# JuliaRobotics/IncrementalInference.jl

Measured on AMD Instinct MI355X. Metric: clique-messages/sec, higher is better.
Workload: dtype f64; 1 GPU; config 2: ContinuousEuclid(2) 1000-variable odometry chain + priors every 100, N=200 particles, nested-dissection order, full up+down solveTree; variables_per_gpu=1000, particles=200, cliques=983, parallelism=single GPU

## Files before the change

include/nbp.h:

```cpp
#ifndef NBP_H
#define NBP_H

#include <stdint.h>

#ifdef __cplusplus
extern "C" {
#endif

#define NBP_MAXV 6
#define NBP_MAXF 128
#define NBP_MAXD 3
#define NBP_MAXC 4
#define NBP_MAXK 8
#define NBP_MAXN 512
#define NBP_COMP_STRIDE 13
enum nbp_dist {
  NBP_DIST_GAUSSIAN = 0,
  NBP_DIST_UNIFORM = 1,
  NBP_DIST_RAYLEIGH = 2,
  NBP_DIST_TABLE = 3
};

typedef int32_t nbp_status;
#define NBP_OK 0
#define NBP_ERR_ARG (-1)
#define NBP_ERR_HIP (-2)
#define NBP_ERR_NOGPU (-3)
#define NBP_ERR_RANGE (-4)

enum nbp_manifold {
  NBP_EUCLID1 = 1,
  NBP_EUCLID2 = 2,
  NBP_EUCLID3 = 3,
  NBP_CIRCULAR = 4,
  NBP_SE2 = 5
};

enum nbp_factor {
  NBP_F_PRIOR = 1,
  NBP_F_MSGPRIOR = 2,
  NBP_F_LINREL = 3,
  NBP_F_CIRCULAR = 4,
  NBP_F_SE2 = 5,
  NBP_F_EUCLIDDIST = 6,
  NBP_F_PASSTHROUGH = 7
};

typedef struct nbp_proposal_desc {
  int32_t factor_kind;
  int32_t manifold;
  int32_t nvars;
  int32_t sfidx;
  int32_t var_slot[NBP_MAXV];
  int32_t out_slot;
  int32_t ncomp;
  int32_t has_multihypo;
  int32_t inflate_cycles;
  int32_t mhidx_in;
  int32_t mhidx_out;
  int32_t skip_bandwidth;
  int32_t partial_mask;
  int32_t meas_kde;
  int32_t keep_count;
  double multihypo[NBP_MAXV];
  double nullhypo;
  double inflation;
  double spread_nh;
  double comp[NBP_MAXC][NBP_COMP_STRIDE];
  uint64_t seed;
  uint64_t meas_seed;
} nbp_proposal_desc;

typedef struct nbp_product_desc {
  int32_t manifold;
  int32_t nfactors;
  int32_t niter;
  int32_t out_slot;
  int32_t in_slot[NBP_MAXF];
  int32_t labels_out;
  int32_t old_slot;
  uint8_t in_partial[NBP_MAXF];
  uint64_t seed;
} nbp_product_desc;

typedef struct nbp_copy_desc {
  int32_t src_slot;
  int32_t dst_slot;
} nbp_copy_desc;

typedef struct nbp_diag {
  int64_t solves;
  int64_t nonconverged;
  int64_t nan_results;
  int64_t residual_evals;
  int64_t lcv_evals;
  int64_t lcv_evals_f32;
  int64_t proposal_launches_workgroup;
  int64_t proposal_launches_wave;
  int64_t proposal_launches_split;
  int64_t lane_side_launches;
  int64_t lane_waits;
  int64_t lane_side_updates;
} nbp_diag;

typedef struct nbp_ctx nbp_ctx;

int64_t nbp_arena_bytes(int32_t N, int32_t n_slots);
int64_t nbp_slot_stride_doubles(int32_t N);
nbp_status nbp_ctx_create(int32_t device, int32_t N, int32_t n_slots, void *arena,
                          int64_t arena_bytes, int32_t side_ints, nbp_ctx **out);
nbp_status nbp_ctx_destroy(nbp_ctx *ctx);
nbp_status nbp_ctx_attach(nbp_ctx *ctx, void *obj, void (*destroy)(void *obj));
void *nbp_ctx_attached(const nbp_ctx *ctx);
const char *nbp_last_error(void);
nbp_status nbp_synchronize(nbp_ctx *ctx);
void *nbp_arena_ptr(nbp_ctx *ctx);
void *nbp_stream_ptr(nbp_ctx *ctx);
int32_t nbp_ctx_particles(const nbp_ctx *ctx);
int32_t nbp_ctx_slots(const nbp_ctx *ctx);
int32_t nbp_ctx_device(const nbp_ctx *ctx);
nbp_status nbp_ctx_reserve_resident(nbp_ctx *ctx, int32_t n);
int32_t nbp_ctx_resident(const nbp_ctx *ctx);

nbp_status nbp_slot_write(nbp_ctx *ctx, int32_t slot, int32_t manifold, const double *pts_NxP,
                          const double *bw_D );
nbp_status nbp_slot_read(nbp_ctx *ctx, int32_t slot, int32_t manifold, double *pts_NxP,
                         double *bw_D );
nbp_status nbp_belief_write(nbp_ctx *ctx, int32_t slot, int32_t manifold, const double *pts_NxP, int32_t n_pts,
                            const double *bw_D , const double *ipc_D );
nbp_status nbp_belief_read(nbp_ctx *ctx, int32_t slot, int32_t manifold, double *pts_NxP, int32_t *n_pts ,
                           double *bw_D , double *ipc_D );
nbp_status nbp_belief_write_batch(nbp_ctx *ctx, int32_t n, const int32_t *slots, const int32_t *manifolds, const double *const *pts,
                                  const int32_t *n_pts, const double *const *bw, const double *const *ipc);
nbp_status nbp_belief_read_batch(nbp_ctx *ctx, int32_t n, const int32_t *slots, const int32_t *manifolds, double *const *pts,
                                 int32_t *n_pts, double *const *bw, double *const *ipc);
typedef struct nbp_read_token nbp_read_token;
nbp_status nbp_belief_write_batch_async(nbp_ctx *ctx, int32_t n, const int32_t *slots, const int32_t *manifolds, const double *const *pts,
                                        const int32_t *n_pts, const double *const *bw, const double *const *ipc);
nbp_status nbp_belief_read_batch_begin(nbp_ctx *ctx, int32_t n, const int32_t *slots, nbp_read_token **out);
nbp_status nbp_belief_read_batch_end(nbp_read_token *token, const int32_t *manifolds, double *const *pts, int32_t *n_pts,
                                     double *const *bw, double *const *ipc);
nbp_status nbp_run_resample(nbp_ctx *ctx, const int32_t *slots, const int32_t *manifolds, int32_t n, uint64_t seed);
nbp_status nbp_side_write(nbp_ctx *ctx, int32_t offset, const int32_t *src, int32_t n);
nbp_status nbp_side_read(nbp_ctx *ctx, int32_t offset, int32_t *dst, int32_t n);

nbp_status nbp_run_proposals(nbp_ctx *ctx, const nbp_proposal_desc *descs, int32_t n);
nbp_status nbp_run_bandwidth(nbp_ctx *ctx, const int32_t *slots, const int32_t *manifolds, int32_t n);
nbp_status nbp_run_ppe(nbp_ctx *ctx, const int32_t *slots, const int32_t *manifolds, int32_t n,
                       double *mean_out , double *max_out ,
                       int32_t *max_index_out );
nbp_status nbp_kde_ppe(nbp_ctx *ctx, int32_t manifold, const double *pts_NxP, int32_t n_pts, const double *bw_D,
                       double *mean_out_D, double *max_out_D, int32_t *max_index_out );
nbp_status nbp_run_evaluate(nbp_ctx *ctx, const int32_t *slots, const int32_t *manifolds, int32_t n,
                            const int32_t *q_first ,
                            const double *queries , double *dens_out );
nbp_status nbp_kde_evaluate(nbp_ctx *ctx, int32_t manifold, const double *pts_NxP, int32_t n_pts, const double *bw_D,
                            const double *queries , int32_t nq, double *dens_out);
#define NBP_GRID_MAX 1024
#define NBP_GRID_AUTO_EXTENT 1
typedef struct nbp_grid_desc {
  int32_t slot;
  int32_t manifold;
  int32_t dims[2];
  int32_t n[2];
  int32_t flags;
  double lo[2];
  double step[2];
  double margin;
} nbp_grid_desc;
nbp_status nbp_run_marginal_grid(nbp_ctx *ctx, const nbp_grid_desc *descs, int32_t n_desc, const int32_t *first ,
                                 double *out , double *extent_out );
nbp_status nbp_kde_marginal_grid(nbp_ctx *ctx, int32_t manifold, const double *pts_NxP, int32_t n_pts, const double *bw_D,
                                 const nbp_grid_desc *desc, double *out, double *extent_out_4 );
nbp_status nbp_run_evaluate_marginal(nbp_ctx *ctx, const int32_t *slots, const int32_t *manifolds, const int32_t *masks, int32_t n,
                                     const int32_t *q_first ,
                                     const double *queries , double *dens_out );
nbp_status nbp_run_mmd(nbp_ctx *ctx, const int32_t *slots_a, const int32_t *slots_b, const int32_t *manifolds, int32_t n,
                       double sigma, double *mmd_out );
nbp_status nbp_kde_mmd(nbp_ctx *ctx, int32_t manifold, const double *a_NxP, int32_t na, const double *b_NxP, int32_t nb,
                       double sigma, double *mmd_out);
nbp_status nbp_run_meancov(nbp_ctx *ctx, const int32_t *slots, const int32_t *manifolds, int32_t n,
                           double *mean_out , double *cov_out );
nbp_status nbp_kde_meancov(nbp_ctx *ctx, int32_t manifold, const double *pts_NxP, int32_t n_pts, double *mean_out_D,
                           double *cov_out_DxD);
nbp_status nbp_run_kld(nbp_ctx *ctx, const int32_t *slots_a, const int32_t *slots_b, const int32_t *manifolds, int32_t n,
// ... 124 lines not shown
  double comp[NBP_MAXC][NBP_COMP_STRIDE];
} nbp_likelihood_desc;
nbp_status nbp_run_factor_likelihood(nbp_ctx *ctx, const nbp_likelihood_desc *descs, int32_t n, double *loglik_out ,
                                     double *comp_loglik_out );
nbp_status nbp_factor_likelihood(nbp_ctx *ctx, const nbp_likelihood_desc *desc, const double *a_NxP, int32_t na, const double *b_NxP,
                                 int32_t nb, double *loglik_out, double *comp_loglik_out );
#define NBP_PGRID_AUTO_EXTENT 1
#define NBP_PGRID_MAX_CELLS (1 << 22)
#define NBP_PGRID_CHUNK 256
typedef struct nbp_product_item {
  nbp_likelihood_desc lik;
  int32_t role;
  int32_t other;
  int32_t group;
  int32_t pad;
  double log_prior;
} nbp_product_item;
typedef struct nbp_product_grid_desc {
  int32_t manifold;
  int32_t slot;
  int32_t n[3];
  int32_t flags;
  int32_t first_item;
  int32_t n_items;
  double lo[3];
  double step[3];
  double margin;
} nbp_product_grid_desc;
typedef struct nbp_product_grid_rec {
  double logZ;
  double logmax;
  int32_t argmax;
  int32_t pad;
} nbp_product_grid_rec;
nbp_status nbp_run_product_grid(nbp_ctx *ctx, const nbp_product_grid_desc *descs, int32_t n_desc, const nbp_product_item *items,
                                int32_t n_items, const int32_t *first , double *logp_out ,
                                nbp_product_grid_rec *recs_out , double *extent_out );
nbp_status nbp_product_grid(nbp_ctx *ctx, const nbp_product_grid_desc *desc, const nbp_product_item *items, int32_t n_items,
                            const double *const *others , const int32_t *counts , const double *own_NxP,
                            int32_t n_own, const double *own_bw_D, double *logp_out, nbp_product_grid_rec *rec_out ,
                            double *extent_out_6 );
nbp_status nbp_run_factor_mode_likelihood(nbp_ctx *ctx, const nbp_likelihood_desc *descs, const int32_t *row_a ,
                                          const int32_t *row_b , int32_t n, const int32_t *labels ,
                                          int32_t n_rows, double *table_out ,
                                          int32_t *counts_out );
nbp_status nbp_factor_mode_likelihood(nbp_ctx *ctx, const nbp_likelihood_desc *desc, const double *a_NxP, int32_t na,
                                      const int32_t *labels_a , const double *b_NxP, int32_t nb,
                                      const int32_t *labels_b , double *table_out ,
                                      int32_t *counts_out );
#define NBP_ERR_INVALID (-5)
typedef struct nbp_heatmap nbp_heatmap;
nbp_status nbp_heatmap_create(nbp_ctx *ctx, const double *data , int32_t nx, int32_t ny, const double *x, const double *y,
                              double bw_factor, nbp_heatmap **out);
nbp_status nbp_heatmap_build(nbp_heatmap *hm, int32_t M, uint64_t seed, int32_t *cell_M, double *pre_Mx2, double *d_M, double *W_M);
nbp_status nbp_heatmap_draw(nbp_heatmap *hm, int32_t n, uint64_t seed, int32_t jitter, int32_t slot , int32_t *pick_n,
                            double *pts_nx2, double *bw_2);
nbp_status nbp_heatmap_info(const nbp_heatmap *hm, double *bw_2, double *total, double *wtotal, int32_t *M);
nbp_status nbp_heatmap_destroy(nbp_heatmap *hm);
nbp_status nbp_heatmap_scan_eval(nbp_ctx *ctx, const double *in, int32_t n, double *out);
nbp_status nbp_heatmap_search_eval(nbp_ctx *ctx, const double *cdf, int32_t n, const double *t, int32_t nt, int32_t *idx_out);
nbp_status nbp_run_products(nbp_ctx *ctx, const nbp_product_desc *descs, int32_t n);
nbp_status nbp_kde_bandwidth(nbp_ctx *ctx, int32_t manifold, const double *pts_NxP, double *bw_out_D);
nbp_status nbp_conv(nbp_ctx *ctx, const nbp_proposal_desc *tmpl, const double *const *var_pts, const double *const *var_bw,
                    const int32_t *mhidx_in, double *out_pts_NxP, double *out_bw_D, int32_t *out_mhidx);
nbp_status nbp_manifold_product(nbp_ctx *ctx, int32_t manifold, int32_t nfactors, const double *const *dens_pts,
                                const double *const *dens_bw, const uint8_t *partial_masks, const double *old_pts,
                                int32_t niter, uint64_t seed, double *out_pts_NxP, double *out_bw_D, int32_t *out_labels);

nbp_status nbp_run_deconv(nbp_ctx *ctx, const nbp_proposal_desc *descs, const int32_t *meas_slots, int32_t n);
nbp_status nbp_run_copies(nbp_ctx *ctx, const nbp_copy_desc *descs, int32_t n);
nbp_status nbp_run_copies_async(nbp_ctx *ctx, const nbp_copy_desc *descs, int32_t n, int32_t points_only);

typedef struct nbp_program nbp_program;
enum nbp_stage_kind {
  NBP_STAGE_PROPOSALS = 1,
  NBP_STAGE_PRODUCTS = 2,
  NBP_STAGE_COPIES = 3,
  NBP_STAGE_DECONV = 4,
  NBP_STAGE_COPY_POINTS = 5
};
nbp_status nbp_program_create(nbp_ctx *ctx, nbp_program **out);
nbp_status nbp_program_add_stage(nbp_program *prog, int32_t kind, const void *descs, int32_t n);
enum nbp_program_option { NBP_OPT_LAZY_BANDWIDTH = 1, NBP_OPT_GRAPH_REPLAY = 2, NBP_OPT_FUSED_UPDATES = 3,
                          NBP_OPT_ASYNC_UPLOAD = 4  };
nbp_status nbp_program_set_option(nbp_program *prog, int32_t option, int32_t value);
nbp_status nbp_program_finalize(nbp_program *prog);
nbp_status nbp_program_run(nbp_program *prog, int32_t first_stage, int32_t last_stage );
nbp_status nbp_program_reseed(nbp_program *prog, uint64_t salt);
nbp_status nbp_program_num_seeds(nbp_program *prog, int32_t *out);
nbp_status nbp_program_set_seeds(nbp_program *prog, const uint64_t *seeds, int32_t n);
nbp_status nbp_program_seed_order(nbp_program *prog, int32_t *order, int32_t n);
nbp_status nbp_program_num_stages(nbp_program *prog, int32_t *out);
nbp_status nbp_program_num_fused(nbp_program *prog, int32_t *out);
nbp_status nbp_program_num_two_stream(nbp_program *prog, int32_t *out);
nbp_status nbp_program_set_lanes(nbp_program *prog, int32_t stage, const int32_t *lane_of_descriptor, int32_t n);
typedef struct nbp_lane_part_rec {
  int32_t stage, lane, first_desc, n, wait, signals;
} nbp_lane_part_rec;
nbp_status nbp_program_lane_plan(nbp_program *prog, nbp_lane_part_rec *out, int32_t cap, int32_t *n_out);
nbp_status nbp_program_destroy(nbp_program *prog);
nbp_status nbp_program_retire(nbp_program *prog);

#define NBP_COMM_ID_BYTES 128
typedef struct nbp_comm nbp_comm;
#ifndef NBP_XFER_DEFINED
#define NBP_XFER_DEFINED
typedef struct nbp_xfer { int32_t peer; int32_t slot; } nbp_xfer;
#endif
nbp_status nbp_comm_unique_id(void *id_out );
nbp_status nbp_comm_create(nbp_ctx *ctx, int32_t world, int32_t rank, const void *id, nbp_comm **out);
nbp_status nbp_comm_destroy(nbp_comm *comm);
nbp_status nbp_comm_info(nbp_comm *comm, int32_t *nranks_out, int32_t *rank_out);
nbp_status nbp_exchange(nbp_ctx *ctx, nbp_comm *comm, const nbp_xfer *sends, int32_t n_sends, const nbp_xfer *recvs, int32_t n_recvs);

nbp_status nbp_timing_enable(nbp_ctx *ctx, int32_t on);
nbp_status nbp_timing_read(nbp_ctx *ctx, double *ms, int64_t *launches);
nbp_status nbp_timing_read_n(nbp_ctx *ctx, double *ms, int64_t *launches, int32_t n);
nbp_status nbp_diag_read(nbp_ctx *ctx, nbp_diag *out, int32_t reset);

typedef struct nbp_product_plan_req {
  int32_t N;
  int32_t n;
  int32_t F, D;
  int32_t mani;
  int32_t geom_n;
} nbp_product_plan_req;
#define NBP_PLAN_REFUSED_BIG_IN_ROUND 1
#define NBP_PLAN_REFUSED_LDS 2
#define NBP_PLAN_REFUSED_NO_KERNEL 3
typedef struct nbp_product_plan_rec {
  int32_t status, refusal;
  int32_t HL, wpb, G;
  int32_t big, xs, circ, nch, all_levels, w1;
  int32_t row;
  int32_t row_HL, row_mani, row_xs, row_w1;
  int32_t launch_bound;
  int32_t N, n, F, D, mani, geom_n;
  int32_t pad;
  int64_t lds, gstats;
  char kernel[40];
} nbp_product_plan_rec;
typedef struct nbp_fit_plan_req {
  int32_t N;
  int32_t fits, coords;
  int32_t products, kdF;
  int32_t geom_blocks;
} nbp_fit_plan_req;
typedef struct nbp_fit_plan_rec {
  int32_t status;
  int32_t P, depth, KS, w5, threads;
  int32_t prep;
  int32_t kd_nostats;
  int32_t N, fits, coords, products, kdF, geom_blocks;
  int32_t pad[2];
  int64_t lds;
  char kernel[40];
} nbp_fit_plan_rec;
typedef struct nbp_proposal_plan_req {
  int32_t N, n;
  int32_t manifold;
  int32_t simple;
} nbp_proposal_plan_req;
typedef struct nbp_proposal_plan_rec {
  int32_t status;
  int32_t geometry;
  int32_t blocks, threads;
  int32_t N, n, manifold, simple;
  int64_t lds;
  char kernel[40];
} nbp_proposal_plan_rec;
nbp_status nbp_plan_products(const nbp_product_plan_req *req, nbp_product_plan_rec *out, int64_t n);
nbp_status nbp_plan_fits(const nbp_fit_plan_req *req, nbp_fit_plan_rec *out, int64_t n);
nbp_status nbp_plan_proposals(const nbp_proposal_plan_req *req, nbp_proposal_plan_rec *out, int64_t n);
nbp_status nbp_last_plans(nbp_ctx *ctx, nbp_product_plan_rec *product, nbp_fit_plan_rec *prep, nbp_fit_plan_rec *fits);

nbp_status nbp_math_eval(nbp_ctx *ctx, int32_t fn, const double *a, const double *b, double *out0, double *out1, int64_t n);

#ifdef __cplusplus
}
#endif
#endif
```

incrementalinference.jl_amd/abi.py:

```python
import ctypes as C
import os

MAXV, MAXF, MAXD, MAXC, MAXN, COMP_STRIDE = 6, 128, 3, 4, 512, 13

EUCLID1, EUCLID2, EUCLID3, CIRCULAR, SE2 = 1, 2, 3, 4, 5
F_PRIOR, F_MSGPRIOR, F_LINREL, F_CIRCULAR, F_SE2, F_EUCLIDDIST, F_PASSTHROUGH = 1, 2, 3, 4, 5, 6, 7
DIST_GAUSSIAN, DIST_UNIFORM, DIST_RAYLEIGH, DIST_TABLE = 0, 1, 2, 3
STAGE_PROPOSALS, STAGE_PRODUCTS, STAGE_COPIES, STAGE_DECONV, STAGE_COPY_POINTS = 1, 2, 3, 4, 5
OPT_LAZY_BANDWIDTH = 1
OPT_GRAPH_REPLAY = 2
OPT_FUSED_UPDATES = 3

MANIFOLD_DIM = {EUCLID1: 1, EUCLID2: 2, EUCLID3: 3, CIRCULAR: 1, SE2: 3}
MANIFOLD_P = {EUCLID1: 1, EUCLID2: 2, EUCLID3: 3, CIRCULAR: 1, SE2: 6}


class ProposalDesc(C.Structure):
    _fields_ = [
        ("factor_kind", C.c_int32),
        ("manifold", C.c_int32),
        ("nvars", C.c_int32),
        ("sfidx", C.c_int32),
        ("var_slot", C.c_int32 * MAXV),
        ("out_slot", C.c_int32),
        ("ncomp", C.c_int32),
        ("has_multihypo", C.c_int32),
        ("inflate_cycles", C.c_int32),
        ("mhidx_in", C.c_int32),
        ("mhidx_out", C.c_int32),
        ("skip_bandwidth", C.c_int32),
        ("partial_mask", C.c_int32),
        ("meas_kde", C.c_int32),
        ("keep_count", C.c_int32),
        ("multihypo", C.c_double * MAXV),
        ("nullhypo", C.c_double),
        ("inflation", C.c_double),
        ("spread_nh", C.c_double),
        ("comp", (C.c_double * COMP_STRIDE) * MAXC),
        ("seed", C.c_uint64),
        ("meas_seed", C.c_uint64),
    ]


class ProductDesc(C.Structure):
    _fields_ = [
        ("manifold", C.c_int32),
        ("nfactors", C.c_int32),
        ("niter", C.c_int32),
        ("out_slot", C.c_int32),
        ("in_slot", C.c_int32 * MAXF),
        ("labels_out", C.c_int32),
        ("old_slot", C.c_int32),
        ("in_partial", C.c_uint8 * MAXF),
        ("seed", C.c_uint64),
    ]


class CopyDesc(C.Structure):
    _fields_ = [("src_slot", C.c_int32), ("dst_slot", C.c_int32)]


class GridDesc(C.Structure):
    _fields_ = [
        ("slot", C.c_int32),
        ("manifold", C.c_int32),
        ("dims", C.c_int32 * 2),
        ("n", C.c_int32 * 2),
        ("flags", C.c_int32),
        ("lo", C.c_double * 2),
        ("step", C.c_double * 2),
        ("margin", C.c_double),
    ]


GRID_MAX, GRID_AUTO_EXTENT = 1024, 1


class ModesOpts(C.Structure):
    _fields_ = [("bw_scale", C.c_double), ("tol", C.c_double), ("merge", C.c_double), ("max_iter", C.c_int32), ("pad", C.c_int32)]


class ModeRec(C.Structure):
    _fields_ = [("location", C.c_double * MAXD), ("density", C.c_double), ("count", C.c_int32), ("leader", C.c_int32)]


MODES_MAX = 32
MODES_BW_SCALE, MODES_TOL, MODES_MAX_ITER, MODES_MERGE = 2.0, 1e-6, 500, 1e-2

MIX_MAX = 8
MIX_TOL, MIX_MAX_ITER = 1e-8, 500


class MixtureOpts(C.Structure):
    _fields_ = [("tol", C.c_double), ("max_iter", C.c_int32), ("pad", C.c_int32)]
# ... 10 lines not shown
                ("partial_mask", C.c_int32), ("comp", (C.c_double * COMP_STRIDE) * MAXC)]


class ProductItem(C.Structure):
    _fields_ = [("lik", LikelihoodDesc), ("role", C.c_int32), ("other", C.c_int32), ("group", C.c_int32), ("pad", C.c_int32),
                ("log_prior", C.c_double)]


class ProductGridDesc(C.Structure):
    _fields_ = [("manifold", C.c_int32), ("slot", C.c_int32), ("n", C.c_int32 * 3), ("flags", C.c_int32), ("first_item", C.c_int32),
                ("n_items", C.c_int32), ("lo", C.c_double * 3), ("step", C.c_double * 3), ("margin", C.c_double)]


class ProductGridRec(C.Structure):
    _fields_ = [("logZ", C.c_double), ("logmax", C.c_double), ("argmax", C.c_int32), ("pad", C.c_int32)]


PGRID_AUTO_EXTENT, PGRID_MAX_CELLS, PGRID_CHUNK, PGRID_MARGIN = 1, 1 << 22, 256, 4.0


MAXK = 8


class OverlapRec(C.Structure):
    _fields_ = [("logc", C.c_double), ("lab", C.c_double), ("laa", C.c_double), ("lbb", C.c_double)]


class OverlapOpts(C.Structure):
    _fields_ = [("reach", C.c_double), ("min_coeff", C.c_double), ("topk", C.c_int32), ("pad", C.c_int32)]


OVERLAP_MAXK, OVERLAP_REACH, OVERLAP_MIN_COEFF, OVERLAP_TOPK = 16, 6.0, 1e-3, 8


class SceneDesc(C.Structure):
    _fields_ = [("n", C.c_int32 * 2), ("flags", C.c_int32), ("pad", C.c_int32), ("lo", C.c_double * 2), ("step", C.c_double * 2),
                ("margin", C.c_double), ("reach", C.c_double)]


SCENE_AUTO_EXTENT, SCENE_MAX, SCENE_REACH, SCENE_MARGIN, SCENE_MAX_POINTS = 1, 4096, 6.0, 4.0, 1 << 22

CRED_MAX = 8


class CredibleOpts(C.Structure):
    _fields_ = [("n_mass", C.c_int32), ("n_prob", C.c_int32), ("mass", C.c_double * CRED_MAX), ("prob", C.c_double * CRED_MAX)]


class CredibleRec(C.Structure):
    _fields_ = [("log_level", C.c_double * CRED_MAX), ("quant", (C.c_double * CRED_MAX) * MAXD), ("mean", C.c_double * MAXD),
                ("log_min", C.c_double), ("log_max", C.c_double), ("n_inside", C.c_int32 * CRED_MAX), ("count", C.c_int32),
                ("pad", C.c_int32)]


class CredibilityRec(C.Structure):
    _fields_ = [("logdens", C.c_double), ("mass", C.c_double), ("n_above", C.c_int32), ("pad", C.c_int32)]


ERR_INVALID = -5
HM_MAX_CELLS = 1 << 26


class Xfer(C.Structure):
    _fields_ = [("peer", C.c_int32), ("slot", C.c_int32)]


COMM_ID_BYTES = 128


class Diag(C.Structure):
    _fields_ = [
        ("solves", C.c_int64),
        ("nonconverged", C.c_int64),
        ("nan_results", C.c_int64),
        ("residual_evals", C.c_int64),
        ("lcv_evals", C.c_int64),
        ("lcv_evals_f32", C.c_int64),
        ("proposal_launches_workgroup", C.c_int64),
        ("proposal_launches_wave", C.c_int64),
        ("proposal_launches_split", C.c_int64),
        ("lane_side_launches", C.c_int64),
        ("lane_waits", C.c_int64),
        ("lane_side_updates", C.c_int64),
    ]


class LanePartRec(C.Structure):
    _fields_ = [("stage", C.c_int32), ("lane", C.c_int32), ("first_desc", C.c_int32), ("n", C.c_int32), ("wait", C.c_int32), ("signals", C.c_int32)]


class ProductPlanReq(C.Structure):
    _fields_ = [(k, C.c_int32) for k in ("N", "n", "F", "D", "mani", "geom_n")]


PLAN_REFUSED_BIG_IN_ROUND, PLAN_REFUSED_LDS, PLAN_REFUSED_NO_KERNEL = 1, 2, 3


class _PlanRec(C.Structure):
    def as_dict(self):
        return {k: (getattr(self, k).decode() if k == "kernel" else getattr(self, k)) for k, _ in self._fields_ if not k.startswith("pad")}


class ProductPlanRec(_PlanRec):
    _fields_ = [(k, C.c_int32) for k in ("status", "refusal", "HL", "wpb", "G", "big", "xs", "circ", "nch", "all_levels", "w1", "row", "row_HL",
                                         "row_mani", "row_xs", "row_w1", "launch_bound", "N", "n", "F", "D", "mani", "geom_n", "pad")] + \
               [("lds", C.c_int64), ("gstats", C.c_int64), ("kernel", C.c_char * 40)]


class FitPlanReq(C.Structure):
    _fields_ = [(k, C.c_int32) for k in ("N", "fits", "coords", "products", "kdF", "geom_blocks")]


class FitPlanRec(_PlanRec):
    _fields_ = [(k, C.c_int32) for k in ("status", "P", "depth", "KS", "w5", "threads", "prep", "kd_nostats", "N", "fits", "coords", "products",
                                         "kdF", "geom_blocks")] + [("pad", C.c_int32 * 2), ("lds", C.c_int64), ("kernel", C.c_char * 40)]


class ProposalPlanReq(C.Structure):
    _fields_ = [(k, C.c_int32) for k in ("N", "n", "manifold", "simple")]


class ProposalPlanRec(_PlanRec):
    _fields_ = [(k, C.c_int32) for k in ("status", "geometry", "blocks", "threads", "N", "n", "manifold", "simple")] + \
               [("lds", C.c_int64), ("kernel", C.c_char * 40)]


def _plan(fn_name, Req, Rec, reqs):
    lib = load_library()
    n = len(reqs)
    arr = (Req * n)(*[Req(*r) for r in reqs])
    out = (Rec * n)()
    rc = getattr(lib, fn_name)(arr, out, n)
    if rc != 0:
        raise ValueError(f"{fn_name}: status {rc}: {lib.nbp_last_error().decode()}")
    return out


def plan_products(reqs):
    return _plan("nbp_plan_products", ProductPlanReq, ProductPlanRec, reqs)


def plan_fits(reqs):
    return _plan("nbp_plan_fits", FitPlanReq, FitPlanRec, reqs)


def plan_proposals(reqs):
    return _plan("nbp_plan_proposals", ProposalPlanReq, ProposalPlanRec, reqs)


def slot_stride(N):
    return 3 * N + 8


_PKG_DIR = os.path.dirname(os.path.abspath(__file__))
LIB_PATH = os.path.join(_PKG_DIR, "csrc", "libnbp.so")

EXPORTS = [
    "nbp_arena_bytes", "nbp_slot_stride_doubles", "nbp_ctx_create", "nbp_ctx_destroy",
    "nbp_last_error", "nbp_synchronize", "nbp_arena_ptr", "nbp_stream_ptr", "nbp_ctx_particles", "nbp_ctx_slots", "nbp_ctx_device",
    "nbp_ctx_reserve_resident", "nbp_ctx_resident", "nbp_belief_write_batch_async", "nbp_belief_read_batch_begin", "nbp_belief_read_batch_end",
    "nbp_run_copies_async", "nbp_program_retire",
    "nbp_slot_write", "nbp_slot_read", "nbp_belief_write", "nbp_belief_read", "nbp_belief_write_batch", "nbp_belief_read_batch", "nbp_run_resample", "nbp_side_write", "nbp_side_read",
    "nbp_run_proposals", "nbp_run_bandwidth", "nbp_run_ppe", "nbp_kde_ppe", "nbp_run_evaluate", "nbp_kde_evaluate", "nbp_run_marginal_grid", "nbp_kde_marginal_grid", "nbp_run_evaluate_marginal", "nbp_run_mmd", "nbp_kde_mmd", "nbp_run_meancov", "nbp_kde_meancov", "nbp_run_kld", "nbp_kde_kld", "nbp_run_overlap", "nbp_kde_overlap", "nbp_run_overlap_search", "nbp_run_scene_grid", "nbp_run_credible", "nbp_kde_credible", "nbp_run_modes", "nbp_kde_modes", "nbp_run_mixture", "nbp_kde_mixture", "nbp_run_factor_likelihood", "nbp_factor_likelihood", "nbp_run_factor_mode_likelihood", "nbp_factor_mode_likelihood", "nbp_run_product_grid", "nbp_product_grid", "nbp_heatmap_create", "nbp_heatmap_build", "nbp_heatmap_draw", "nbp_heatmap_info", "nbp_heatmap_destroy", "nbp_heatmap_scan_eval", "nbp_heatmap_search_eval", "nbp_run_products", "nbp_run_copies", "nbp_run_deconv", "nbp_kde_bandwidth", "nbp_conv", "nbp_manifold_product",
    "nbp_program_create", "nbp_program_add_stage", "nbp_program_set_option", "nbp_program_finalize", "nbp_program_run",
    "nbp_program_reseed", "nbp_program_num_seeds", "nbp_program_set_seeds", "nbp_program_seed_order", "nbp_ctx_attach", "nbp_ctx_attached", "nbp_program_num_stages", "nbp_program_num_fused", "nbp_program_num_two_stream", "nbp_program_set_lanes", "nbp_program_lane_plan", "nbp_program_destroy",
    "nbp_timing_enable", "nbp_timing_read", "nbp_timing_read_n", "nbp_diag_read",
    "nbp_plan_products", "nbp_plan_fits", "nbp_plan_proposals", "nbp_last_plans",
    "nbp_comm_unique_id", "nbp_comm_create", "nbp_comm_destroy", "nbp_comm_info", "nbp_exchange", "nbp_math_eval",
]

_lib = None


def load_library(path=None):
    global _lib
    if _lib is not None and path is None:
        return _lib
    path = path or os.environ.get("NBP_LIB_OVERRIDE") or LIB_PATH
    if not os.path.exists(path):
        raise RuntimeError(
            f"libnbp.so not found at {path}: build it with `python __graft_entry__.py` "
            "(hipcc --offload-arch=gfx950). The product path has no CPU fallback."
        )
    try:
        import torch
    except ImportError:
        pass
    lib = C.CDLL(path)
    vp, i32, i64, dp = C.c_void_p, C.c_int32, C.c_int64, C.POINTER(C.c_double)
    ip = C.POINTER(C.c_int32)
    lib.nbp_arena_bytes.restype = i64
    lib.nbp_arena_bytes.argtypes = [i32, i32]
    lib.nbp_slot_stride_doubles.restype = i64
    lib.nbp_slot_stride_doubles.argtypes = [i32]
    lib.nbp_ctx_create.argtypes = [i32, i32, i32, vp, i64, i32, C.POINTER(vp)]
    lib.nbp_ctx_destroy.argtypes = [vp]
    lib.nbp_last_error.restype = C.c_char_p
    lib.nbp_synchronize.argtypes = [vp]
    lib.nbp_arena_ptr.restype = vp
    lib.nbp_arena_ptr.argtypes = [vp]
    lib.nbp_stream_ptr.restype = vp
    lib.nbp_stream_ptr.argtypes = [vp]
    lib.nbp_ctx_particles.argtypes = [vp]
    lib.nbp_ctx_slots.argtypes = [vp]
    lib.nbp_ctx_device.argtypes = [vp]
    lib.nbp_slot_write.argtypes = [vp, i32, i32, dp, dp]
    lib.nbp_slot_read.argtypes = [vp, i32, i32, dp, dp]
    lib.nbp_belief_write.argtypes = [vp, i32, i32, dp, i32, dp, dp]
    lib.nbp_belief_read.argtypes = [vp, i32, i32, dp, ip, dp, dp]
    lib.nbp_belief_write_batch.argtypes = [vp, i32, ip, ip, C.POINTER(dp), ip, C.POINTER(dp), C.POINTER(dp)]
    lib.nbp_belief_read_batch.argtypes = [vp, i32, ip, ip, C.POINTER(dp), ip, C.POINTER(dp), C.POINTER(dp)]
    lib.nbp_run_resample.argtypes = [vp, ip, ip, i32, C.c_uint64]
    lib.nbp_side_write.argtypes = [vp, i32, ip, i32]
    lib.nbp_side_read.argtypes = [vp, i32, ip, i32]
    lib.nbp_run_proposals.argtypes = [vp, C.POINTER(ProposalDesc), i32]
    lib.nbp_run_bandwidth.argtypes = [vp, ip, ip, i32]
    lib.nbp_run_ppe.argtypes = [vp, ip, ip, i32, dp, dp, ip]
    lib.nbp_kde_ppe.argtypes = [vp, i32, dp, i32, dp, dp, dp, ip]
    lib.nbp_run_evaluate.argtypes = [vp, ip, ip, i32, ip, dp, dp]
    lib.nbp_kde_evaluate.argtypes = [vp, i32, dp, i32, dp, dp, i32, dp]
    lib.nbp_run_marginal_grid.argtypes = [vp, C.POINTER(GridDesc), i32, ip, dp, dp]
    lib.nbp_kde_marginal_grid.argtypes = [vp, i32, dp, i32, dp, C.POINTER(GridDesc), dp, dp]
    lib.nbp_run_evaluate_marginal.argtypes = [vp, ip, ip, ip, i32, ip, dp, dp]
    lib.nbp_run_mmd.argtypes = [vp, ip, ip, ip, i32, C.c_double, dp]
    lib.nbp_kde_mmd.argtypes = [vp, i32, dp, i32, dp, i32, C.c_double, dp]
    lib.nbp_run_meancov.argtypes = [vp, ip, ip, i32, dp, dp]
    lib.nbp_kde_meancov.argtypes = [vp, i32, dp, i32, dp, dp]
    lib.nbp_run_kld.argtypes = [vp, ip, ip, ip, i32, dp, dp]
    lib.nbp_kde_kld.argtypes = [vp, i32, dp, i32, dp, dp, i32, dp, dp, dp]
    lib.nbp_run_overlap.argtypes = [vp, ip, ip, ip, ip, ip, ip, i32, C.POINTER(OverlapRec)]
    lib.nbp_kde_overlap.argtypes = [vp, i32, dp, i32, dp, i32, i32, dp, i32, dp, i32, C.POINTER(OverlapRec)]
    lib.nbp_run_overlap_search.argtypes = [vp, ip, ip, ip, i32, C.POINTER(OverlapOpts), ip, dp, ip, ip]
    lib.nbp_run_scene_grid.argtypes = [vp, ip, ip, ip, dp, i32, C.POINTER(SceneDesc), dp, ip, ip, dp, C.POINTER(i64)]
    lib.nbp_run_credible.argtypes = [vp, ip, ip, ip, i32, C.POINTER(CredibleOpts), ip, dp, C.POINTER(CredibleRec), dp, ip,
                                     C.POINTER(CredibilityRec)]
    lib.nbp_kde_credible.argtypes = [vp, i32, dp, i32, dp, i32, C.POINTER(CredibleOpts), dp, i32, C.POINTER(CredibleRec), dp, ip,
                                     C.POINTER(CredibilityRec)]
    lib.nbp_run_modes.argtypes = [vp, ip, ip, i32, C.POINTER(ModesOpts), C.POINTER(ModeRec), ip, ip, ip, ip]
    lib.nbp_kde_modes.argtypes = [vp, i32, dp, i32, dp, C.POINTER(ModesOpts), C.POINTER(ModeRec), ip, ip, ip, ip]
    lib.nbp_run_mixture.argtypes = [vp, ip, ip, i32, ip, ip, dp, C.POINTER(MixtureOpts), C.POINTER(MixtureRec), ip]
    lib.nbp_kde_mixture.argtypes = [vp, i32, dp, i32, dp, ip, dp, C.POINTER(MixtureOpts), C.POINTER(MixtureRec), ip]
    lib.nbp_run_factor_likelihood.argtypes = [vp, C.POINTER(LikelihoodDesc), i32, dp, dp]
    lib.nbp_factor_likelihood.argtypes = [vp, C.POINTER(LikelihoodDesc), dp, i32, dp, i32, dp, dp]
    lib.nbp_run_factor_mode_likelihood.argtypes = [vp, C.POINTER(LikelihoodDesc), ip, ip, i32, ip, i32, dp, ip]
    lib.nbp_factor_mode_likelihood.argtypes = [vp, C.POINTER(LikelihoodDesc), dp, i32, ip, dp, i32, ip, dp, ip]
    lib.nbp_run_product_grid.argtypes = [vp, C.POINTER(ProductGridDesc), i32, C.POINTER(ProductItem), i32, ip, dp, C.POINTER(ProductGridRec), dp]
    lib.nbp_product_grid.argtypes = [vp, C.POINTER(ProductGridDesc), C.POINTER(ProductItem), i32, C.POINTER(dp), ip, dp, i32, dp, dp,
                                     C.POINTER(ProductGridRec), dp]
    lib.nbp_heatmap_create.argtypes = [vp, dp, i32, i32, dp, dp, C.c_double, C.POINTER(vp)]
    lib.nbp_heatmap_build.argtypes = [vp, i32, C.c_uint64, ip, dp, dp, dp]
    lib.nbp_heatmap_draw.argtypes = [vp, i32, C.c_uint64, i32, i32, ip, dp, dp]
    lib.nbp_heatmap_info.argtypes = [vp, dp, dp, dp, ip]
    lib.nbp_heatmap_destroy.argtypes = [vp]
    lib.nbp_heatmap_scan_eval.argtypes = [vp, dp, i32, dp]
    lib.nbp_heatmap_search_eval.argtypes = [vp, dp, i32, dp, i32, ip]
    lib.nbp_run_deconv.argtypes = [vp, C.POINTER(ProposalDesc), ip, i32]
    dpp = C.POINTER(dp)
    lib.nbp_kde_bandwidth.argtypes = [vp, i32, dp, dp]
    lib.nbp_conv.argtypes = [vp, C.POINTER(ProposalDesc), dpp, dpp, ip, dp, dp, ip]
    lib.nbp_manifold_product.argtypes = [vp, i32, i32, dpp, dpp, C.POINTER(C.c_uint8), dp, i32, C.c_uint64, dp, dp, ip]
    lib.nbp_run_products.argtypes = [vp, C.POINTER(ProductDesc), i32]
    lib.nbp_run_copies.argtypes = [vp, C.POINTER(CopyDesc), i32]
    lib.nbp_program_create.argtypes = [vp, C.POINTER(vp)]
    lib.nbp_program_add_stage.argtypes = [vp, i32, vp, i32]
    lib.nbp_program_set_option.argtypes = [vp, i32, i32]
    lib.nbp_program_finalize.argtypes = [vp]
    lib.nbp_program_run.argtypes = [vp, i32, i32]
    lib.nbp_program_reseed.argtypes = [vp, C.c_uint64]
    lib.nbp_program_num_seeds.argtypes = [vp, ip]
    lib.nbp_program_set_seeds.argtypes = [vp, C.POINTER(C.c_uint64), i32]
    lib.nbp_program_seed_order.argtypes = [vp, ip, i32]
    lib.nbp_program_num_stages.argtypes = [vp, ip]
    lib.nbp_program_destroy.argtypes = [vp]
    lib.nbp_comm_unique_id.argtypes = [vp]
    lib.nbp_comm_create.argtypes = [vp, i32, i32, vp, C.POINTER(vp)]
    lib.nbp_comm_destroy.argtypes = [vp]
    lib.nbp_comm_info.argtypes = [vp, ip, ip]
    lib.nbp_math_eval.argtypes = [vp, i32, dp, dp, dp, dp, i64]
    lib.nbp_exchange.argtypes = [vp, vp, C.POINTER(Xfer), i32, C.POINTER(Xfer), i32]
    lib.nbp_timing_enable.argtypes = [vp, i32]
    lib.nbp_timing_read.argtypes = [vp, dp, C.POINTER(i64)]
    lib.nbp_timing_read_n.argtypes = [vp, dp, C.POINTER(i64), i32]
    lib.nbp_program_num_fused.argtypes = [vp, C.POINTER(i32)]
    lib.nbp_program_num_two_stream.argtypes = [vp, C.POINTER(i32)]
    lib.nbp_program_set_lanes.argtypes = [vp, i32, ip, i32]
    lib.nbp_program_lane_plan.argtypes = [vp, C.POINTER(LanePartRec), i32, C.POINTER(i32)]
    lib.nbp_diag_read.argtypes = [vp, C.POINTER(Diag), i32]
    lib.nbp_plan_products.argtypes = [C.POINTER(ProductPlanReq), C.POINTER(ProductPlanRec), i64]
    lib.nbp_plan_fits.argtypes = [C.POINTER(FitPlanReq), C.POINTER(FitPlanRec), i64]
    lib.nbp_plan_proposals.argtypes = [C.POINTER(ProposalPlanReq), C.POINTER(ProposalPlanRec), i64]
    lib.nbp_last_plans.argtypes = [vp, C.POINTER(ProductPlanRec), C.POINTER(FitPlanRec), C.POINTER(FitPlanRec)]
    for name in EXPORTS:
        fn = getattr(lib, name)
        if fn.restype is C.c_int:
            fn.restype = C.c_int32
    if path == LIB_PATH:
        _lib = lib
    return lib
```

incrementalinference.jl_amd/backend.py:

```python
import ctypes as C
import weakref

import numpy as np

from . import abi


class NbpError(RuntimeError):
    """Hard error from libnbp (status < 0).  The Julia shim maps this to `error()`, which fails
    the clique Task and makes `monitorCSMs` tear the solve down with a CompositeException
    (reference: CliqStateMachineUtils.jl:184-246, test/testCSMMonitor.jl:51)."""


_IP, _DP = C.POINTER(C.c_int32), C.POINTER(C.c_double)


def _i32(seq):
    a = np.ascontiguousarray(seq, dtype=np.int32)
    return a, a.ctypes.data_as(_IP)


def _f64(a, shape=None):
    a = np.ascontiguousarray(a, dtype=np.float64)
    a = a if shape is None else a.reshape(shape)
# ... 637 lines not shown

    def math_eval(self, fn, a, b=None):
        dp = C.POINTER(C.c_double)
        a = np.ascontiguousarray(a, dtype=np.float64)
        b = None if b is None else np.ascontiguousarray(b, dtype=np.float64)
        o0, o1 = np.empty_like(a), np.empty_like(a)
        self._check(self.lib.nbp_math_eval(self._ctx, fn, a.ctypes.data_as(dp), b.ctypes.data_as(dp) if b is not None else C.cast(None, dp),
                                           o0.ctypes.data_as(dp), o1.ctypes.data_as(dp), a.size))
        return o0, o1

    def comm_destroy(self):
        if getattr(self, "_comm", None):
            self.lib.nbp_comm_destroy(self._comm)
            self._comm = None

    def exchange(self, sends, recvs):
        sx = (abi.Xfer * max(1, len(sends)))(*[abi.Xfer(p, s) for p, s in sends])
        rx = (abi.Xfer * max(1, len(recvs)))(*[abi.Xfer(p, s) for p, s in recvs])
        self._check(self.lib.nbp_exchange(self._ctx, self._comm, sx, len(sends), rx, len(recvs)))

    def program(self, stages, lazy_bandwidth=False, fused_updates=True):
        return HipProgram(self, stages, lazy_bandwidth, fused_updates)

    def timing_enable(self, on=True):
        self._check(self.lib.nbp_timing_enable(self._ctx, int(on)))

    KERNELS = ("nbp_proposal_kernel", "nbp_prep_kernel", "nbp_product_kernel", "nbp_bandwidth_kernel", "nbp_update_kernel")

    def timing_read(self):
        ms = (C.c_double * 5)()
        nl = (C.c_int64 * 5)()
        self._check(self.lib.nbp_timing_read_n(self._ctx, ms, nl, 5))
        return {k: (ms[i], nl[i]) for i, k in enumerate(self.KERNELS)}

    def diag(self, reset=False):
        d = abi.Diag()
        self._check(self.lib.nbp_diag_read(self._ctx, C.byref(d), int(reset)))
        return {k: getattr(d, k) for k, _ in abi.Diag._fields_}

    def last_plans(self):
        p, q, f = abi.ProductPlanRec(), abi.FitPlanRec(), abi.FitPlanRec()
        self._check(self.lib.nbp_last_plans(self._ctx, C.byref(p), C.byref(q), C.byref(f)))
        return {"product": p.as_dict(), "prep": q.as_dict(), "fits": f.as_dict()}

    def arena_ptr(self):
        return self.lib.nbp_arena_ptr(self._ctx)

    def stream_ptr(self):
        return self.lib.nbp_stream_ptr(self._ctx)


_STAGE_CTYPE = {abi.STAGE_PROPOSALS: abi.ProposalDesc, abi.STAGE_PRODUCTS: abi.ProductDesc,
                abi.STAGE_COPIES: abi.CopyDesc, abi.STAGE_DECONV: abi.ProposalDesc,
                abi.STAGE_COPY_POINTS: abi.CopyDesc}


class HipProgram:

    def __init__(self, backend, stages, lazy_bandwidth=False, fused_updates=True, lanes=None):
        self.backend, lib = backend, backend.lib
        self._p = C.c_void_p()
        backend._check(lib.nbp_program_create(backend._ctx, C.byref(self._p)))
        backend._programs.add(self)
        if lazy_bandwidth:
            backend._check(lib.nbp_program_set_option(self._p, abi.OPT_LAZY_BANDWIDTH, 1))
        if not fused_updates:
            backend._check(lib.nbp_program_set_option(self._p, abi.OPT_FUSED_UPDATES, 0))
        for kind, descs in stages:
            arr, n = _as_array(descs, _STAGE_CTYPE[kind])
            backend._check(lib.nbp_program_add_stage(self._p, kind, C.cast(arr, C.c_void_p), n))
        for s, hint in (lanes or {}).items():
            arr = (C.c_int32 * max(len(hint), 1))(*[int(x) for x in hint])
            backend._check(lib.nbp_program_set_lanes(self._p, s, arr, len(hint)))
        backend._check(lib.nbp_program_finalize(self._p))
        self.n_stages = len(stages)

    def lane_plan(self):
        n = C.c_int32(0)
        self.backend._check(self.backend.lib.nbp_program_lane_plan(self._p, None, 0, C.byref(n)))
        recs = (abi.LanePartRec * max(n.value, 1))()
        self.backend._check(self.backend.lib.nbp_program_lane_plan(self._p, recs, n.value, C.byref(n)))
        return [{k: getattr(r, k) for k, _ in abi.LanePartRec._fields_} for r in recs[:n.value]]

    def num_fused(self):
        n = C.c_int32(0)
        self.backend._check(self.backend.lib.nbp_program_num_fused(self._p, C.byref(n)))
        return n.value

    def num_two_stream(self):
        n = C.c_int32(0)
        self.backend._check(self.backend.lib.nbp_program_num_two_stream(self._p, C.byref(n)))
        return n.value

    def run(self, first=0, last=-1):
        self.backend._check(self.backend.lib.nbp_program_run(self._p, first, last))

    def reseed(self, salt):
        self.backend._check(self.backend.lib.nbp_program_reseed(self._p, C.c_uint64(salt)))

    def num_seeds(self):
        n = C.c_int32(0)
        self.backend._check(self.backend.lib.nbp_program_num_seeds(self._p, C.byref(n)))
        return n.value

    def set_seeds(self, seeds):
        arr = (C.c_uint64 * len(seeds))(*[int(x) for x in seeds])
        self.backend._check(self.backend.lib.nbp_program_set_seeds(self._p, arr, len(seeds)))

    def seed_order(self):
        n = self.num_seeds()
        arr = (C.c_int32 * max(n, 1))()
        self.backend._check(self.backend.lib.nbp_program_seed_order(self._p, arr, n))
        return list(arr[:n])

    @staticmethod
    def seeds_of(stages):
        out = []
        for kind, descs in stages:
            if kind in (abi.STAGE_PROPOSALS, abi.STAGE_DECONV):
                for d in descs:
                    out.append(d.seed)
                    if d.meas_seed:
                        out.append(d.meas_seed)
            elif kind == abi.STAGE_PRODUCTS:
                out.extend(d.seed for d in descs)
        return out

    def close(self):
        if self._p:
            self.backend.lib.nbp_program_destroy(self._p)
            self._p = C.c_void_p()

    def __del__(self):
        try:
            self.close()
        except Exception:
            pass
```

incrementalinference.jl_amd/csrc/nbp_api.hip:

```cpp
#include <hip/hip_runtime.h>

#include <cmath>
#include <cstdio>
#include <cstring>
#include <string>
#include <thread>
#include <vector>

#include <unordered_map>

#include <dlfcn.h>
#include <algorithm>
#include <rccl/rccl.h>

#ifndef NBP_TU
#define NBP_TU 0
#endif
#include "nbp_kernels.h"
#include "nbp_fused.h"
#include "nbp_ppe.h"
#include "nbp_query.h"
#include "nbp_stats.h"
#include "nbp_marginal.h"
#include "nbp_heatmap.h"
#include "nbp_modes.h"
#include "nbp_likelihood.h"
#include "nbp_overlap.h"
#include "nbp_credible.h"
#include "nbp_mixture.h"
#include "nbp_scene.h"
#include "nbp_productgrid.h"
#include "../../include/nbp_lanes.h"

static thread_local std::string g_err;
static nbp_status fail(nbp_status code, const std::string &msg) {
  g_err = msg;
  return code;
}
template <class F>
static void host_parallel_for(int n, int grain, F &&f) {
  const unsigned hw = std::thread::hardware_concurrency();
  int nt = n / grain;
  if (nt > 8) nt = 8;
  if (hw && nt > (int)hw) nt = (int)hw;
  if (nt <= 1) {
    for (int i = 0; i < n; i++) f(i);
    return;
  }
  auto part = [&](int t) {
    const int a = (int)((int64_t)n * t / nt), b = (int)((int64_t)n * (t + 1) / nt);
    for (int i = a; i < b; i++) f(i);
  };
  std::vector<std::thread> th;
  for (int t = 1; t < nt; t++) th.emplace_back(part, t);
  part(0);
  for (std::thread &x : th) x.join();
}

extern "C" nbp_status nbp_internal_fail(nbp_status code, const char *msg) { return fail(code, msg ? msg : ""); }
#define HIPCHK(expr)                                                                               \
  do {                                                                                             \
    hipError_t e_ = (expr);                                                                        \
    if (e_ != hipSuccess)                                                                          \
      return fail(NBP_ERR_HIP, std::string(#expr) + " (nbp_api.hip:" + std::to_string(__LINE__) + "): " + hipGetErrorString(e_)); \
  } while (0)

#ifndef NBP_SPEC_MAXJOBS
#define NBP_SPEC_MAXJOBS 40
#endif
#ifndef NBP_SPEC_MAXBLOCKS
#define NBP_SPEC_MAXBLOCKS 224
#endif
struct nbp_program;
struct nbp_comm;
struct nbp_ctx {
  std::vector<nbp_heatmap *> heatmaps;
  std::vector<nbp_program *> programs;
  std::vector<nbp_comm *> comms;
  void *attached = nullptr;
  void (*attached_destroy)(void *) = nullptr;
  uint64_t ws_gen = 0;
  int device = 0, N = 0, n_slots = 0, side_ints = 0, threads = 0, Npad = 0, P = 1;
  int64_t S = 0;
  double *arena = nullptr;
  bool own_arena = false;
  int32_t *side = nullptr;
  nbp_counters *counters = nullptr;
  hipStream_t stream = nullptr;
  nbp_levels T{};
  int32_t *lv_ints = nullptr;
  double *lv_dbls = nullptr;
  double *ws = nullptr;
  size_t ws_doubles = 0;
  nbp_spec_area *spec = nullptr;
  bool spec_on = true;
  bool spec_depth3 = true;
  double *gstats = nullptr;
  size_t gstats_doubles = 0;
  void *stage = nullptr;
  size_t stage_bytes = 0;
  double *query = nullptr;
  size_t query_cap = 0;
  double *pin = nullptr;
  size_t pin_doubles = 0;
  std::vector<std::pair<char *, size_t>> blob_cache;
  struct pin_buf { char *p = nullptr; size_t bytes = 0; hipEvent_t ev = nullptr; bool pending = false, held = false; };
  std::vector<pin_buf *> pin_pool;
  std::vector<std::pair<nbp_program *, hipEvent_t>> retired;
  int resident = 0;
  bool fused_on = true;
  int fused_min = 1 << 30;
  int prop_wave_min = -1;
  int prop_split_min = -1;
  int64_t prop_launches[3] = {0, 0, 0};
  int fused_p1_min = 2048;
  hipStream_t stream2 = nullptr;
  hipEvent_t pipe_ev[2] = {nullptr, nullptr};
  int pipe_min = 1 << 30;
  bool no_lanes = false;
  std::vector<hipEvent_t> lane_ev;
  hipEvent_t lane_fork = nullptr, lane_join = nullptr;
  double *gstats1 = nullptr;
  size_t gstats1_doubles = 0;
  int64_t lane_side_launches = 0, lane_waits = 0, lane_side_updates = 0;
  int lcv_p2_min = 256, lcv_p1_min = 4 * 256;
  bool fit_w5 = true, debug_occupancy = false;
  int prod_hl2_min = 192, prod_nch = 0, prod_all_levels_hl = 8;
  bool prod_xs = true, prod_lat_uni = true;
  nbp_product_plan_rec last_product{};
  nbp_fit_plan_rec last_prep{}, last_fit{};
  bool timing = false;
  std::vector<std::pair<hipEvent_t, hipEvent_t>> ev[5];
  double ms[5] = {0, 0, 0, 0, 0};
  int64_t nl[5] = {0, 0, 0, 0, 0};
};

typedef void (*nbp_product_fn)(const nbp_product_desc *, double *, const double *, int, double *, int, int64_t, int32_t *, nbp_levels);
struct nbp_product_kernel_row { nbp_product_fn fn; int HL, mani; bool xs, w1; const char *name; int lb; };
#define NBP_ROW(NAME, HL_, MANI_, XS_, W1_, LB_) {NAME, HL_, MANI_, XS_, W1_, #NAME, LB_}
static const nbp_product_kernel_row NBP_PRODUCT_KERNELS[] = {
    NBP_ROW(nbp_product_kernel_y32, 32, 0, false, false, 512),           NBP_ROW(nbp_product_kernel_y32_w1, 32, 0, false, true, 256),
    NBP_ROW(nbp_product_kernel_l8, 8, 0, false, false, 512),             NBP_ROW(nbp_product_kernel_l8_w1, 8, 0, false, true, 256),
    NBP_ROW(nbp_product_kernel_t2, 2, 0, false, false, 512),
    NBP_ROW(nbp_product_kernel_y32_e1, 32, NBP_EUCLID1, false, false, 512), NBP_ROW(nbp_product_kernel_y32_e2, 32, NBP_EUCLID2, false, false, 512),
    NBP_ROW(nbp_product_kernel_y32_e3, 32, NBP_EUCLID3, false, false, 512), NBP_ROW(nbp_product_kernel_y32_ci, 32, NBP_CIRCULAR, false, false, 512),
    NBP_ROW(nbp_product_kernel_y32_se, 32, NBP_SE2, false, false, 512),
    NBP_ROW(nbp_product_kernel_l8_e1, 8, NBP_EUCLID1, false, false, 512),   NBP_ROW(nbp_product_kernel_l8_e2, 8, NBP_EUCLID2, false, false, 512),
    NBP_ROW(nbp_product_kernel_l8_e3, 8, NBP_EUCLID3, false, false, 512),   NBP_ROW(nbp_product_kernel_l8_ci, 8, NBP_CIRCULAR, false, false, 512),
    NBP_ROW(nbp_product_kernel_l8_se, 8, NBP_SE2, false, false, 512),
    NBP_ROW(nbp_product_kernel_t2_e1, 2, NBP_EUCLID1, false, false, NBP_PROD_LB(NBP_EUCLID1)),   NBP_ROW(nbp_product_kernel_t2_e2, 2, NBP_EUCLID2, false, false, NBP_PROD_LB(NBP_EUCLID2)),
    NBP_ROW(nbp_product_kernel_t2_e3, 2, NBP_EUCLID3, false, false, NBP_PROD_LB(NBP_EUCLID3)),   NBP_ROW(nbp_product_kernel_t2_ci, 2, NBP_CIRCULAR, false, false, NBP_PROD_LB(NBP_CIRCULAR)),
    NBP_ROW(nbp_product_kernel_t2_se, 2, NBP_SE2, false, false, NBP_PROD_LB(NBP_SE2)),
    NBP_ROW(nbp_product_kernel_t2_e1_xs, 2, NBP_EUCLID1, true, false, NBP_PROD_LB(NBP_EUCLID1)), NBP_ROW(nbp_product_kernel_t2_e2_xs, 2, NBP_EUCLID2, true, false, NBP_PROD_LB(NBP_EUCLID2)),
    NBP_ROW(nbp_product_kernel_t2_e3_xs, 2, NBP_EUCLID3, true, false, NBP_PROD_LB(NBP_EUCLID3)), NBP_ROW(nbp_product_kernel_t2_ci_xs, 2, NBP_CIRCULAR, true, false, NBP_PROD_LB(NBP_CIRCULAR)),
    NBP_ROW(nbp_product_kernel_t2_se_xs, 2, NBP_SE2, true, false, NBP_PROD_LB(NBP_SE2)),
};
#undef NBP_ROW

static int manifold_dim_h(int m) { return m == NBP_SE2 ? 3 : (m == NBP_CIRCULAR ? 1 : m); }
static int manifold_P_h(int m) { return m == NBP_SE2 ? 6 : manifold_dim_h(m); }
static bool manifold_ok(int m) { return m >= NBP_EUCLID1 && m <= NBP_SE2; }
static bool manifold_circ_h(int m, int d) { return (m == NBP_CIRCULAR && d == 0) || (m == NBP_SE2 && d == 2); }
static double wrap_h(double a) { return nbpm_wrap_pi(a); }

#define NBPCHK(...)                    \
  do {                                 \
    nbp_status rc_ = (__VA_ARGS__);    \
    if (rc_) return rc_;               \
  } while (0)
struct refusal {
  nbp_status code;
  const char *what;
};
static refusal no_refusal(int) { return {NBP_OK, nullptr}; }
static refusal mask_refusal(int manifold, int32_t mask) {
  if (mask == 0) return {NBP_ERR_RANGE, "empty mask"};
  if (mask < 0 || (mask >> manifold_dim_h(manifold)) != 0) return {NBP_ERR_RANGE, "coordinate outside the manifold"};
  return {NBP_OK, nullptr};
}

template <class K, class... A>
static nbp_status launch_checked(nbp_ctx *c, K kernel, size_t blocks, int lanes, size_t lds, A... args) {
  (void)hipGetLastError();
  hipLaunchKernelGGL(kernel, dim3((unsigned)blocks), dim3(lanes), lds, c->stream, args...);
  HIPCHK(hipGetLastError());
  return NBP_OK;
}

template <class Extra>
static nbp_status batch_check(nbp_ctx *c, const char *who, std::initializer_list<const int32_t *> slot_cols, const int32_t *manifolds,
                              int n, Extra extra) {
  HIPCHK(hipSetDevice(c->device));
  for (int i = 0; i < n; i++) {
    refusal r{NBP_OK, nullptr};
    for (const int32_t *s : slot_cols)
      if (s[i] < 0 || s[i] >= c->n_slots) r = {NBP_ERR_RANGE, "slot out of range"};
    if (!r.what && !manifold_ok(manifolds[i])) r = {NBP_ERR_ARG, "unknown manifold"};
    if (!r.what) r = extra(i);
    if (r.what) return fail(r.code, std::string(who) + ": belief " + std::to_string(i) + ": " + r.what);
  }
  return NBP_OK;
}

extern "C" {

int64_t nbp_slot_stride_doubles(int32_t N) { return 3 * (int64_t)N + 8; }
int64_t nbp_arena_bytes(int32_t N, int32_t n_slots) { return nbp_slot_stride_doubles(N) * 8 * (int64_t)n_slots; }
// ... 4 lines not shown
  lo[0] = {0};
  hi[0] = {N};
  int l = 0;
  for (;;) {
    bool all_leaf = true;
    for (size_t k = 0; k < lo[l].size(); k++)
      if (hi[l][k] - lo[l][k] > 1) all_leaf = false;
    if (all_leaf) break;
    lo.emplace_back();
    hi.emplace_back();
    child.emplace_back();
    for (size_t k = 0; k < lo[l].size(); k++) {
      int a = lo[l][k], b = hi[l][k];
      if (b - a == 1) {
        lo[l + 1].push_back(a);
        hi[l + 1].push_back(b);
      } else {
        int mid = a + (b - a + 1) / 2;
        lo[l + 1].push_back(a); hi[l + 1].push_back(mid);
        lo[l + 1].push_back(mid); hi[l + 1].push_back(b);
      }
      child[l].push_back((int)lo[l + 1].size() - 1);
    }
    l++;
    if (l >= NBP_MAXLEVELS - 1) return fail(NBP_ERR_RANGE, "tree too deep");
  }
  const int L = l;
  int total = 0;
  for (int i = 0; i <= L; i++) { T.cnt[i] = (int)lo[i].size(); T.off[i] = total; total += T.cnt[i]; }
  if ((size_t)total > nbp_kd_nodes_cap(N)) return fail(NBP_ERR_RANGE, "level tables exceed the node-sum workspace");
  std::vector<int32_t> nlo(total), nhi(total), nch(total, 0), pos((size_t)(L + 1) * N);
  dbls.resize(2 * (size_t)total);
  for (int i = 0; i <= L; i++)
    for (int k = 0; k < T.cnt[i]; k++) {
      nlo[T.off[i] + k] = lo[i][k];
      nhi[T.off[i] + k] = hi[i][k];
      if (i < L) nch[T.off[i] + k] = child[i][k];
      dbls[T.off[i] + k] = std::log((double)(hi[i][k] - lo[i][k]) / (double)N);
      dbls[total + T.off[i] + k] = (double)(hi[i][k] - lo[i][k]) / (double)N;
      for (int p = lo[i][k]; p < hi[i][k]; p++) pos[(size_t)i * N + p] = k;
    }
  ints.insert(ints.end(), nlo.begin(), nlo.end());
  ints.insert(ints.end(), nhi.begin(), nhi.end());
  ints.insert(ints.end(), nch.begin(), nch.end());
  ints.insert(ints.end(), pos.begin(), pos.end());
  T.N = N;
  T.L = L;
  return NBP_OK;
}
static nbp_status build_levels(nbp_ctx *c) {
  std::vector<int32_t> ints;
  std::vector<double> dbls;
  NBPCHK(levels_host(c->N, c->T, ints, dbls));
  const int total = c->T.off[c->T.L] + c->T.cnt[c->T.L];
  HIPCHK(hipMalloc(&c->lv_ints, ints.size() * 4));
  HIPCHK(hipMalloc(&c->lv_dbls, dbls.size() * 8));
  HIPCHK(hipMemcpy(c->lv_ints, ints.data(), ints.size() * 4, hipMemcpyHostToDevice));
  HIPCHK(hipMemcpy(c->lv_dbls, dbls.data(), dbls.size() * 8, hipMemcpyHostToDevice));
  c->T.node_lo = c->lv_ints;
  c->T.node_hi = c->lv_ints + total;
  c->T.node_child = c->lv_ints + 2 * total;
  c->T.pos_node = c->lv_ints + 3 * total;
  c->T.node_logw = c->lv_dbls;
  c->T.node_w = c->lv_dbls + total;
  return NBP_OK;
}

static void ctx_plan_fields(nbp_ctx *c, int N) {
  c->N = N;
  c->S = nbp_slot_stride_doubles(N);
  c->Npad = ((N + 63) / 64) * 64;
  c->P = 1024 / c->Npad;
  if (c->P > 4) c->P = 4;
  if (c->P < 1) c->P = 1;
  c->threads = c->P * c->Npad;
  c->spec_on = getenv("NBP_NO_SPECULATIVE_FITS") == nullptr;
  c->spec_depth3 = !(getenv("NBP_SPEC_DEPTH3") && atoi(getenv("NBP_SPEC_DEPTH3")) == 0);
  c->fused_on = getenv("NBP_NO_FUSED_UPDATE") == nullptr;
  if (getenv("NBP_FUSED_MIN")) c->fused_min = atoi(getenv("NBP_FUSED_MIN"));
  if (getenv("NBP_PROPOSAL_WAVE_MIN")) c->prop_wave_min = atoi(getenv("NBP_PROPOSAL_WAVE_MIN"));
  if (getenv("NBP_PROPOSAL_SPLIT_MIN")) c->prop_split_min = atoi(getenv("NBP_PROPOSAL_SPLIT_MIN"));
  if (getenv("NBP_PIPELINE_MIN")) c->pipe_min = atoi(getenv("NBP_PIPELINE_MIN"));
  c->no_lanes = getenv("NBP_NO_LANES") && atoi(getenv("NBP_NO_LANES")) != 0;
  if (getenv("NBP_FUSED_P1_MIN")) c->fused_p1_min = atoi(getenv("NBP_FUSED_P1_MIN"));
  if (getenv("NBP_PRODUCT_HL2_MIN")) c->prod_hl2_min = atoi(getenv("NBP_PRODUCT_HL2_MIN"));
  if (getenv("NBP_PRODUCT_NCH")) c->prod_nch = atoi(getenv("NBP_PRODUCT_NCH"));
  if (getenv("NBP_PRODUCT_ALL_LEVELS_HL")) c->prod_all_levels_hl = atoi(getenv("NBP_PRODUCT_ALL_LEVELS_HL"));
  c->prod_xs = getenv("NBP_NO_XS_PRODUCTS") == nullptr;
  c->prod_lat_uni = getenv("NBP_NO_UNIFORM_LATENCY_PRODUCTS") == nullptr;
  if (getenv("NBP_LCV_P2_MIN")) c->lcv_p2_min = atoi(getenv("NBP_LCV_P2_MIN"));
  if (getenv("NBP_LCV_P1_MIN")) c->lcv_p1_min = atoi(getenv("NBP_LCV_P1_MIN"));
  c->fit_w5 = getenv("NBP_NO_W5_FITS") == nullptr;
  c->debug_occupancy = getenv("NBP_DEBUG_OCCUPANCY") != nullptr;
}

nbp_status nbp_ctx_create(int32_t device, int32_t N, int32_t n_slots, void *arena, int64_t arena_bytes,
                          int32_t side_ints, nbp_ctx **out) {
  if (!out) return fail(NBP_ERR_ARG, "out is null");
  if (N < 8 || N > NBP_MAXN) return fail(NBP_ERR_RANGE, "N must be in [8, 512]");
  if (n_slots < 1) return fail(NBP_ERR_ARG, "n_slots < 1");
  int ndev = 0;
  if (hipGetDeviceCount(&ndev) != hipSuccess || ndev == 0)
    return fail(NBP_ERR_NOGPU, "no HIP device visible: libnbp has no CPU fallback");
  if (device < 0 || device >= ndev) return fail(NBP_ERR_ARG, "bad device index");
  HIPCHK(hipSetDevice(device));
  nbp_ctx *c = new nbp_ctx();
  struct guard_t {
    nbp_ctx *c;
    ~guard_t() { if (c) nbp_ctx_destroy(c); }
  } guard{c};
  c->device = device;
  c->n_slots = n_slots;
  ctx_plan_fields(c, N);
  c->side_ints = side_ints > 0 ? side_ints : 1;
  if (arena) {
    if (arena_bytes < nbp_arena_bytes(N, n_slots)) return fail(NBP_ERR_ARG, "arena too small");
    c->arena = (double *)arena;
  } else {
    HIPCHK(hipMalloc(&c->arena, nbp_arena_bytes(N, n_slots)));
    HIPCHK(hipMemset(c->arena, 0, nbp_arena_bytes(N, n_slots)));
    c->own_arena = true;
  }
  HIPCHK(hipMalloc(&c->side, (size_t)c->side_ints * 4));
  HIPCHK(hipMemset(c->side, 0, (size_t)c->side_ints * 4));
  HIPCHK(hipMalloc(&c->counters, sizeof(nbp_counters)));
  HIPCHK(hipMemset(c->counters, 0, sizeof(nbp_counters)));
  {
    const char *e = getenv("NBP_FIT_F64");
    const unsigned long long fl = (e && *e && *e != '0') ? 1ull : 0ull;
    HIPCHK(hipMemcpy(&c->counters->flags, &fl, sizeof(fl), hipMemcpyHostToDevice));
  }
  HIPCHK(hipStreamCreateWithFlags(&c->stream, hipStreamNonBlocking));
  HIPCHK(hipMalloc(&c->spec, sizeof(nbp_spec_area) * 3 * NBP_SPEC_MAXJOBS * 2));
  HIPCHK(hipStreamCreateWithFlags(&c->stream2, hipStreamNonBlocking));
  for (int i = 0; i < 2; i++) HIPCHK(hipEventCreateWithFlags(&c->pipe_ev[i], hipEventDisableTiming));
  HIPCHK(hipEventCreateWithFlags(&c->lane_fork, hipEventDisableTiming));
  HIPCHK(hipEventCreateWithFlags(&c->lane_join, hipEventDisableTiming));
  nbp_status rc = build_levels(c);
  if (rc != NBP_OK) return rc;
  for (const nbp_product_kernel_row &k : NBP_PRODUCT_KERNELS)
    HIPCHK(hipFuncSetAttribute((const void *)k.fn, hipFuncAttributeMaxDynamicSharedMemorySize, 160 * 1024));
  for (const void *k : {(const void *)nbp_bandwidth_kernel, (const void *)nbp_prep_kernel, (const void *)nbp_bandwidth_kernel_spec<2>,
                        (const void *)nbp_bandwidth_kernel_spec<3>, (const void *)nbp_prep_kernel_spec<2>, (const void *)nbp_prep_kernel_spec<3>})
    HIPCHK(hipFuncSetAttribute(k, hipFuncAttributeMaxDynamicSharedMemorySize, 160 * 1024));
  HIPCHK(hipFuncSetAttribute((const void *)nbp_update_kernel_lin2_p1, hipFuncAttributeMaxDynamicSharedMemorySize, 158 * 1024));
  HIPCHK(hipFuncSetAttribute((const void *)nbp_update_kernel_lin2_p2, hipFuncAttributeMaxDynamicSharedMemorySize, 158 * 1024));

  guard.c = nullptr;
  *out = c;
  return NBP_OK;
}

static void program_detach(nbp_program *p);
static void program_delete(nbp_program *p);
static void ctx_detach_comms(nbp_ctx *c);
static void heatmap_release(nbp_heatmap *hm);
static void reap_retired(nbp_ctx *c);

nbp_status nbp_ctx_attach(nbp_ctx *c, void *obj, void (*destroy)(void *)) {
  if (!c) return fail(NBP_ERR_ARG, "ctx is null");
  if (c->attached && c->attached_destroy && c->attached != obj) c->attached_destroy(c->attached);
  c->attached = obj;
  c->attached_destroy = destroy;
  return NBP_OK;
}
void *nbp_ctx_attached(const nbp_ctx *c) { return c ? c->attached : nullptr; }
// ... 2276 lines not shown
  delete hm;
  return NBP_OK;
}

nbp_status nbp_heatmap_scan_eval(nbp_ctx *c, const double *in, int32_t n, double *out) {
  if (!c) return fail(NBP_ERR_ARG, "null argument");
  if (n < 1 || n > NBP_HM_MAX_CELLS) return fail(NBP_ERR_INVALID, "heatmap scan_eval: n outside 1 .. 2^26");
  if (!in || !out) return fail(NBP_ERR_ARG, "null argument");
  HIPCHK(hipSetDevice(c->device));
  const size_t tiles = ((size_t)n + NBP_HM_TILE - 1) / NBP_HM_TILE;
  double *d_in = nullptr, *d_out = nullptr, *t2 = nullptr, *p2 = nullptr;
  auto body = [&]() -> nbp_status {
    HIPCHK(hipMalloc(&d_in, sizeof(double) * (size_t)n));
    HIPCHK(hipMalloc(&d_out, sizeof(double) * (size_t)n));
    HIPCHK(hipMalloc(&t2, sizeof(double) * tiles));
    HIPCHK(hipMalloc(&p2, sizeof(double) * tiles));
    HIPCHK(hipMemcpyAsync(d_in, in, sizeof(double) * (size_t)n, hipMemcpyHostToDevice, c->stream));
    NBPCHK(heatmap_scan(c, d_in, n, t2, p2, d_out));
    HIPCHK(hipMemcpyAsync(out, d_out, sizeof(double) * (size_t)n, hipMemcpyDeviceToHost, c->stream));
    HIPCHK(hipStreamSynchronize(c->stream));
    return NBP_OK;
  };
  const nbp_status rc = body();
  if (rc) hipStreamSynchronize(c->stream);
  for (void *p : {(void *)d_in, (void *)d_out, (void *)t2, (void *)p2})
    if (p) hipFree(p);
  return rc;
}

nbp_status nbp_heatmap_search_eval(nbp_ctx *c, const double *cdf, int32_t n, const double *t, int32_t nt, int32_t *idx_out) {
  if (!c) return fail(NBP_ERR_ARG, "null argument");
  if (n < 1 || n > NBP_HM_MAX_CELLS) return fail(NBP_ERR_INVALID, "heatmap search_eval: n outside 1 .. 2^26");
  if (nt < 1 || nt > NBP_HM_MAX_CELLS) return fail(NBP_ERR_INVALID, "heatmap search_eval: nt outside 1 .. 2^26");
  if (!cdf || !t || !idx_out) return fail(NBP_ERR_ARG, "null argument");
  HIPCHK(hipSetDevice(c->device));
  double *d_cdf = nullptr, *d_t = nullptr;
  int32_t *d_idx = nullptr;
  auto body = [&]() -> nbp_status {
    HIPCHK(hipMalloc(&d_cdf, sizeof(double) * (size_t)n));
    HIPCHK(hipMalloc(&d_t, sizeof(double) * (size_t)nt));
    HIPCHK(hipMalloc(&d_idx, sizeof(int32_t) * (size_t)nt));
    HIPCHK(hipMemcpyAsync(d_cdf, cdf, sizeof(double) * (size_t)n, hipMemcpyHostToDevice, c->stream));
    HIPCHK(hipMemcpyAsync(d_t, t, sizeof(double) * (size_t)nt, hipMemcpyHostToDevice, c->stream));
    NBPCHK(launch_checked(c, nbp_hm_search_eval_kernel, ((size_t)nt + NBP_HM_LANES - 1) / NBP_HM_LANES, NBP_HM_LANES, 0,
                          (const double *)d_cdf, (int)n, (const double *)d_t, (int)nt, d_idx));
    HIPCHK(hipMemcpyAsync(idx_out, d_idx, sizeof(int32_t) * (size_t)nt, hipMemcpyDeviceToHost, c->stream));
    HIPCHK(hipStreamSynchronize(c->stream));
    return NBP_OK;
  };
  const nbp_status rc = body();
  if (rc) hipStreamSynchronize(c->stream);
  for (void *p : {(void *)d_cdf, (void *)d_t, (void *)d_idx})
    if (p) hipFree(p);
  return rc;
}

nbp_status nbp_run_resample(nbp_ctx *c, const int32_t *slots, const int32_t *manifolds, int32_t n, uint64_t seed) {
  if (!c || ((!slots || !manifolds) && n > 0)) return fail(NBP_ERR_ARG, "null argument");
  if (n <= 0) return NBP_OK;
  NBPCHK(batch_check(c, "resample", {slots}, manifolds, n, no_refusal));
  const int32_t *d[2];
  NBPCHK(stage_columns(c, {{slots, 4 * (size_t)n}, {manifolds, 4 * (size_t)n}}, d, 0));
  NBPCHK(launch_checked(c, nbp_resample_kernel, n, 256, 0, d[0], d[1], c->arena, c->N, c->S, seed));
  HIPCHK(hipStreamSynchronize(c->stream));
  return NBP_OK;
}

struct nbp_stage {
  int kind = 0, n = 0, maxfd = 0, mani = 0;
  size_t offset = 0;
  nbp_fits ent;
  bool flush_before = false;
  bool need_prep = true;
  bool fused = false, fused_second = false;
  int upd_F = 0;
  std::vector<nbp_update_desc> upd;
  size_t upd_off = 0;
  nbp_fits split_out;
  bool pipe = false;
  int pipe_split = -1, pipe_ent = 0;
  std::vector<int> moved_to;
  std::vector<int32_t> lane_hint;
  int lane_split = -1;
  int lane = 0, user = -1;
  nbp_fits bound;
  std::vector<int> waits;
  bool signals = false;
};
struct nbp_program {
  nbp_ctx *ctx = nullptr;
  std::vector<nbp_stage> stages;
  std::vector<char> blob;
  char *dev = nullptr;
  size_t dev_bytes = 0;
  bool finalized = false;
  bool lazy_bw = false;
  bool use_graph = true;
  bool use_fused = true;
  bool async_upload = false;
  int n_user_stages = 0;
  struct captured { hipGraphExec_t exec; uint64_t ws_gen; };
  std::unordered_map<uint64_t, captured> graphs;
  std::unordered_map<uint64_t, int> runs;
  size_t seed_off = 0;
  size_t seed_val_off = 0;
  int n_seeds = 0;
  std::vector<int32_t> seed_rank;
  std::vector<nbp_stage> parts;
  std::vector<int> first_part;
  size_t lane_ws = 0, lane_gstats = 0;
};

nbp_status nbp_program_create(nbp_ctx *c, nbp_program **out) {
  if (!c || !out) return fail(NBP_ERR_ARG, "null argument");
  nbp_program *p = new nbp_program();
  p->ctx = c;
  c->programs.push_back(p);
  *out = p;
  return NBP_OK;
}
static void program_detach(nbp_program *p) {
  for (auto &kv : p->graphs) hipGraphExecDestroy(kv.second.exec);
  p->graphs.clear();
  if (p->dev) hipFree(p->dev);
  p->dev = nullptr;
  p->ctx = nullptr;
}
static void program_delete(nbp_program *p) {
  program_detach(p);
  delete p;
}
#define PROG_ALIVE(p) do { if (!(p)->ctx) return fail(NBP_ERR_ARG, "the program's context was destroyed"); } while (0)

nbp_status nbp_program_add_stage(nbp_program *p, int32_t kind, const void *descs, int32_t n) {
  if (!p || (!descs && n > 0)) return fail(NBP_ERR_ARG, "null argument");
  PROG_ALIVE(p);
  if (p->finalized) return fail(NBP_ERR_ARG, "program already finalized");
  if (n < 0) return fail(NBP_ERR_ARG, "n < 0");
  size_t esz;
  nbp_status rc = NBP_OK;
  nbp_stage st;
  switch (kind) {
  case NBP_STAGE_PROPOSALS:
    esz = sizeof(nbp_proposal_desc);
    rc = check_proposals(p->ctx, (const nbp_proposal_desc *)descs, n);
    st.mani = proposals_uniform_class((const nbp_proposal_desc *)descs, n);
    break;
  case NBP_STAGE_PRODUCTS:
    esz = sizeof(nbp_product_desc);
    rc = check_products(p->ctx, (const nbp_product_desc *)descs, n);
    st.maxfd = products_maxfd((const nbp_product_desc *)descs, n);
    st.mani = products_uniform_manifold((const nbp_product_desc *)descs, n);
    break;
  case NBP_STAGE_COPIES:
  case NBP_STAGE_COPY_POINTS: esz = sizeof(nbp_copy_desc); rc = check_copies(p->ctx, (const nbp_copy_desc *)descs, n); break;
  case NBP_STAGE_DECONV: esz = sizeof(nbp_proposal_desc); rc = check_deconv(p->ctx, (const nbp_proposal_desc *)descs, n); break;
  default: return fail(NBP_ERR_ARG, "unknown stage kind");
  }
  if (rc) return rc;
  size_t off = (p->blob.size() + 63) & ~(size_t)63;
  p->blob.resize(off + esz * (size_t)n);
  if (n) memcpy(p->blob.data() + off, descs, esz * (size_t)n);
  st.kind = kind; st.n = n; st.offset = off;
  p->stages.push_back(st);
  return NBP_OK;
}

nbp_status nbp_program_set_lanes(nbp_program *p, int32_t stage, const int32_t *lane_of_descriptor, int32_t n) {
  if (!p || (!lane_of_descriptor && n > 0)) return fail(NBP_ERR_ARG, "null argument");
  PROG_ALIVE(p);
  if (p->finalized) return fail(NBP_ERR_ARG, "program already finalized");
  if (stage < 0 || stage >= (int)p->stages.size()) return fail(NBP_ERR_RANGE, "set_lanes: no such stage");
  nbp_stage &st = p->stages[(size_t)stage];
  if (n != st.n) return fail(NBP_ERR_ARG, "set_lanes: one lane per descriptor of the stage");
  for (int i = 0; i < n; i++)
    if (lane_of_descriptor[i] != 0 && lane_of_descriptor[i] != 1) return fail(NBP_ERR_RANGE, "set_lanes: a lane is 0 or 1");
  st.lane_hint.assign(lane_of_descriptor, lane_of_descriptor + n);
  return NBP_OK;
}

nbp_status nbp_program_set_option(nbp_program *p, int32_t option, int32_t value) {
  if (!p) return fail(NBP_ERR_ARG, "null argument");
  if (option == NBP_OPT_GRAPH_REPLAY && p->finalized) { p->use_graph = value != 0; return NBP_OK; }
  if (p->finalized) return fail(NBP_ERR_ARG, "program already finalized");
  if (option == NBP_OPT_LAZY_BANDWIDTH) { p->lazy_bw = value != 0 && getenv("NBP_NO_LAZY_BANDWIDTH") == nullptr; return NBP_OK; }
  if (option == NBP_OPT_GRAPH_REPLAY) { p->use_graph = value != 0; return NBP_OK; }
  if (option == NBP_OPT_FUSED_UPDATES) { p->use_fused = value != 0; return NBP_OK; }
  if (option == NBP_OPT_ASYNC_UPLOAD) { p->async_upload = value != 0; return NBP_OK; }
  return fail(NBP_ERR_ARG, "unknown program option");
}

enum nbp_access {
  NBP_RD_POINTS,
  NBP_RD_KDE,
  NBP_RD_CARRY
};
extern "C++" {
template <class F>
static void proposal_reads(const nbp_proposal_desc &d, F &&f) {
  for (int k = 0; k < d.nvars; k++) f(d.var_slot[k], NBP_RD_POINTS);
  if (d.factor_kind == NBP_F_MSGPRIOR || d.factor_kind == NBP_F_PASSTHROUGH) f(d.var_slot[1], NBP_RD_KDE);
  if (d.meas_kde > 0) f(d.meas_kde - 1, NBP_RD_KDE);
}
template <class F>
static void stage_reads(const nbp_program *p, const nbp_stage &st, F &&f, bool idle_old = false) {
  const char *d = p->blob.data() + st.offset;
  for (int i = 0; i < st.n; i++)
    if (st.kind == NBP_STAGE_PROPOSALS || st.kind == NBP_STAGE_DECONV) {
      proposal_reads(((const nbp_proposal_desc *)d)[i], [&](int32_t slot, nbp_access a) { f(i, slot, a); });
    } else if (st.kind == NBP_STAGE_PRODUCTS) {
      const nbp_product_desc &q = ((const nbp_product_desc *)d)[i];
      for (int j = 0; j < q.nfactors; j++) f(i, q.in_slot[j], q.nfactors > 1 ? NBP_RD_KDE : NBP_RD_CARRY);
      if (q.old_slot >= 0 && (q.nfactors > 1 || idle_old)) f(i, q.old_slot, NBP_RD_POINTS);
    } else if (st.kind == NBP_STAGE_COPIES || st.kind == NBP_STAGE_COPY_POINTS) {
      f(i, ((const nbp_copy_desc *)d)[i].src_slot, st.kind == NBP_STAGE_COPIES ? NBP_RD_KDE : NBP_RD_POINTS);
    }
}
template <class F>
static void stage_writes(const nbp_program *p, const nbp_stage &st, F &&f) {
  const char *d = p->blob.data() + st.offset;
  for (int i = 0; i < st.n; i++)
    if (st.kind == NBP_STAGE_PROPOSALS || st.kind == NBP_STAGE_DECONV) f(i, ((const nbp_proposal_desc *)d)[i].out_slot);
    else if (st.kind == NBP_STAGE_PRODUCTS) f(i, ((const nbp_product_desc *)d)[i].out_slot);
    else if (st.kind == NBP_STAGE_COPIES || st.kind == NBP_STAGE_COPY_POINTS) f(i, ((const nbp_copy_desc *)d)[i].dst_slot);
}
}

struct nbp_liveness {
  std::vector<std::vector<char>> dead_product, dead_proposal;
};
static nbp_liveness product_liveness(const nbp_program *p) {
  nbp_liveness L;
  L.dead_product.resize(p->n_user_stages);
  L.dead_proposal.resize(p->n_user_stages);
  struct Open { int stage, idx, pstage, pidx; };
  std::unordered_map<int32_t, Open> open;
  std::unordered_map<int32_t, std::pair<int, int>> last_prop;
  std::vector<std::pair<int, int>> needed;
  auto read_kde = [&](int32_t slot) {
    open.erase(slot);
    auto lp = last_prop.find(slot);
    if (lp != last_prop.end()) needed.push_back(lp->second);
  };
  auto kill = [&](int32_t slot) {
    auto it = open.find(slot);
    if (it == open.end()) return;
    const Open &o = it->second;
    if (o.pstage >= 0) L.dead_proposal[o.pstage][o.pidx] = 1;
    else L.dead_product[o.stage][o.idx] = 1;
    open.erase(it);
  };
  for (int s = 0; s < p->n_user_stages; s++) {
    const nbp_stage &st = p->stages[s];
    if (st.kind == NBP_STAGE_PROPOSALS) L.dead_proposal[s].assign(st.n, 0);
    if (st.kind == NBP_STAGE_PRODUCTS) L.dead_product[s].assign(st.n, 0);
    if (!p->lazy_bw) continue;
    if (st.kind == NBP_STAGE_COPIES && st.n == 0) {
      open.clear();
      for (auto &lp : last_prop) needed.push_back(lp.second);
    }
    if (st.kind != NBP_STAGE_DECONV)
      stage_reads(p, st, [&](int, int32_t slot, nbp_access a) {
        if (a == NBP_RD_KDE) read_kde(slot);
        else if (a == NBP_RD_CARRY) open.erase(slot);
      });
    stage_writes(p, st, [&](int i, int32_t slot) {
      kill(slot);
      if (st.kind == NBP_STAGE_PROPOSALS) { last_prop[slot] = {s, i}; return; }
      if (st.kind == NBP_STAGE_PRODUCTS) {
        const nbp_product_desc &q = ((const nbp_product_desc *)(p->blob.data() + st.offset))[i];
        if (q.nfactors > 1) {
          open[slot] = {s, i, -1, -1};
        } else {
          auto lp = last_prop.find(q.in_slot[0]);
          if (lp != last_prop.end() && !((const nbp_proposal_desc *)(p->blob.data() + p->stages[lp->second.first].offset))[lp->second.second].skip_bandwidth)
            open[slot] = {s, i, lp->second.first, lp->second.second};
        }
      }
      last_prop.erase(slot);
    });
  }
  for (auto &nd : needed) L.dead_proposal[nd.first][nd.second] = 0;
  return L;
}

static bool fused_plan(const nbp_program *p, int s, std::vector<nbp_update_desc> &upd, int &Fmax) {
  const nbp_ctx *c = p->ctx;
  if (!c->fused_on || !p->use_fused || s + 1 >= p->n_user_stages || c->Npad > 256) return false;
  const nbp_stage &A = p->stages[s], &B = p->stages[s + 1];
  if (A.kind != NBP_STAGE_PROPOSALS || B.kind != NBP_STAGE_PRODUCTS || B.n < c->fused_min || A.n < B.n) return false;
  if ((A.mani & (NBP_CLS_SIMPLE - 1)) != NBP_CLS_LIN2) return false;
  const int M = NBP_EUCLID2;
  const nbp_proposal_desc *pd = (const nbp_proposal_desc *)(p->blob.data() + A.offset);
  const nbp_product_desc *qd = (const nbp_product_desc *)(p->blob.data() + B.offset);
  std::unordered_map<int32_t, int> prop_of, prod_of;
  for (int i = 0; i < A.n; i++) {
    if (pd[i].manifold != M) return false;
    if (!prop_of.emplace(pd[i].out_slot, i).second) return false;
  }
  for (int i = 0; i < B.n; i++) {
    if (qd[i].manifold != M || qd[i].nfactors > NBP_FUSED_MAXF || qd[i].labels_out >= 0 || qd[i].old_slot >= 0) return false;
    if (!prod_of.emplace(qd[i].out_slot, i).second) return false;
  }
  upd.assign(B.n, nbp_update_desc{});
  std::vector<char> used(A.n, 0);
  int nused = 0;
  Fmax = 2;
  for (int i = 0; i < B.n; i++) {
    nbp_update_desc &u = upd[i];
    u.prod = i;
    if (qd[i].nfactors > Fmax) Fmax = qd[i].nfactors;
    for (int j = 0; j < qd[i].nfactors; j++) {
      if (qd[i].in_partial[j]) return false;
      auto it = prop_of.find(qd[i].in_slot[j]);
      if (it == prop_of.end() || used[it->second]) return false;
      const nbp_proposal_desc &q = pd[it->second];
      if (qd[i].nfactors > 1 && q.skip_bandwidth && q.factor_kind != NBP_F_PASSTHROUGH) return false;
      if (q.factor_kind == NBP_F_PASSTHROUGH && qd[i].nfactors == 1 && q.keep_count) return false;
      used[it->second] = 1;
      nused++;
      u.prop[j] = it->second;
      bool clash = false;
      proposal_reads(q, [&](int32_t r, nbp_access) {
        auto w = prod_of.find(r);
        clash |= (w != prod_of.end() && w->second != i) || prop_of.count(r);
      });
      if (clash) return false;
    }
  }
  if (nused != A.n) return false;
  std::unordered_map<int32_t, std::pair<int, int>> watch;
  for (int i = 0; i < B.n; i++)
    for (int j = 0; j < qd[i].nfactors; j++) watch[qd[i].in_slot[j]] = {i, j};
  for (int i = 0; i < B.n; i++) watch.erase(qd[i].out_slot);
  for (int t = s + 2; t < p->n_user_stages && !watch.empty(); t++) {
    const nbp_stage &st = p->stages[t];
    if ((st.kind == NBP_STAGE_COPIES || st.kind == NBP_STAGE_COPY_POINTS) && st.n == 0) break;
    stage_reads(p, st, [&](int, int32_t slot, nbp_access) {
      auto it = watch.find(slot);
      if (it == watch.end()) return;
      upd[it->second.first].flags |= 2 << it->second.second;
      watch.erase(it);
    }, true);
    stage_writes(p, st, [&](int, int32_t slot) { watch.erase(slot); });
  }
  for (auto &w : watch) upd[w.second.first].flags |= 2 << w.second.second;
  return true;
}

static nbp_status launch_update(nbp_ctx *c, const nbp_stage &st, const nbp_update_desc *uds, const nbp_proposal_desc *props,
                                const nbp_product_desc *prods, int n) {
  nbp_status rc = tic(c, c->ev[4]);
  if (rc) return rc;
  (void)hipGetLastError();
  const int P = n >= c->fused_p1_min ? 1 : 2;
  const size_t lds = nbp_update_lds_bytes(st.upd_F, 2, c->N, c->Npad, P, false);
  hipLaunchKernelGGL(P == 1 ? nbp_update_kernel_lin2_p1 : nbp_update_kernel_lin2_p2, dim3(n), dim3(P * c->Npad), lds, c->stream, uds, props, prods,
                     c->arena, c->N, c->Npad, c->S, c->side, c->T, c->counters, st.upd_F);
  HIPCHK(hipGetLastError());
  return toc(c, c->ev[4]);
}

static void plan_lanes(nbp_program *p) {
  if (p->ctx->no_lanes) return;
  for (int s = 0; s < p->n_user_stages; s++) {
    nbp_stage &st = p->stages[(size_t)s];
    if (st.lane_hint.empty()) continue;
    const size_t esz = st.kind == NBP_STAGE_PROPOSALS ? sizeof(nbp_proposal_desc) : (st.kind == NBP_STAGE_PRODUCTS ? sizeof(nbp_product_desc) :
                       (st.kind == NBP_STAGE_COPY_POINTS ? sizeof(nbp_copy_desc) : 0));
    if (!esz) continue;
    int n1 = 0;
    for (int32_t l : st.lane_hint) n1 += l;
    if (!n1) continue;
    std::vector<char> moved((size_t)st.n * esz);
    st.moved_to.assign((size_t)st.n, 0);
    int at = 0;
    for (int l = 0; l < 2; l++)
      for (int i = 0; i < st.n; i++)
        if (st.lane_hint[(size_t)i] == l) {
          st.moved_to[(size_t)i] = at;
          memcpy(moved.data() + (size_t)at++ * esz, p->blob.data() + st.offset + (size_t)i * esz, esz);
        }
    memcpy(p->blob.data() + st.offset, moved.data(), moved.size());
    st.lane_split = st.n - n1;
  }
}

static void plan_pipeline(nbp_program *p, int s) {
  nbp_stage &ps = p->stages[s], &qs = p->stages[s + 1];
  if (ps.kind != NBP_STAGE_PROPOSALS || qs.kind != NBP_STAGE_PRODUCTS || qs.n < p->ctx->pipe_min || qs.n < 128) return;
  if (ps.lane_split >= 0 || qs.lane_split >= 0) return;
  nbp_proposal_desc *pd = (nbp_proposal_desc *)(p->blob.data() + ps.offset);
  nbp_product_desc *qd = (nbp_product_desc *)(p->blob.data() + qs.offset);
  std::unordered_map<int32_t, int> prop_of, prod_of, reader_of;
  for (int i = 0; i < ps.n; i++) prop_of[pd[i].out_slot] = i;
  for (int i = 0; i < qs.n; i++) prod_of[qd[i].out_slot] = i;
  std::vector<int> uf(qs.n), owner(ps.n, -1);
  for (int i = 0; i < qs.n; i++) uf[i] = i;
  auto find = [&](int a) { while (uf[a] != a) a = uf[a] = uf[uf[a]]; return a; };
  auto unite = [&](int a, int b) { a = find(a); b = find(b); if (a != b) uf[a] = b; };
  for (int i = 0; i < qs.n; i++) {
    if (qd[i].old_slot >= 0) return;
    for (int j = 0; j < qd[i].nfactors; j++) {
      auto rd = reader_of.find(qd[i].in_slot[j]);
      if (rd == reader_of.end()) reader_of[qd[i].in_slot[j]] = i; else unite(rd->second, i);
      auto it = prop_of.find(qd[i].in_slot[j]);
      if (it != prop_of.end() && owner[it->second] < 0) owner[it->second] = i;
    }
  }
  stage_reads(p, ps, [&](int k, int32_t slot, nbp_access) {
    if (owner[k] < 0) return;
    auto it = prod_of.find(slot);
    if (it != prod_of.end()) unite(owner[k], it->second);
  });
  std::unordered_map<int, std::pair<int, std::vector<int>>> comp;
  for (int i = 0; i < qs.n; i++) { auto &c = comp[find(i)]; c.first += qd[i].nfactors; c.second.push_back(i); }
  std::vector<std::pair<int, std::vector<int>>> cs;
  for (auto &kv : comp) cs.push_back(std::move(kv.second));
  std::sort(cs.begin(), cs.end(), [](const auto &a, const auto &b) { return a.first != b.first ? a.first > b.first : a.second[0] < b.second[0]; });
  std::vector<char> half(qs.n, 0);
  int w[2] = {0, 0}, cnt[2] = {0, 0};
  for (auto &c : cs) {
    const int h = w[1] < w[0] ? 1 : 0;
    w[h] += c.first;
    for (int i : c.second) { half[i] = (char)h; cnt[h]++; }
  }
  if (cnt[0] < qs.n / 3 || cnt[1] < qs.n / 3) return;
  std::vector<nbp_product_desc> q2;
  qs.moved_to.assign((size_t)qs.n, 0);
  for (int h = 0; h < 2; h++)
    for (int i = 0; i < qs.n; i++) if (half[i] == h) { qs.moved_to[(size_t)i] = (int)q2.size(); q2.push_back(qd[i]); }
  std::vector<nbp_proposal_desc> p2;
  ps.moved_to.assign((size_t)ps.n, 0);
  int np0 = 0;
  for (int h = 0; h < 2; h++)
    for (int k = 0; k < ps.n; k++) {
      const int hk = owner[k] < 0 ? 0 : half[owner[k]];
      if (hk == h) { ps.moved_to[(size_t)k] = (int)p2.size(); p2.push_back(pd[k]); np0 += h == 0; }
    }
  memcpy(qd, q2.data(), q2.size() * sizeof(nbp_product_desc));
  memcpy(pd, p2.data(), p2.size() * sizeof(nbp_proposal_desc));
  ps.pipe_split = np0;
  qs.pipe_split = cnt[0];
}

static void schedule_fused_pair(nbp_program *p, int s, std::vector<nbp_update_desc> &upd, int Fmax, const nbp_liveness &live, nbp_fits &pend) {
  nbp_stage &st = p->stages[s], &nx = p->stages[s + 1];
  const nbp_proposal_desc *pd = (const nbp_proposal_desc *)(p->blob.data() + st.offset);
  const nbp_product_desc *qd = (const nbp_product_desc *)(p->blob.data() + nx.offset);
  nx.split_out.clear();
  for (int i = 0; i < nx.n; i++) {
    const int k = upd[i].prop[0];
    if (wants_fit(qd[i]) ? live.dead_product[s + 1][i] : (!wants_fit(pd[k]) || live.dead_proposal[s][k])) continue;
    upd[i].flags |= NBP_UPD_FIT_OUT;
    nx.split_out.push(qd[i].out_slot, qd[i].manifold);
  }
  nx.ent.clear();
  queue_fits(nx.ent, pd, st.n);
  nx.fused_second = true;
  nx.need_prep = false;
  st.fused = true;
  st.upd = std::move(upd);
  st.upd_F = Fmax;
  st.flush_before = !pend.empty();
  pend.clear();
}

static void schedule_fits(nbp_program *p, const nbp_liveness &live) {
  nbp_fits pend;
  for (int s = 0; s < (int)p->stages.size(); s++) {
    nbp_stage &st = p->stages[s];
    if (st.fused_second) continue;
    const char *d = p->blob.data() + st.offset;
    st.ent = pend;
    auto flush_if_read = [&](nbp_access what) {
      stage_reads(p, st, [&](int, int32_t slot, nbp_access a) { st.flush_before |= a == what && pend.has(slot); });
      if (st.flush_before) pend.clear();
    };
    if (st.kind == NBP_STAGE_PROPOSALS) {
      std::vector<nbp_update_desc> upd;
      int Fm = 0;
      if (s + 1 < p->n_user_stages && fused_plan(p, s, upd, Fm) && nbp_update_lds_bytes(Fm, 2, p->ctx->N, p->ctx->Npad, 2, false) <= 158 * 1024) {
        schedule_fused_pair(p, s, upd, Fm, live, pend);
        continue;
      }
      flush_if_read(NBP_RD_KDE);
      queue_fits(pend, (const nbp_proposal_desc *)d, st.n, live.dead_proposal[s].data());
    } else if (st.kind == NBP_STAGE_PRODUCTS) {
      const nbp_product_desc *qd = (const nbp_product_desc *)d;
      st.need_prep = false;
      for (int i = 0; i < st.n; i++) st.need_prep |= qd[i].nfactors > 1;
      flush_if_read(NBP_RD_POINTS);
      if (st.need_prep) {
        pend.clear();
      } else {
        for (int i = 0; i < st.n; i++) pend.rename(qd[i].in_slot[0], qd[i].out_slot);
        pend.dedup();
      }
      queue_fits(pend, qd, st.n, live.dead_product[s].data());
    } else if (st.kind == NBP_STAGE_DECONV || st.kind == NBP_STAGE_COPY_POINTS) {
      stage_writes(p, st, [&](int, int32_t slot) { pend.drop(slot); });
      st.ent = pend;
      if (st.kind == NBP_STAGE_DECONV)
        for (int i = 0; i < st.n; i++) pend.push(((const nbp_proposal_desc *)d)[i].out_slot, ((const nbp_proposal_desc *)d)[i].manifold);
    } else {
      st.flush_before = true;
      pend.clear();
    }
  }
}

static void split_piped_entry_fits(nbp_program *p) {
  for (int s = 0; s + 1 < p->n_user_stages; s++) {
    nbp_stage &ps = p->stages[s], &qs = p->stages[s + 1];
    if (ps.kind != NBP_STAGE_PROPOSALS || qs.kind != NBP_STAGE_PRODUCTS || ps.pipe_split < 0 || qs.pipe_split < 0) continue;
    if (ps.fused || !qs.need_prep || qs.flush_before) continue;
    nbp_launch_env round = ctx_env(p->ctx);
    round.geom_n = qs.n;
    if (product_plan(p->ctx, round, qs.n, qs.maxfd, qs.mani).big) continue;
    const nbp_product_desc *qd = (const nbp_product_desc *)(p->blob.data() + qs.offset);
    std::unordered_map<int32_t, int> second;
    for (int i = qs.pipe_split; i < qs.n; i++)
      for (int j = 0; j < qd[i].nfactors; j++) second[qd[i].in_slot[j]] = 1;
    nbp_fits ent;
    for (int h = 0; h < 2; h++)
      for (const nbp_fits::fit &f : qs.ent.v)
        if ((int)second.count(f.slot) == h) { ent.push(f.slot, f.mani); if (!h) qs.pipe_ent++; }
    qs.ent = ent;
    ps.pipe = true;
  }
}

#define NBP_LANE_SLOT_SIDE (-2)
static void plan_parts(nbp_program *p, const nbp_liveness &live) {
  bool any = false;
  for (int s = 0; s < p->n_user_stages; s++) {
    const nbp_stage &st = p->stages[(size_t)s];
    if (st.lane_split < 0) continue;
    if (st.fused || st.fused_second) return;
    any = true;
  }
  if (!any) return;
  std::vector<nbp_stage> &parts = p->parts;
  std::vector<const char *> dead;
  p->first_part.assign((size_t)p->n_user_stages + 1, 0);
  for (int s = 0; s < p->n_user_stages; s++) {
    const nbp_stage &st = p->stages[(size_t)s];
    p->first_part[(size_t)s] = (int)parts.size();
    const size_t esz = st.kind == NBP_STAGE_PRODUCTS ? sizeof(nbp_product_desc) : (st.kind == NBP_STAGE_COPIES || st.kind == NBP_STAGE_COPY_POINTS ?
                       sizeof(nbp_copy_desc) : sizeof(nbp_proposal_desc));
    const int cut = st.lane_split < 0 ? st.n : st.lane_split;
    for (int l = 0; l < 2; l++) {
      const int from = l ? cut : 0, n = l ? st.n - cut : cut;
      if (n == 0 && (l || st.lane_split >= 0)) continue;
      nbp_stage pt;
      pt.kind = st.kind; pt.n = n; pt.offset = st.offset + (size_t)from * esz; pt.lane = l; pt.user = s;
      pt.maxfd = st.maxfd; pt.mani = st.mani;
      if (st.kind == NBP_STAGE_PRODUCTS && st.lane_split >= 0) {
        pt.maxfd = products_maxfd((const nbp_product_desc *)(p->blob.data() + pt.offset), n);
        pt.mani = products_uniform_manifold((const nbp_product_desc *)(p->blob.data() + pt.offset), n);
      }
      if (st.kind == NBP_STAGE_PROPOSALS && st.lane_split >= 0) pt.mani = proposals_uniform_class((const nbp_proposal_desc *)(p->blob.data() + pt.offset), n);
      const std::vector<char> &row = st.kind == NBP_STAGE_PRODUCTS ? live.dead_product[(size_t)s] : live.dead_proposal[(size_t)s];
      dead.push_back(row.empty() ? nullptr : row.data() + from);
      parts.push_back(std::move(pt));
    }
  }
  p->first_part[(size_t)p->n_user_stages] = (int)parts.size();
  {
    nbp_stage pt;
    pt.user = p->n_user_stages;
    dead.push_back(nullptr);
    parts.push_back(std::move(pt));
  }
  nbp_fits pend[2];
  std::vector<nbp_fits> ran(parts.size());
  for (int k = 0; k < (int)parts.size(); k++) {
    nbp_stage &st = parts[(size_t)k];
    const int l = st.lane, o = 1 - l;
    const char *d = p->blob.data() + st.offset;
    if (k == p->first_part[(size_t)st.user]) {
      st.bound = pend[0];
      for (const nbp_fits::fit &f : pend[1].v) st.bound.push(f.slot, f.mani);
    }
    if (st.kind == NBP_STAGE_DECONV || st.kind == NBP_STAGE_COPY_POINTS)
      stage_writes(p, st, [&](int, int32_t slot) { pend[0].drop(slot); pend[1].drop(slot); });
    if (!pend[o].empty()) {
      auto claim = [&](int32_t slot) {
        for (size_t i = 0; i < pend[o].v.size();)
          if (pend[o].v[i].slot == slot) { pend[l].v.push_back(pend[o].v[i]); pend[o].v.erase(pend[o].v.begin() + (long)i); } else i++;
      };
      stage_reads(p, st, [&](int, int32_t slot, nbp_access a) { if (a != NBP_RD_POINTS || st.kind == NBP_STAGE_PRODUCTS) claim(slot); });
      if (st.kind == NBP_STAGE_PROPOSALS || st.kind == NBP_STAGE_PRODUCTS) stage_writes(p, st, [&](int, int32_t slot) { claim(slot); });
      if (st.kind == NBP_STAGE_COPIES || st.kind == 0) {
        for (const nbp_fits::fit &f : pend[o].v) pend[l].v.push_back(f);
        pend[o].clear();
      }
    }
    st.ent = pend[l];
    auto flush_if_read = [&](nbp_access what) {
      stage_reads(p, st, [&](int, int32_t slot, nbp_access a) { st.flush_before |= a == what && pend[l].has(slot); });
      if (st.flush_before) { for (const nbp_fits::fit &f : pend[l].v) ran[(size_t)k].push(f.slot, f.mani); pend[l].clear(); }
    };
    if (st.kind == NBP_STAGE_PROPOSALS) {
      flush_if_read(NBP_RD_KDE);
      queue_fits(pend[l], (const nbp_proposal_desc *)d, st.n, dead[(size_t)k]);
    } else if (st.kind == NBP_STAGE_PRODUCTS) {
      const nbp_product_desc *qd = (const nbp_product_desc *)d;
      st.need_prep = false;
      for (int i = 0; i < st.n; i++) st.need_prep |= qd[i].nfactors > 1;
      flush_if_read(NBP_RD_POINTS);
      if (st.need_prep) {
        for (const nbp_fits::fit &f : pend[l].v) ran[(size_t)k].push(f.slot, f.mani);
        pend[l].clear();
      } else {
        for (int i = 0; i < st.n; i++) pend[l].rename(qd[i].in_slot[0], qd[i].out_slot);
        pend[l].dedup();
      }
      queue_fits(pend[l], qd, st.n, dead[(size_t)k]);
    } else if (st.kind == NBP_STAGE_DECONV || st.kind == NBP_STAGE_COPY_POINTS) {
      if (st.kind == NBP_STAGE_DECONV)
        for (int i = 0; i < st.n; i++) pend[l].push(((const nbp_proposal_desc *)d)[i].out_slot, ((const nbp_proposal_desc *)d)[i].manifold);
    } else {
      st.flush_before = true;
      for (const nbp_fits::fit &f : pend[l].v) ran[(size_t)k].push(f.slot, f.mani);
      pend[l].clear();
    }
  }
  std::vector<nbp_lane_part> sw(parts.size());
  for (int k = 0; k < (int)parts.size(); k++) {
    const nbp_stage &st = parts[(size_t)k];
    nbp_lane_part &a = sw[(size_t)k];
    a.stage = st.user;
    a.lane = st.lane;
    a.barrier = st.kind == 0 || ((st.kind == NBP_STAGE_COPIES || st.kind == NBP_STAGE_COPY_POINTS) && st.n == 0);
    stage_reads(p, st, [&](int, int32_t slot, nbp_access acc) {
      a.reads.push_back(2 * slot);
      if (acc != NBP_RD_POINTS || st.kind == NBP_STAGE_PRODUCTS) a.reads.push_back(2 * slot + 1);
      if (acc == NBP_RD_POINTS && st.kind == NBP_STAGE_PRODUCTS) a.writes.push_back(2 * slot);
    }, true);
    stage_writes(p, st, [&](int, int32_t slot) {
      a.writes.push_back(2 * slot);
      if (st.kind != NBP_STAGE_COPY_POINTS) a.writes.push_back(2 * slot + 1);
    });
    for (const nbp_fits::fit &f : ran[(size_t)k].v) { a.reads.push_back(2 * f.slot); a.writes.push_back(2 * f.slot + 1); }
    const char *d = p->blob.data() + st.offset;
    for (int i = 0; i < st.n; i++)
      if (st.kind == NBP_STAGE_PROPOSALS || st.kind == NBP_STAGE_DECONV) {
        const nbp_proposal_desc &q = ((const nbp_proposal_desc *)d)[i];
        if (q.mhidx_in >= 0) a.reads.push_back(NBP_LANE_SLOT_SIDE);
        if (q.mhidx_out >= 0) a.writes.push_back(NBP_LANE_SLOT_SIDE);
      } else if (st.kind == NBP_STAGE_PRODUCTS && ((const nbp_product_desc *)d)[i].labels_out >= 0) {
        a.writes.push_back(NBP_LANE_SLOT_SIDE);
      }
  }
  nbp_lane_sweep(sw);
  for (int k = 0; k < (int)parts.size(); k++) {
    parts[(size_t)k].waits = sw[(size_t)k].waits;
    parts[(size_t)k].signals = sw[(size_t)k].signals;
  }
  for (const nbp_stage &st : parts)
    if (st.lane == 1 && st.kind == NBP_STAGE_PRODUCTS && st.n > 0) {
      p->lane_ws = std::max(p->lane_ws, (size_t)st.n * (size_t)(st.maxfd / 4) * nbp_kd_ws_doubles(p->ctx->N));
      nbp_launch_env env = ctx_env(p->ctx);
      p->lane_gstats = std::max(p->lane_gstats, std::max(product_plan(p->ctx, env, st.n, st.maxfd, st.mani).gstats, product_plan(p->ctx, env, st.n, st.maxfd, -1).gstats));
    }
}

static void layout_blob(nbp_program *p) {
  for (nbp_stage &st : p->stages) append_fits(p->blob, st.ent);
  for (nbp_stage &st : p->stages)
    if (st.fused_second) append_fits(p->blob, st.split_out, 4);
  for (nbp_stage &st : p->parts) {
    append_fits(p->blob, st.ent);
    append_fits(p->blob, st.bound);
  }
  for (nbp_stage &st : p->stages)
    if (st.fused) {
      st.upd_off = (p->blob.size() + 63) & ~(size_t)63;
      p->blob.resize(st.upd_off + st.upd.size() * sizeof(nbp_update_desc));
      memcpy(p->blob.data() + st.upd_off, st.upd.data(), st.upd.size() * sizeof(nbp_update_desc));
    }
  std::vector<int64_t> so;
  for (int s = 0; s < p->n_user_stages; s++) {
    const nbp_stage &st = p->stages[s];
    if (st.kind == NBP_STAGE_PROPOSALS || st.kind == NBP_STAGE_DECONV)
      for (int i = 0; i < st.n; i++) {
        const size_t o = st.offset + (size_t)(st.moved_to.empty() ? i : st.moved_to[(size_t)i]) * sizeof(nbp_proposal_desc);
        so.push_back((int64_t)(o + offsetof(nbp_proposal_desc, seed)));
        if (((const nbp_proposal_desc *)(p->blob.data() + o))->meas_seed) so.push_back((int64_t)(o + offsetof(nbp_proposal_desc, meas_seed)));
      }
    else if (st.kind == NBP_STAGE_PRODUCTS)
      for (int i = 0; i < st.n; i++)
        so.push_back((int64_t)(st.offset + (size_t)(st.moved_to.empty() ? i : st.moved_to[(size_t)i]) * sizeof(nbp_product_desc) + offsetof(nbp_product_desc, seed)));
  }
  std::vector<int64_t> sorted(so);
  std::sort(sorted.begin(), sorted.end());
  p->seed_rank.resize(so.size());
  for (size_t i = 0; i < so.size(); i++) p->seed_rank[i] = (int32_t)(std::lower_bound(sorted.begin(), sorted.end(), so[i]) - sorted.begin());
  p->seed_off = (p->blob.size() + 63) & ~(size_t)63;
  p->n_seeds = (int)so.size();
  p->seed_val_off = p->seed_off + so.size() * 8;
  p->blob.resize(p->seed_val_off + so.size() * 8);
  if (!so.empty()) memcpy(p->blob.data() + p->seed_off, so.data(), so.size() * 8);
}

static nbp_status presize(nbp_program *p) {
  for (const nbp_stage &st : p->stages)
    if (st.kind == NBP_STAGE_PRODUCTS && st.n > 0 && !st.fused_second) {
      nbp_status rc = presize_products(p->ctx, st.n, st.maxfd, st.mani);
      if (rc) return rc;
    }
  if (p->parts.empty()) return NBP_OK;
  nbp_ctx *c = p->ctx;
  size_t nsig = 0;
  for (const nbp_stage &st : p->parts) nsig += st.signals ? 1 : 0;
  while (c->lane_ev.size() < nsig) {
    hipEvent_t e = nullptr;
    HIPCHK(hipEventCreateWithFlags(&e, hipEventDisableTiming));
    c->lane_ev.push_back(e);
  }
  size_t main = 0;
  for (const nbp_stage &st : p->parts)
    if (st.lane == 0 && st.kind == NBP_STAGE_PRODUCTS) main = std::max(main, (size_t)st.n * (size_t)(st.maxfd / 4) * nbp_kd_ws_doubles(c->N));
  if (main + p->lane_ws > c->ws_doubles) {
    HIPCHK(hipStreamSynchronize(c->stream));
    HIPCHK(hipStreamSynchronize(c->stream2));
    if (c->ws) HIPCHK(hipFree(c->ws));
    c->ws = nullptr;
    c->ws_doubles = 0;
    c->ws_gen++;
    const size_t grown = main + p->lane_ws + (main + p->lane_ws) / 4;
    HIPCHK(hipMalloc(&c->ws, grown * 8));
    c->ws_doubles = grown;
  }
  if (p->lane_gstats > c->gstats1_doubles) {
    HIPCHK(hipStreamSynchronize(c->stream2));
    if (c->gstats1) HIPCHK(hipFree(c->gstats1));
    c->gstats1 = nullptr;
    c->ws_gen++;
    c->gstats1_doubles = p->lane_gstats + p->lane_gstats / 4;
    HIPCHK(hipMalloc(&c->gstats1, c->gstats1_doubles * 8));
  }
  return NBP_OK;
}

static nbp_status acquire_device_blob(nbp_program *p) {
  const size_t bytes = p->blob.size() ? p->blob.size() : 64;
  auto &bc = p->ctx->blob_cache;
  int best = -1;
  for (size_t i = 0; i < bc.size(); i++)
    if (bc[i].second >= bytes && (best < 0 || bc[i].second < bc[(size_t)best].second)) best = (int)i;
  if (best >= 0) {
    p->dev = bc[(size_t)best].first;
    p->dev_bytes = bc[(size_t)best].second;
    bc.erase(bc.begin() + best);
    return NBP_OK;
  }
  p->dev_bytes = bytes < 65536 ? 65536 : bytes;
  HIPCHK(hipMalloc(&p->dev, p->dev_bytes));
  return NBP_OK;
}

static nbp_status upload_blob(nbp_program *p) {
  if (p->blob.empty()) return NBP_OK;
  if (p->async_upload) {
    nbp_ctx::pin_buf *b = pin_acquire(p->ctx, p->blob.size());
    if (!b) return fail(NBP_ERR_HIP, "pinned staging buffer");
    memcpy(b->p, p->blob.data(), p->blob.size());
    const hipError_t e = hipMemcpyAsync(p->dev, b->p, p->blob.size(), hipMemcpyHostToDevice, p->ctx->stream);
    pin_release_behind_stream(p->ctx, b);
    if (e != hipSuccess) return fail(NBP_ERR_HIP, std::string("hipMemcpyAsync (descriptors): ") + hipGetErrorString(e));
    return NBP_OK;
  }
  if (!p->ctx->retired.empty()) HIPCHK(hipStreamSynchronize(p->ctx->stream));
  HIPCHK(hipMemcpy(p->dev, p->blob.data(), p->blob.size(), hipMemcpyHostToDevice));
  return NBP_OK;
}

nbp_status nbp_program_finalize(nbp_program *p) {
  if (!p) return fail(NBP_ERR_ARG, "null argument");
  PROG_ALIVE(p);
  if (p->finalized) return NBP_OK;
  HIPCHK(hipSetDevice(p->ctx->device));
  p->n_user_stages = (int)p->stages.size();
  p->stages.emplace_back();
  plan_lanes(p);
  for (int s = 0; s + 1 < p->n_user_stages; s++) plan_pipeline(p, s);
  const nbp_liveness live = product_liveness(p);
  schedule_fits(p, live);
  split_piped_entry_fits(p);
  plan_parts(p, live);
  layout_blob(p);
  nbp_status rc = presize(p);
  if (!rc) rc = acquire_device_blob(p);
  if (!rc) rc = upload_blob(p);
  if (rc) return rc;
  p->finalized = true;
  return NBP_OK;
}

static bool lanes_apply(const nbp_program *p, int first, int last) {
  if (p->parts.empty() || p->ctx->timing || first >= last) return false;
  auto has1 = [&](int s) { return s >= 0 && s < p->n_user_stages && p->stages[(size_t)s].lane_split >= 0; };
  if ((has1(first - 1) && has1(first)) || (has1(last - 1) && has1(last))) return false;
  for (int s = first; s < last; s++)
    if (has1(s)) return true;
  return false;
}
static nbp_status run_lanes(nbp_program *p, int first, int last) {
  nbp_ctx *c = p->ctx;
  if (p->lane_ws > c->ws_doubles) return fail(NBP_ERR_RANGE, "KD workspace smaller than lane 1's share (sized at nbp_program_finalize)");
  nbp_launch_env env[2] = {ctx_env(c), ctx_env(c)};
  env[0].lane = 1;
  env[0].ws_doubles = c->ws_doubles - p->lane_ws;
  env[1].lane = 2;
  env[1].stream = c->stream2;
  env[1].ws = c->ws + env[0].ws_doubles;
  env[1].ws_doubles = p->lane_ws;
  const int k0 = p->first_part[(size_t)first], k1 = p->first_part[(size_t)last];
  std::vector<hipEvent_t> ev((size_t)(k1 - k0), nullptr);
  size_t nev = 0;
  std::vector<char> issued((size_t)(k1 - k0), 0);
#define LANECHK(expr) do { hipError_t e_ = (expr); if (e_ != hipSuccess) return fail(NBP_ERR_HIP, std::string("lanes: " #expr ": ") + hipGetErrorString(e_)); } while (0)
  LANECHK(hipEventRecord(c->lane_fork, c->stream));
  LANECHK(hipStreamWaitEvent(c->stream2, c->lane_fork, 0));
  int nx[2] = {k0, k0};
  auto seek = [&](int l) { while (nx[l] < k1 && p->parts[(size_t)nx[l]].lane != l) nx[l]++; };
  auto ready = [&](int k) {
    for (int w : p->parts[(size_t)k].waits)
      if (w >= k0 && !issued[(size_t)(w - k0)]) return false;
    return true;
  };
  for (;;) {
    seek(0);
    seek(1);
    if (nx[0] >= k1 && nx[1] >= k1) break;
    const int l = nx[1] < k1 && (ready(nx[1]) || nx[0] >= k1) ? 1 : 0;
    const int k = nx[l]++;
    issued[(size_t)(k - k0)] = 1;
    const nbp_stage &st = p->parts[(size_t)k];
    nbp_launch_env &e = env[st.lane];
    for (int w : st.waits)
      if (w >= k0) {
        LANECHK(hipStreamWaitEvent(e.stream, ev[(size_t)(w - k0)], 0));
        c->lane_waits++;
      }
    int launches = 0;
    nbp_status rc = NBP_OK;
    if (st.flush_before && st.ent.size()) { rc = launch_bandwidth(c, e, fits_dev(st.ent, p->dev)); launches++; }
    if (rc) return rc;
    if (st.kind == NBP_STAGE_PROPOSALS) {
      rc = launch_proposals(c, e, (const nbp_proposal_desc *)(p->dev + st.offset), st.n, st.mani);
      launches += st.n > 0;
    } else if (st.kind == NBP_STAGE_PRODUCTS) {
      const nbp_product_desc *dd = (const nbp_product_desc *)(p->dev + st.offset);
      if (st.need_prep) { rc = launch_prep(c, e, fits_dev(st.ent, p->dev), dd, st.n, st.maxfd, st.mani); launches++; }
      if (!rc) rc = launch_products(c, e, dd, st.n, st.maxfd, st.mani);
      launches += st.n > 0;
      if (st.lane) c->lane_side_updates += st.n;
    } else if (st.kind == NBP_STAGE_DECONV) {
      rc = launch_deconv(c, (const nbp_proposal_desc *)(p->dev + st.offset), nullptr, st.n);
    } else {
      rc = launch_copies(c, (const nbp_copy_desc *)(p->dev + st.offset), st.n, st.kind == NBP_STAGE_COPY_POINTS, e.stream);
      launches += st.n > 0;
    }
    if (rc) return rc;
    if (st.lane) c->lane_side_launches += launches;
    if (st.signals) {
      if (nev >= c->lane_ev.size()) return fail(NBP_ERR_RANGE, "lanes: fewer events than signalling parts (sized at nbp_program_finalize)");
      ev[(size_t)(k - k0)] = c->lane_ev[nev++];
      LANECHK(hipEventRecord(ev[(size_t)(k - k0)], e.stream));
    }
  }
  LANECHK(hipEventRecord(c->lane_join, c->stream2));
  LANECHK(hipStreamWaitEvent(c->stream, c->lane_join, 0));
#undef LANECHK
  return launch_bandwidth(c, ctx_env(c), fits_dev(p->parts[(size_t)k1].bound, p->dev));
}

static nbp_status run_range(nbp_program *p, int first, int last) {
  if (lanes_apply(p, first, last)) return run_lanes(p, first, last);
  nbp_ctx *c = p->ctx;
  nbp_launch_env env = ctx_env(c);
  for (int s = first; s < last; s++) {
    const nbp_stage &st = p->stages[s];
    nbp_status rc = NBP_OK;
    if (st.flush_before) rc = launch_bandwidth(c, env, fits_dev(st.ent, p->dev));
    if (rc) return rc;
    if (st.kind == NBP_STAGE_PROPOSALS && st.fused && s + 1 >= last) {
      rc = launch_proposals(c, env, (const nbp_proposal_desc *)(p->dev + st.offset), st.n, st.mani);
    } else if (st.kind == NBP_STAGE_PROPOSALS && st.fused) {
      const nbp_stage &nx = p->stages[s + 1];
      rc = launch_update(c, st, (const nbp_update_desc *)(p->dev + st.upd_off), (const nbp_proposal_desc *)(p->dev + st.offset),
                         (const nbp_product_desc *)(p->dev + nx.offset), nx.n);
      s++;
    } else if (st.kind == NBP_STAGE_PROPOSALS && st.pipe && !c->timing && s + 1 < last) {
      const nbp_stage &nx = p->stages[s + 1];
      const nbp_proposal_desc *pd = (const nbp_proposal_desc *)(p->dev + st.offset);
      const nbp_product_desc *dd = (const nbp_product_desc *)(p->dev + nx.offset);
      const int ne = nx.ent.size(), ea = nx.pipe_ent, qa = nx.pipe_split, pa = st.pipe_split;
      const size_t wsa = (size_t)qa * (size_t)(nx.maxfd / 4) * nbp_kd_ws_doubles(c->N);
      nbp_launch_env h[2] = {env, env};
      h[0].geom_n = h[1].geom_n = nx.n;
      h[0].geom_blocks = h[1].geom_blocks = 2 * ne + 2 * nx.n;
      h[1].stream = c->stream2;
      h[1].ws = env.ws + wsa;
      h[1].ws_doubles = env.ws_doubles - wsa;
      auto half = [&](int k) -> nbp_status {
        const nbp_product_desc *dh = dd + (k ? qa : 0);
        const int nq = k ? nx.n - qa : qa;
        nbp_status r = launch_prep(c, h[k], fits_dev(nx.ent, p->dev, k ? ea : 0, k ? ne - ea : ea), dh, nq, nx.maxfd, nx.mani);
        if (!r) r = launch_products(c, h[k], dh, nq, nx.maxfd, nx.mani);
        return r;
      };
      rc = launch_proposals(c, h[0], pd, pa, st.mani);
      hipError_t he = hipSuccess;
      if (!rc) he = hipEventRecord(c->pipe_ev[0], env.stream);
      if (!rc && he == hipSuccess) he = hipStreamWaitEvent(c->stream2, c->pipe_ev[0], 0);
      if (!rc && he == hipSuccess) {
        rc = launch_proposals(c, h[1], pd + pa, st.n - pa, st.mani);
        if (!rc) rc = half(1);
        if (!rc) he = hipEventRecord(c->pipe_ev[1], c->stream2);
      }
      if (!rc && he == hipSuccess) rc = half(0);
      if (!rc && he == hipSuccess) he = hipStreamWaitEvent(env.stream, c->pipe_ev[1], 0);
      if (he != hipSuccess) return fail(NBP_ERR_HIP, std::string("two-stream round: ") + hipGetErrorString(he));
      s++;
    } else if (st.kind == NBP_STAGE_PROPOSALS) {
      rc = launch_proposals(c, env, (const nbp_proposal_desc *)(p->dev + st.offset), st.n, st.mani);
    } else if (st.kind == NBP_STAGE_PRODUCTS) {
      const nbp_product_desc *dd = (const nbp_product_desc *)(p->dev + st.offset);
      if (st.need_prep || st.fused_second) rc = launch_prep(c, env, fits_dev(st.ent, p->dev), dd, st.n, st.maxfd, st.mani);
      if (!rc) rc = launch_products(c, env, dd, st.n, st.maxfd, st.mani);
      if (!rc && st.fused_second) rc = launch_bandwidth(c, env, fits_dev(st.split_out, p->dev));
    } else if (st.kind == NBP_STAGE_DECONV) {
      rc = launch_deconv(c, (const nbp_proposal_desc *)(p->dev + st.offset), nullptr, st.n);
    } else {
      rc = launch_copies(c, (const nbp_copy_desc *)(p->dev + st.offset), st.n, st.kind == NBP_STAGE_COPY_POINTS);
    }
    if (rc) return rc;
  }
  return launch_bandwidth(c, env, fits_dev(p->stages[last].ent, p->dev));
}

nbp_status nbp_program_run(nbp_program *p, int32_t first, int32_t last) {
  if (!p) return fail(NBP_ERR_ARG, "null argument");
  PROG_ALIVE(p);
  if (!p->finalized) return fail(NBP_ERR_ARG, "program not finalized");
  nbp_ctx *c = p->ctx;
  HIPCHK(hipSetDevice(c->device));
  const int nuser = p->n_user_stages;
  if (last < 0 || last > nuser) last = nuser;
  if (first < 0) first = 0;
  if (c->timing || !p->use_graph || last - first < 4) return run_range(p, first, last);
  const uint64_t key = ((uint64_t)(uint32_t)first << 32) | (uint32_t)last;
  auto it = p->graphs.find(key);
  if (it != p->graphs.end() && it->second.ws_gen != c->ws_gen) {
    HIPCHK(hipStreamSynchronize(c->stream));
    hipGraphExecDestroy(it->second.exec);
    p->graphs.erase(it);
    it = p->graphs.end();
  }
  if (it == p->graphs.end() && p->runs[key]++ == 0) return run_range(p, first, last);
  if (it == p->graphs.end()) {
    hipGraph_t g = nullptr;
    hipGraphExec_t ge = nullptr;
    HIPCHK(hipStreamBeginCapture(c->stream, hipStreamCaptureModeRelaxed));
    nbp_status rc = run_range(p, first, last);
    hipError_t e = hipStreamEndCapture(c->stream, &g);
    if (rc) { if (g) hipGraphDestroy(g); return rc; }
    if (e != hipSuccess || !g) {
      (void)hipGetLastError();
      p->use_graph = false;
      return run_range(p, first, last);
    }
    e = hipGraphInstantiate(&ge, g, nullptr, nullptr, 0);
    hipGraphDestroy(g);
    if (e != hipSuccess) {
      (void)hipGetLastError();
      p->use_graph = false;
      return run_range(p, first, last);
    }
    it = p->graphs.emplace(key, nbp_program::captured{ge, c->ws_gen}).first;
  }
  HIPCHK(hipGraphLaunch(it->second.exec, c->stream));
  return NBP_OK;
}

nbp_status nbp_program_reseed(nbp_program *p, uint64_t salt) {
  if (!p || !p->finalized) return fail(NBP_ERR_ARG, "program not finalized");
  PROG_ALIVE(p);
  nbp_ctx *c = p->ctx;
  HIPCHK(hipSetDevice(c->device));
  (void)hipGetLastError();
  if (p->n_seeds > 0)
    hipLaunchKernelGGL(nbp_reseed_kernel, dim3((p->n_seeds + 255) / 256), dim3(256), 0, c->stream, p->dev,
                       (const int64_t *)(p->dev + p->seed_off), p->n_seeds, salt);
  HIPCHK(hipGetLastError());
  return NBP_OK;
}

__global__ void nbp_setseed_kernel(char *blob, const int64_t *seed_off, const uint64_t *vals, int n) {
  const int i = blockIdx.x * blockDim.x + threadIdx.x;
  if (i < n) *(uint64_t *)(blob + seed_off[i]) = vals[i];
}
nbp_status nbp_program_num_seeds(nbp_program *p, int32_t *out) {
  if (!p || !out) return fail(NBP_ERR_ARG, "null argument");
  if (!p->finalized) return fail(NBP_ERR_ARG, "program not finalized");
  *out = p->n_seeds;
  return NBP_OK;
}
nbp_status nbp_program_set_seeds(nbp_program *p, const uint64_t *seeds, int32_t n) {
  if (!p || !p->finalized) return fail(NBP_ERR_ARG, "program not finalized");
  PROG_ALIVE(p);
  if (n != p->n_seeds || (n > 0 && !seeds)) return fail(NBP_ERR_ARG, "set_seeds: the count is not the program's (nbp_program_num_seeds)");
  if (n == 0) return NBP_OK;
  nbp_ctx *c = p->ctx;
  HIPCHK(hipSetDevice(c->device));
  nbp_ctx::pin_buf *b = pin_acquire(c, (size_t)n * 8);
  if (!b) return fail(NBP_ERR_HIP, "pinned staging buffer");
  memcpy(b->p, seeds, (size_t)n * 8);
  const hipError_t e = hipMemcpyAsync(p->dev + p->seed_val_off, b->p, (size_t)n * 8, hipMemcpyHostToDevice, c->stream);
  pin_release_behind_stream(c, b);
  if (e != hipSuccess) return fail(NBP_ERR_HIP, std::string("hipMemcpyAsync (seeds): ") + hipGetErrorString(e));
  (void)hipGetLastError();
  hipLaunchKernelGGL(nbp_setseed_kernel, dim3((n + 255) / 256), dim3(256), 0, c->stream, p->dev, (const int64_t *)(p->dev + p->seed_off),
                     (const uint64_t *)(p->dev + p->seed_val_off), n);
  HIPCHK(hipGetLastError());
  return NBP_OK;
}

nbp_status nbp_program_seed_order(nbp_program *p, int32_t *order, int32_t n) {
  if (!p || !p->finalized) return fail(NBP_ERR_ARG, "program not finalized");
  if (n != p->n_seeds || (n > 0 && !order)) return fail(NBP_ERR_ARG, "seed_order: the count is not the program's (nbp_program_num_seeds)");
  if (n > 0) memcpy(order, p->seed_rank.data(), (size_t)n * sizeof(int32_t));
  return NBP_OK;
}

nbp_status nbp_program_num_stages(nbp_program *p, int32_t *out) {
  if (!p || !out) return fail(NBP_ERR_ARG, "null argument");
  *out = p->finalized ? p->n_user_stages : (int32_t)p->stages.size();
  return NBP_OK;
}

nbp_status nbp_program_num_fused(nbp_program *p, int32_t *out) {
  if (!p || !out) return fail(NBP_ERR_ARG, "null argument");
  int n = 0;
  for (const nbp_stage &st : p->stages) n += st.fused ? 1 : 0;
  *out = n;
  return NBP_OK;
}

nbp_status nbp_program_num_two_stream(nbp_program *p, int32_t *out) {
  if (!p || !out) return fail(NBP_ERR_ARG, "null argument");
  int n = 0;
  for (const nbp_stage &st : p->stages) n += st.pipe ? 1 : 0;
  *out = n;
  return NBP_OK;
}

nbp_status nbp_program_lane_plan(nbp_program *p, nbp_lane_part_rec *out, int32_t cap, int32_t *n_out) {
  if (!p || !n_out || (!out && cap > 0)) return fail(NBP_ERR_ARG, "null argument");
  if (!p->finalized) return fail(NBP_ERR_ARG, "program not finalized");
  const int np = p->parts.empty() ? 0 : (int)p->parts.size() - 1;
  *n_out = np;
  for (int k = 0; k < np && k < cap; k++) {
    const nbp_stage &st = p->parts[(size_t)k];
    const nbp_stage &us = p->stages[(size_t)st.user];
    const size_t esz = st.kind == NBP_STAGE_PRODUCTS ? sizeof(nbp_product_desc) : (st.kind == NBP_STAGE_COPIES || st.kind == NBP_STAGE_COPY_POINTS ?
                       sizeof(nbp_copy_desc) : sizeof(nbp_proposal_desc));
    out[k] = {st.user, st.lane, (int32_t)((st.offset - us.offset) / esz), st.n, st.waits.empty() ? -1 : st.waits[0], st.signals ? 1 : 0};
  }
  return NBP_OK;
}

static void program_free(nbp_program *p, bool sync);
static void reap_retired(nbp_ctx *c) {
  for (size_t i = 0; i < c->retired.size();) {
    if (hipEventQuery(c->retired[i].second) == hipSuccess) {
      hipEventDestroy(c->retired[i].second);
      nbp_program *p = c->retired[i].first;
      c->retired.erase(c->retired.begin() + (long)i);
      program_free(p, false);
    } else
      i++;
  }
}
nbp_status nbp_program_retire(nbp_program *p) {
  if (!p) return NBP_OK;
  if (!p->ctx) { delete p; return NBP_OK; }
  nbp_ctx *c = p->ctx;
  hipSetDevice(c->device);
  reap_retired(c);
  hipEvent_t ev = nullptr;
  if (hipEventCreateWithFlags(&ev, hipEventDisableTiming) != hipSuccess || hipEventRecord(ev, c->stream) != hipSuccess) {
    if (ev) hipEventDestroy(ev);
    return nbp_program_destroy(p);
  }
  c->retired.emplace_back(p, ev);
  return NBP_OK;
}
nbp_status nbp_program_destroy(nbp_program *p) {
  if (!p) return NBP_OK;
  program_free(p, true);
  return NBP_OK;
}
static void program_free(nbp_program *p, bool sync) {
  if (p->ctx) {
    hipSetDevice(p->ctx->device);
    if (sync) hipStreamSynchronize(p->ctx->stream);
    if (p->dev) {
      auto &bc = p->ctx->blob_cache;
      if (p->dev_bytes <= (16u << 20) && bc.size() < 64) bc.emplace_back(p->dev, p->dev_bytes);
      else hipFree(p->dev);
    }
    for (auto &kv : p->graphs) hipGraphExecDestroy(kv.second.exec);
    auto &v = p->ctx->programs;
    for (size_t i = 0; i < v.size(); i++)
      if (v[i] == p) { v.erase(v.begin() + i); break; }
  }
  delete p;
}

struct rccl_api {
  void *h = nullptr;
  decltype(&ncclGetUniqueId) GetUniqueId = nullptr;
  decltype(&ncclCommInitRank) CommInitRank = nullptr;
  decltype(&ncclCommDestroy) CommDestroy = nullptr;
  decltype(&ncclCommCount) CommCount = nullptr;
  decltype(&ncclCommUserRank) CommUserRank = nullptr;
  decltype(&ncclGroupStart) GroupStart = nullptr;
  decltype(&ncclGroupEnd) GroupEnd = nullptr;
  decltype(&ncclSend) Send = nullptr;
  decltype(&ncclRecv) Recv = nullptr;
  decltype(&ncclGetErrorString) GetErrorString = nullptr;
};
static rccl_api g_rccl;
static nbp_status rccl_load() {
  if (g_rccl.Send) return NBP_OK;
  const char *env = getenv("NBP_RCCL_LIB");
  const char *names[] = {env, "librccl.so", "librccl.so.1"};
  void *h = nullptr;
  for (const char *n : names)
    if (n && !h) h = dlopen(n, RTLD_NOW | RTLD_NOLOAD);
  for (const char *n : names)
    if (n && !h) h = dlopen(n, RTLD_NOW | RTLD_GLOBAL);
  if (!h) return fail(NBP_ERR_HIP, std::string("RCCL not found (librccl.so): ") + (dlerror() ? dlerror() : ""));
  g_rccl.h = h;
#define NBP_RCCL_SYM(F) g_rccl.F = (decltype(g_rccl.F))dlsym(h, "nccl" #F); if (!g_rccl.F) return fail(NBP_ERR_HIP, "RCCL: missing symbol nccl" #F)
  NBP_RCCL_SYM(GetUniqueId);
  NBP_RCCL_SYM(CommInitRank);
  NBP_RCCL_SYM(CommDestroy);
  NBP_RCCL_SYM(CommCount);
  NBP_RCCL_SYM(CommUserRank);
  NBP_RCCL_SYM(GroupStart);
// ... 196 lines not shown
      return fail(NBP_ERR_ARG, "plan query: request " + std::to_string(i) + ": out of range");
    nbp_launch_env env;
    env.geom_n = q.geom_n;
    if (q.mani > 0 && manifold_dim_h(q.mani) != q.D) {
      out[i] = nbp_product_plan_rec{};
      out[i].status = NBP_ERR_ARG;
      out[i].row = -1;
      out[i].N = q.N; out[i].n = q.n; out[i].F = q.F; out[i].D = q.D; out[i].mani = q.mani; out[i].geom_n = q.geom_n;
      continue;
    }
    out[i] = product_plan_rec(&c, env, q.n, q.F * 4 + q.D, q.mani, product_plan(&c, env, q.n, q.F * 4 + q.D, q.mani));
  }
  return NBP_OK;
}
nbp_status nbp_plan_fits(const nbp_fit_plan_req *req, nbp_fit_plan_rec *out, int64_t n) {
  if ((!req || !out) && n > 0) return fail(NBP_ERR_ARG, "null argument");
  nbp_ctx c;
  for (int64_t i = 0; i < n; i++) {
    const nbp_fit_plan_req &q = req[i];
    if (c.N != q.N) {
      c = nbp_ctx();
      NBPCHK(plan_ctx(c, q.N));
    }
    if (q.fits < 0 || q.coords < 0 || q.products < 0 || q.kdF < 0 || q.geom_blocks < 0 || (q.fits == 0 && q.products == 0))
      return fail(NBP_ERR_ARG, "plan query: request " + std::to_string(i) + ": out of range");
    nbp_launch_env env;
    env.geom_blocks = q.geom_blocks;
    env.geom_n = q.geom_blocks ? std::max(q.products, 1) : 0;
    const bool prep = q.products > 0;
    out[i] = fit_plan_rec(&c, env, q.fits, q.coords, q.products, q.kdF, prep, fit_plan(&c, env, q.fits, q.coords, q.products, q.kdF));
  }
  return NBP_OK;
}
nbp_status nbp_plan_proposals(const nbp_proposal_plan_req *req, nbp_proposal_plan_rec *out, int64_t n) {
  if ((!req || !out) && n > 0) return fail(NBP_ERR_ARG, "null argument");
  nbp_ctx c;
  for (int64_t i = 0; i < n; i++) {
    const nbp_proposal_plan_req &q = req[i];
    if (c.N != q.N) {
      c = nbp_ctx();
      NBPCHK(plan_ctx(c, q.N));
    }
    if (q.n < 1 || q.manifold < 0 || q.manifold > NBP_SE2) return fail(NBP_ERR_ARG, "plan query: request " + std::to_string(i) + ": out of range");
    const int M = q.manifold;
    const int cls = M == NBP_EUCLID2 ? NBP_CLS_LIN2 : (M == NBP_EUCLID3 ? NBP_CLS_LIN3 : (M == NBP_CIRCULAR ? NBP_CLS_CIRC : (M == NBP_SE2 ? NBP_CLS_SE2 : 0)));
    const nbp_proposal_plan p = proposal_plan(&c, q.n, cls | ((cls && q.simple) ? NBP_CLS_SIMPLE : 0));
    nbp_proposal_plan_rec r{};
    r.status = NBP_OK;
    r.geometry = p.geometry; r.blocks = p.blocks; r.threads = p.threads;
    r.N = q.N; r.n = q.n; r.manifold = q.manifold; r.simple = q.simple;
    r.lds = (int64_t)p.lds;
    snprintf(r.kernel, sizeof(r.kernel), "%s", p.name);
    out[i] = r;
  }
  return NBP_OK;
}
nbp_status nbp_last_plans(nbp_ctx *c, nbp_product_plan_rec *product, nbp_fit_plan_rec *prep, nbp_fit_plan_rec *fits) {
  if (!c) return fail(NBP_ERR_ARG, "ctx is null");
  if (product) *product = c->last_product;
  if (prep) *prep = c->last_prep;
  if (fits) *fits = c->last_fit;
  return NBP_OK;
}

nbp_status nbp_diag_read(nbp_ctx *c, nbp_diag *out, int32_t reset) {
  if (!c || !out) return fail(NBP_ERR_ARG, "null argument");
  nbp_counters h;
  HIPCHK(hipStreamSynchronize(c->stream));
  HIPCHK(hipMemcpy(&h, c->counters, sizeof(h), hipMemcpyDeviceToHost));
  out->solves = (int64_t)h.solves;
  out->nonconverged = (int64_t)h.nonconverged;
  out->nan_results = (int64_t)h.nan_results;
  out->residual_evals = (int64_t)h.residual_evals;
  out->lcv_evals = (int64_t)h.lcv_evals;
  out->lcv_evals_f32 = (int64_t)h.lcv_evals_f32;
  out->proposal_launches_workgroup = c->prop_launches[0];
  out->proposal_launches_wave = c->prop_launches[1];
  out->proposal_launches_split = c->prop_launches[2];
  if (reset) c->prop_launches[0] = c->prop_launches[1] = c->prop_launches[2] = 0;
  out->lane_side_launches = c->lane_side_launches;
  out->lane_waits = c->lane_waits;
  out->lane_side_updates = c->lane_side_updates;
  if (reset) c->lane_side_launches = c->lane_waits = c->lane_side_updates = 0;
  if (reset) HIPCHK(hipMemset(c->counters, 0, offsetof(nbp_counters, flags)));
  return NBP_OK;
}

#ifdef NBP_PHASE_TIMING
nbp_status nbp_debug_phase_read(long long *out, int n, int reset) {
  long long h[64];
  HIPCHK(hipDeviceSynchronize());
  HIPCHK(hipMemcpyFromSymbol(h, HIP_SYMBOL(nbp_phase_clk), sizeof(h)));
  for (int i = 0; i < n && i < 64; i++) out[i] = h[i];
  if (reset) {
    memset(h, 0, sizeof(h));
    HIPCHK(hipMemcpyToSymbol(HIP_SYMBOL(nbp_phase_clk), h, sizeof(h)));
  }
  return NBP_OK;
}
nbp_status nbp_debug_block_read(long long *out, int nblocks) {
  HIPCHK(hipDeviceSynchronize());
  HIPCHK(hipMemcpyFromSymbol(out, HIP_SYMBOL(nbp_block_clk), sizeof(long long) * 3 * (size_t)(nblocks < 8192 ? nblocks : 8192)));
  return NBP_OK;
}
nbp_status nbp_debug_block_hist(unsigned int *out, int reset) {
  HIPCHK(hipDeviceSynchronize());
  HIPCHK(hipMemcpyFromSymbol(out, HIP_SYMBOL(nbp_block_hist), sizeof(unsigned int) * 4 * 64));
  if (reset) {
    unsigned int z[4 * 64] = {0};
    HIPCHK(hipMemcpyToSymbol(HIP_SYMBOL(nbp_block_hist), z, sizeof(z)));
  }
  return NBP_OK;
}
#endif

}
```

incrementalinference.jl_amd/csrc/nbp_host.cpp:

```cpp
#include <algorithm>
#include <atomic>
#include <chrono>
#include <array>
#include <deque>
#include <cstdio>
#include <cstdlib>
#include <cstring>
#include <map>
#include <set>
#include <string>
#include <condition_variable>
#include <functional>
#include <mutex>
#include <thread>
#include <vector>

#include "../../include/nbp_host.h"

extern "C" nbp_status nbp_internal_fail(nbp_status code, const char *msg);
static nbp_status hfail(nbp_status c, const char *m) { return nbp_internal_fail(c, m); }

namespace {

struct HVar { int manifold; bool initialized, ismargin; };
// ... 1320 lines not shown
        if (nbp_status rc = batch(true, tt, start, finish, side)) return rc;
      }
    }
    add_stage(t->stages, NBP_STAGE_COPIES, final_cps.data(), sizeof(nbp_copy_desc), (int)final_cps.size());
  }
  t->segments.push_back({0, t->seg_start, (int)t->stages.size(), {}, {}});
  t->st.stages = (int64_t)t->stages.size();
  for (const Stage &s : t->stages) {
    if (s.kind == NBP_STAGE_PROPOSALS) t->st.proposals += s.n;
    if (s.kind == NBP_STAGE_PRODUCTS) t->st.products += s.n;
  }
  int64_t edges = 0;
  for (const Clique &c : t->cl) edges += c.parent != 0;
  t->st.messages = ((g->sp.upsolve ? 1 : 0) + (g->sp.downsolve ? 1 : 0)) * edges;
  t->st.slots = t->n_slots;
  for (Clique &c : t->cl)
    if (c.status != NBP_CLIQ_MARGINALIZED) c.status = g->sp.downsolve ? NBP_CLIQ_DOWNSOLVED : NBP_CLIQ_UPSOLVED;
  return NBP_OK;
}

static void clique_set_status(nbp_tree *t, Clique &c, int status, bool allmarginalized, bool reused) {
  c.status = status;
  c.allmarginalized = allmarginalized;
  c.reused = reused;
  t->replan = true;
}
nbp_status nbp_tree_set_clique_status(nbp_tree *t, int32_t k, int32_t status) {
  if (!t || k < 1 || k > (int)t->cl.size()) return hfail(NBP_ERR_RANGE, "clique id");
  if (status < NBP_CLIQ_NULL || status > NBP_CLIQ_ERROR_STATUS) return hfail(NBP_ERR_ARG, "unknown clique status");
  if (!t->main_slot.empty()) return hfail(NBP_ERR_ARG, "clique statuses are set before the slots are planned");
  clique_set_status(t, t->cl[k - 1], status, status == NBP_CLIQ_MARGINALIZED, status == NBP_CLIQ_UPRECYCLED);
  return NBP_OK;
}
nbp_status nbp_tree_clique_status(const nbp_tree *t, int32_t k, int32_t *status, int32_t *allmarginalized, int32_t *reused) {
  if (!t || k < 1 || k > (int)t->cl.size()) return hfail(NBP_ERR_RANGE, "clique id");
  const Clique &c = t->cl[k - 1];
  if (status) *status = c.status;
  if (allmarginalized) *allmarginalized = c.allmarginalized;
  if (reused) *reused = c.reused;
  return NBP_OK;
}
nbp_status nbp_tree_recycle(nbp_tree *t, const nbp_tree *old, int32_t incremental) {
  if (!t) return hfail(NBP_ERR_ARG, "null argument");
  if (!t->main_slot.empty()) return hfail(NBP_ERR_ARG, "clique statuses are set before the slots are planned");
  const nbp_graph *g = t->g;
  auto same_set = [](std::vector<int> a, std::vector<int> b) {
    std::sort(a.begin(), a.end());
    std::sort(b.begin(), b.end());
    return a == b;
  };
  std::vector<int> oldstatus(t->cl.size(), NBP_CLIQ_NULL);
  for (const Clique &c : t->cl) {
    const int f0 = c.frontals[0];
    if (!old || f0 >= (int)old->frontal_of.size() || old->frontal_of[f0] < 1) continue;
    const Clique &cand = old->cl[old->frontal_of[f0] - 1];
    if (same_set(cand.frontals, c.frontals) && same_set(cand.seps, c.seps) && same_set(cand.potentials, c.potentials))
      oldstatus[c.id - 1] = cand.status;
  }
  for (Clique &c : t->cl) {
    bool allmarg = true;
    for (int v : c.all()) allmarg = allmarg && g->vars[v].ismargin && g->vars[v].initialized;
    if (allmarg) clique_set_status(t, c, NBP_CLIQ_MARGINALIZED, true, false);
    else if (incremental && oldstatus[c.id - 1] == NBP_CLIQ_DOWNSOLVED) clique_set_status(t, c, NBP_CLIQ_UPRECYCLED, false, true);
    else clique_set_status(t, c, NBP_CLIQ_NULL, false, false);
  }
  return NBP_OK;
}
nbp_status nbp_tree_cliques_recycled(const nbp_tree *t, int32_t out[4]) {
  if (!t || !out) return hfail(NBP_ERR_ARG, "null argument");
  out[0] = (int32_t)t->cl.size();
  out[1] = out[2] = out[3] = 0;
  for (const Clique &c : t->cl) {
    out[1] += c.allmarginalized;
    out[2] += c.reused;
    out[3] += c.allmarginalized && c.reused;
  }
  return NBP_OK;
}

nbp_status nbp_tree_compile(nbp_tree *t, nbp_ctx *ctx, uint64_t seed, nbp_program **out) {
  if (!t || !ctx || !out) return hfail(NBP_ERR_ARG, "null argument");
  nbp_status rc = nbp_tree_schedule(t, seed);
  if (rc) return rc;
  return assemble_program(ctx, t->stages, {{NBP_OPT_LAZY_BANDWIDTH, 1}}, out);
}

nbp_status nbp_tree_set_owner(nbp_tree *t, const int32_t *owner, int32_t rank) {
  if (!t) return hfail(NBP_ERR_ARG, "null argument");
  if (!owner) { t->owner.clear(); t->rank = 0; return NBP_OK; }
  if (rank < 0) return hfail(NBP_ERR_ARG, "rank < 0");
  t->owner.assign(owner, owner + t->cl.size());
  for (int o : t->owner)
    if (o < 0) return hfail(NBP_ERR_RANGE, "owner: negative rank");
  t->rank = rank;
  t->main_slot.clear();
  return NBP_OK;
}

nbp_status nbp_tree_partition(const nbp_tree *t, int32_t world, int32_t *owner_out) {
  if (!t || !owner_out || world < 1) return hfail(NBP_ERR_ARG, "bad argument");
  const size_t nc = t->cl.size();
  std::vector<double> w(nc + 1, 0.0), sub(nc + 1, 0.0);
  for (const Clique &c : t->cl) w[c.id] = 1.0 + (double)c.upsched.size();
  for (int cid : postorder(t)) {
    sub[cid] = w[cid];
    for (int chd : t->cl[cid - 1].children) sub[cid] += sub[chd];
  }
  double total = 0;
  for (size_t k = 1; k <= nc; k++) total += w[k];
  std::vector<int> roots(t->roots.begin(), t->roots.end()), top;
  while ((int)roots.size() < 6 * world) {
    int best = -1;
    for (int r : roots)
      if (!t->cl[r - 1].children.empty() && (best < 0 || sub[r] > sub[best])) best = r;
    if (best < 0) break;
    if ((int)roots.size() >= world && sub[best] <= 0.6 * total / world) break;
    roots.erase(std::find(roots.begin(), roots.end(), best));
    top.push_back(best);
    for (int chd : t->cl[best - 1].children) roots.push_back(chd);
  }
  std::vector<int> owner(nc + 1, 0);
  std::vector<double> load(world, 0.0);
  std::stable_sort(roots.begin(), roots.end(), [&](int a, int b) { return sub[a] > sub[b]; });
  for (int r : roots) {
    int k = 0;
    for (int q = 1; q < world; q++)
      if (load[q] < load[k]) k = q;
    load[k] += sub[r];
    std::vector<int> st{r};
    while (!st.empty()) {
      const int c = st.back();
      st.pop_back();
      owner[c] = k;
      for (int chd : t->cl[c - 1].children) st.push_back(chd);
    }
  }
  {
    std::map<int, int> level;
    int maxlevel = 0;
    for (auto it = top.rbegin(); it != top.rend(); ++it) {
      int lv = 0;
      for (int chd : t->cl[*it - 1].children)
        if (level.count(chd)) lv = std::max(lv, level[chd] + 1);
      level[*it] = lv;
      maxlevel = std::max(maxlevel, lv);
    }
    for (int lv = 0; lv <= maxlevel; lv++) {
      std::vector<char> used(world, 0);
      for (auto it = top.rbegin(); it != top.rend(); ++it) {
        if (level[*it] != lv) continue;
        std::vector<int> kids(t->cl[*it - 1].children.begin(), t->cl[*it - 1].children.end());
        std::stable_sort(kids.begin(), kids.end(), [&](int a, int b) { return sub[a] > sub[b]; });
        int pick = owner[kids[0]];
        for (int chd : kids)
          if (!used[owner[chd]]) { pick = owner[chd]; break; }
        owner[*it] = pick;
        used[pick] = 1;
        load[pick] += w[*it];
      }
    }
  }
  for (size_t k = 1; k <= nc; k++) owner_out[k - 1] = owner[k];
  return NBP_OK;
}

nbp_status nbp_tree_run_sharded_cb(const nbp_tree *t, nbp_program *prog, nbp_exchange_fn xchg, void *user) {
  if (!t || !prog) return hfail(NBP_ERR_ARG, "null argument");
// ... 995 lines not shown
```

Baseline: 144,200 messages/s.

## Sink deferrable up-pass product updates into later batched stages

Adds a planner that finds lane-0 proposal/product pairs in the up pass whose outputs are not read until later, and defers them into a shared later stage (the last step, or an earlier pre-wait step). Those descriptors are gathered into a combined launch, with seed duplication so reseeding stays consistent. The aim is to remove many small serial kernel launches along the elimination chain by batching independent clique updates. It adds planning complexity and descriptor gathering, and it is enabled by default for single-owner trees.

```diff
diff --git a/include/nbp.h b/include/nbp.h
--- a/include/nbp.h
+++ b/include/nbp.h
@@ -101,6 +101,8 @@
   int64_t lane_side_launches;
   int64_t lane_waits;
   int64_t lane_side_updates;
+  int64_t sunk_updates;
+  int64_t sink_launches;
 } nbp_diag;
 
 typedef struct nbp_ctx nbp_ctx;
@@ -391,7 +393,8 @@
 nbp_status nbp_program_create(nbp_ctx *ctx, nbp_program **out);
 nbp_status nbp_program_add_stage(nbp_program *prog, int32_t kind, const void *descs, int32_t n);
 enum nbp_program_option { NBP_OPT_LAZY_BANDWIDTH = 1, NBP_OPT_GRAPH_REPLAY = 2, NBP_OPT_FUSED_UPDATES = 3,
-                          NBP_OPT_ASYNC_UPLOAD = 4  };
+                          NBP_OPT_ASYNC_UPLOAD = 4 ,
+                          NBP_OPT_UP_PASS_SINKS = 5  };
 nbp_status nbp_program_set_option(nbp_program *prog, int32_t option, int32_t value);
 nbp_status nbp_program_finalize(nbp_program *prog);
 nbp_status nbp_program_run(nbp_program *prog, int32_t first_stage, int32_t last_stage );
@@ -407,6 +410,7 @@
   int32_t stage, lane, first_desc, n, wait, signals;
 } nbp_lane_part_rec;
 nbp_status nbp_program_lane_plan(nbp_program *prog, nbp_lane_part_rec *out, int32_t cap, int32_t *n_out);
+nbp_status nbp_program_sink_plan(nbp_program *prog, int32_t *gained, int32_t cap, int32_t *n_out);
 nbp_status nbp_program_destroy(nbp_program *prog);
 nbp_status nbp_program_retire(nbp_program *prog);
 
diff --git a/include/nbp_sinks.h b/include/nbp_sinks.h
--- /dev/null
+++ b/include/nbp_sinks.h
@@ -0,0 +1,159 @@
+#ifndef NBP_SINKS_H
+#define NBP_SINKS_H
+#include <cstddef>
+#include <cstdint>
+#include <unordered_map>
+#include <unordered_set>
+#include <vector>
+
+enum { NBP_SINK_OTHER = 0, NBP_SINK_PROPOSALS = 1, NBP_SINK_PRODUCTS = 2 };
+enum { NBP_SINK_TWO = 0, NBP_SINK_LAST = 1 };
+
+struct nbp_sink_desc {
+  int lane = 0;
+  int nfactors = 0;
+  std::vector<int32_t> reads, writes;
+  int to = -1;
+  bool deferrable = false;
+  bool waits_lane1 = false;
+  std::vector<int> props;
+};
+struct nbp_sink_stage {
+  int kind = NBP_SINK_OTHER, pass = -1;
+  std::vector<nbp_sink_desc> d;
+  int gained = 0;
+};
+
+static inline void nbp_sink_plan(std::vector<nbp_sink_stage> &st, int placement = NBP_SINK_TWO) {
+  const int ns = (int)st.size();
+  for (int s = 0; s < ns; s++) {
+    st[(size_t)s].gained = 0;
+    for (nbp_sink_desc &d : st[(size_t)s].d) { d.to = s; d.deferrable = d.waits_lane1 = false; d.props.clear(); }
+  }
+  for (int a = 0; a < ns;) {
+    int b = a;
+    while (b + 1 < ns && st[(size_t)b + 1].pass == st[(size_t)a].pass) b++;
+    const int first = a, last = b;
+    a = b + 1;
+    if (st[(size_t)first].pass < 0) continue;
+    auto is_step = [&](int s) { return s > first && s <= last && st[(size_t)s].kind == NBP_SINK_PRODUCTS && st[(size_t)s - 1].kind == NBP_SINK_PROPOSALS; };
+    std::unordered_map<int32_t, int> nr, nw;
+    auto count = [&](const nbp_sink_stage &g) {
+      for (const nbp_sink_desc &d : g.d) {
+        for (int32_t x : d.reads) nr[x]++;
+        for (int32_t x : d.writes) nw[x]++;
+      }
+    };
+    auto at = [](const std::unordered_map<int32_t, int> &m, int32_t x) { auto it = m.find(x); return it == m.end() ? 0 : it->second; };
+    std::vector<char> lets_go((size_t)ns, 0);
+    for (int s = last; s >= first;) {
+      if (!is_step(s)) { count(st[(size_t)s--]); continue; }
+      nbp_sink_stage &P = st[(size_t)s - 1], &Q = st[(size_t)s];
+      std::vector<char> read_later(Q.d.size(), 0);
+      for (size_t i = 0; i < Q.d.size(); i++)
+        for (int32_t x : Q.d[i].writes) read_later[i] |= at(nr, x) > 0;
+      count(Q);
+      count(P);
+      std::unordered_map<int32_t, int> writer, feeds;
+      for (int k = 0; k < (int)P.d.size(); k++)
+        for (int32_t x : P.d[(size_t)k].writes) { auto r = writer.emplace(x, k); if (!r.second && r.first->second != k) r.first->second = -2; }
+      for (int i = 0; i < (int)Q.d.size(); i++)
+        for (int32_t x : Q.d[(size_t)i].reads) {
+          auto w = writer.find(x);
+          if (w == writer.end() || w->second < 0) continue;
+          auto r = feeds.emplace(w->second, i);
+          if (!r.second && r.first->second != i) r.first->second = -2;
+        }
+      for (int i = 0; i < (int)Q.d.size(); i++) {
+        nbp_sink_desc &q = Q.d[(size_t)i];
+        if (q.lane != 0 || q.nfactors < 2) continue;
+        bool ok = true;
+        std::vector<int> props;
+        for (int32_t x : q.reads) {
+          auto w = writer.find(x);
+          if (w == writer.end()) continue;
+          if (w->second < 0 || feeds[w->second] != i || P.d[(size_t)w->second].lane != 0) { ok = false; break; }
+          bool seen = false;
+          for (int k : props) seen |= k == w->second;
+          if (!seen) props.push_back(w->second);
+        }
+        if (!ok) continue;
+        std::unordered_map<int32_t, int> own_r, own_w;
+        auto own = [&](const nbp_sink_desc &d) {
+          for (int32_t x : d.reads) own_r[x]++;
+          for (int32_t x : d.writes) own_w[x]++;
+        };
+        own(q);
+        for (int k : props) own(P.d[(size_t)k]);
+        for (auto &kv : own_w) ok = ok && at(nw, kv.first) == kv.second && at(nr, kv.first) == at(own_r, kv.first);
+        for (auto &kv : own_r) ok = ok && (own_w.count(kv.first) || at(nw, kv.first) == 0);
+        if (!ok) continue;
+        q.deferrable = true;
+        q.props = props;
+      }
+      bool others = false, plain = true, chain = false;
+      for (size_t i = 0; i < Q.d.size(); i++) {
+        const nbp_sink_desc &q = Q.d[i];
+        if (q.lane != 0 || q.deferrable) continue;
+        others = true;
+        plain = plain && q.nfactors == 1;
+        chain = chain || read_later[i];
+      }
+      lets_go[(size_t)s] = others && plain && chain;
+      s -= 2;
+    }
+    std::unordered_set<int32_t> hot;
+    int first_wait = -1;
+    for (int s = first; s <= last; s++) {
+      nbp_sink_stage &g = st[(size_t)s];
+      for (nbp_sink_desc &d : g.d) {
+        d.waits_lane1 = d.lane != 0;
+        for (int32_t x : d.reads) d.waits_lane1 = d.waits_lane1 || hot.count(x) > 0;
+      }
+      for (const nbp_sink_desc &d : g.d)
+        for (int32_t x : d.writes) { if (d.waits_lane1) hot.insert(x); else hot.erase(x); }
+    }
+    for (int s = first; s <= last && first_wait < 0; s++) {
+      const nbp_sink_stage &g = st[(size_t)s];
+      for (size_t i = 0; i < g.d.size(); i++) {
+        const nbp_sink_desc &d = g.d[i];
+        if (d.lane != 0 || !d.waits_lane1) continue;
+        bool leaves = false;
+        if (g.kind == NBP_SINK_PRODUCTS) leaves = is_step(s) && lets_go[(size_t)s] && d.deferrable;
+        if (g.kind == NBP_SINK_PROPOSALS && is_step(s + 1) && lets_go[(size_t)s + 1])
+          for (const nbp_sink_desc &q : st[(size_t)s + 1].d)
+            if (q.deferrable)
+              for (int k : q.props) leaves = leaves || k == (int)i;
+        if (!leaves) { first_wait = s; break; }
+      }
+    }
+    int sink_last = -1, sink_early = -1;
+    for (int s = last; s >= first && sink_last < 0; s--)
+      if (is_step(s)) sink_last = s;
+    if (sink_last < 0) continue;
+    if (placement == NBP_SINK_TWO && first_wait >= 0) {
+      const int step_start = is_step(first_wait) ? first_wait - 1 : first_wait;
+      for (int s = step_start - 1; s >= first && sink_early < 0; s--)
+        if (is_step(s)) sink_early = s;
+    }
+    for (int s = first; s <= last; s++) {
+      if (!is_step(s) || !lets_go[(size_t)s]) continue;
+      auto target = [&](const nbp_sink_desc &q) {
+        bool waits = q.waits_lane1;
+        for (int k : q.props) waits = waits || st[(size_t)s - 1].d[(size_t)k].waits_lane1;
+        return (sink_early >= s && !waits) ? sink_early : sink_last;
+      };
+      bool keeps = false;
+      for (const nbp_sink_desc &q : st[(size_t)s].d) keeps = keeps || (q.deferrable && target(q) == s);
+      if (keeps) continue;
+      for (nbp_sink_desc &q : st[(size_t)s].d) {
+        if (!q.deferrable) continue;
+        const int to = target(q);
+        q.to = to;
+        st[(size_t)to].gained++;
+        for (int k : q.props) { st[(size_t)s - 1].d[(size_t)k].to = to - 1; st[(size_t)to - 1].gained++; }
+      }
+    }
+  }
+}
+#endif
diff --git a/incrementalinference.jl_amd/abi.py b/incrementalinference.jl_amd/abi.py
--- a/incrementalinference.jl_amd/abi.py
+++ b/incrementalinference.jl_amd/abi.py
@@ -10,6 +10,8 @@
 OPT_LAZY_BANDWIDTH = 1
 OPT_GRAPH_REPLAY = 2
 OPT_FUSED_UPDATES = 3
+OPT_ASYNC_UPLOAD = 4
+OPT_UP_PASS_SINKS = 5
 
 MANIFOLD_DIM = {EUCLID1: 1, EUCLID2: 2, EUCLID3: 3, CIRCULAR: 1, SE2: 3}
 MANIFOLD_P = {EUCLID1: 1, EUCLID2: 2, EUCLID3: 3, CIRCULAR: 1, SE2: 6}
@@ -186,6 +188,8 @@
         ("lane_side_launches", C.c_int64),
         ("lane_waits", C.c_int64),
         ("lane_side_updates", C.c_int64),
+        ("sunk_updates", C.c_int64),
+        ("sink_launches", C.c_int64),
     ]
 
 
@@ -267,7 +271,7 @@
     "nbp_slot_write", "nbp_slot_read", "nbp_belief_write", "nbp_belief_read", "nbp_belief_write_batch", "nbp_belief_read_batch", "nbp_run_resample", "nbp_side_write", "nbp_side_read",
     "nbp_run_proposals", "nbp_run_bandwidth", "nbp_run_ppe", "nbp_kde_ppe", "nbp_run_evaluate", "nbp_kde_evaluate", "nbp_run_marginal_grid", "nbp_kde_marginal_grid", "nbp_run_evaluate_marginal", "nbp_run_mmd", "nbp_kde_mmd", "nbp_run_meancov", "nbp_kde_meancov", "nbp_run_kld", "nbp_kde_kld", "nbp_run_overlap", "nbp_kde_overlap", "nbp_run_overlap_search", "nbp_run_scene_grid", "nbp_run_credible", "nbp_kde_credible", "nbp_run_modes", "nbp_kde_modes", "nbp_run_mixture", "nbp_kde_mixture", "nbp_run_factor_likelihood", "nbp_factor_likelihood", "nbp_run_factor_mode_likelihood", "nbp_factor_mode_likelihood", "nbp_run_product_grid", "nbp_product_grid", "nbp_heatmap_create", "nbp_heatmap_build", "nbp_heatmap_draw", "nbp_heatmap_info", "nbp_heatmap_destroy", "nbp_heatmap_scan_eval", "nbp_heatmap_search_eval", "nbp_run_products", "nbp_run_copies", "nbp_run_deconv", "nbp_kde_bandwidth", "nbp_conv", "nbp_manifold_product",
     "nbp_program_create", "nbp_program_add_stage", "nbp_program_set_option", "nbp_program_finalize", "nbp_program_run",
-    "nbp_program_reseed", "nbp_program_num_seeds", "nbp_program_set_seeds", "nbp_program_seed_order", "nbp_ctx_attach", "nbp_ctx_attached", "nbp_program_num_stages", "nbp_program_num_fused", "nbp_program_num_two_stream", "nbp_program_set_lanes", "nbp_program_lane_plan", "nbp_program_destroy",
+    "nbp_program_reseed", "nbp_program_num_seeds", "nbp_program_set_seeds", "nbp_program_seed_order", "nbp_ctx_attach", "nbp_ctx_attached", "nbp_program_num_stages", "nbp_program_num_fused", "nbp_program_num_two_stream", "nbp_program_set_lanes", "nbp_program_lane_plan", "nbp_program_sink_plan", "nbp_program_destroy",
     "nbp_timing_enable", "nbp_timing_read", "nbp_timing_read_n", "nbp_diag_read",
     "nbp_plan_products", "nbp_plan_fits", "nbp_plan_proposals", "nbp_last_plans",
     "nbp_comm_unique_id", "nbp_comm_create", "nbp_comm_destroy", "nbp_comm_info", "nbp_exchange", "nbp_math_eval",
@@ -389,6 +393,7 @@
     lib.nbp_program_num_two_stream.argtypes = [vp, C.POINTER(i32)]
     lib.nbp_program_set_lanes.argtypes = [vp, i32, ip, i32]
     lib.nbp_program_lane_plan.argtypes = [vp, C.POINTER(LanePartRec), i32, C.POINTER(i32)]
+    lib.nbp_program_sink_plan.argtypes = [vp, C.POINTER(i32), i32, C.POINTER(i32)]
     lib.nbp_diag_read.argtypes = [vp, C.POINTER(Diag), i32]
     lib.nbp_plan_products.argtypes = [C.POINTER(ProductPlanReq), C.POINTER(ProductPlanRec), i64]
     lib.nbp_plan_fits.argtypes = [C.POINTER(FitPlanReq), C.POINTER(FitPlanRec), i64]
diff --git a/incrementalinference.jl_amd/backend.py b/incrementalinference.jl_amd/backend.py
--- a/incrementalinference.jl_amd/backend.py
+++ b/incrementalinference.jl_amd/backend.py
@@ -743,6 +743,13 @@
         self.backend._check(self.backend.lib.nbp_program_lane_plan(self._p, recs, n.value, C.byref(n)))
         return [{k: getattr(r, k) for k, _ in abi.LanePartRec._fields_} for r in recs[:n.value]]
 
+    def sink_plan(self):
+        n = C.c_int32(0)
+        self.backend._check(self.backend.lib.nbp_program_sink_plan(self._p, None, 0, C.byref(n)))
+        arr = (C.c_int32 * max(n.value, 1))()
+        self.backend._check(self.backend.lib.nbp_program_sink_plan(self._p, arr, n.value, C.byref(n)))
+        return list(arr[:n.value])
+
     def num_fused(self):
         n = C.c_int32(0)
         self.backend._check(self.backend.lib.nbp_program_num_fused(self._p, C.byref(n)))
diff --git a/incrementalinference.jl_amd/csrc/nbp_api.hip b/incrementalinference.jl_amd/csrc/nbp_api.hip
--- a/incrementalinference.jl_amd/csrc/nbp_api.hip
+++ b/incrementalinference.jl_amd/csrc/nbp_api.hip
@@ -31,6 +31,7 @@
 #include "nbp_scene.h"
 #include "nbp_productgrid.h"
 #include "../../include/nbp_lanes.h"
+#include "../../include/nbp_sinks.h"
 
 static thread_local std::string g_err;
 static nbp_status fail(nbp_status code, const std::string &msg) {
@@ -123,6 +124,9 @@
   double *gstats1 = nullptr;
   size_t gstats1_doubles = 0;
   int64_t lane_side_launches = 0, lane_waits = 0, lane_side_updates = 0;
+  bool no_sinks = false;
+  int sink_placement = 0;
+  int64_t sunk_updates = 0, sink_launches = 0;
   int lcv_p2_min = 256, lcv_p1_min = 4 * 256;
   bool fit_w5 = true, debug_occupancy = false;
   int prod_hl2_min = 192, prod_nch = 0, prod_all_levels_hl = 8;
@@ -293,6 +297,8 @@
   if (getenv("NBP_PROPOSAL_SPLIT_MIN")) c->prop_split_min = atoi(getenv("NBP_PROPOSAL_SPLIT_MIN"));
   if (getenv("NBP_PIPELINE_MIN")) c->pipe_min = atoi(getenv("NBP_PIPELINE_MIN"));
   c->no_lanes = getenv("NBP_NO_LANES") && atoi(getenv("NBP_NO_LANES")) != 0;
+  c->no_sinks = getenv("NBP_NO_SINKS") && atoi(getenv("NBP_NO_SINKS")) != 0;
+  if (getenv("NBP_SINK_PLACEMENT")) c->sink_placement = atoi(getenv("NBP_SINK_PLACEMENT"));
   if (getenv("NBP_FUSED_P1_MIN")) c->fused_p1_min = atoi(getenv("NBP_FUSED_P1_MIN"));
   if (getenv("NBP_PRODUCT_HL2_MIN")) c->prod_hl2_min = atoi(getenv("NBP_PRODUCT_HL2_MIN"));
   if (getenv("NBP_PRODUCT_NCH")) c->prod_nch = atoi(getenv("NBP_PRODUCT_NCH"));
@@ -2735,6 +2741,12 @@
   std::vector<int> moved_to;
   std::vector<int32_t> lane_hint;
   int lane_split = -1;
+  std::vector<int> sink_to;
+  int sink_stay = -1;
+  size_t gather_off = 0;
+  int gather_n = 0, gained = 0;
+  std::vector<std::pair<int, int>> gather_src;
+  bool sink_touched = false, gathered = false;
   int lane = 0, user = -1;
   nbp_fits bound;
   std::vector<int> waits;
@@ -2762,6 +2774,11 @@
   std::vector<nbp_stage> parts;
   std::vector<int> first_part;
   size_t lane_ws = 0, lane_gstats = 0;
+  bool sinks = false;
+  bool sunk = false;
+  std::vector<std::pair<int, int>> sink_regions;
+  size_t dup_src_off = 0;
+  int n_dup = 0;
 };
 
 nbp_status nbp_program_create(nbp_ctx *c, nbp_program **out) {
@@ -2840,6 +2857,7 @@
   if (option == NBP_OPT_GRAPH_REPLAY) { p->use_graph = value != 0; return NBP_OK; }
   if (option == NBP_OPT_FUSED_UPDATES) { p->use_fused = value != 0; return NBP_OK; }
   if (option == NBP_OPT_ASYNC_UPLOAD) { p->async_upload = value != 0; return NBP_OK; }
+  if (option == NBP_OPT_UP_PASS_SINKS) { p->sinks = value != 0; return NBP_OK; }
   return fail(NBP_ERR_ARG, "unknown program option");
 }
 
@@ -2876,6 +2894,28 @@
     if (st.kind == NBP_STAGE_PROPOSALS || st.kind == NBP_STAGE_DECONV) f(i, ((const nbp_proposal_desc *)d)[i].out_slot);
     else if (st.kind == NBP_STAGE_PRODUCTS) f(i, ((const nbp_product_desc *)d)[i].out_slot);
     else if (st.kind == NBP_STAGE_COPIES || st.kind == NBP_STAGE_COPY_POINTS) f(i, ((const nbp_copy_desc *)d)[i].dst_slot);
+}
+#define NBP_LANE_SLOT_SIDE (-2)
+template <class R, class W>
+static void stage_touches(const nbp_program *p, const nbp_stage &st, R &&rd, W &&wr) {
+  stage_reads(p, st, [&](int i, int32_t slot, nbp_access acc) {
+    rd(i, 2 * slot);
+    if (acc != NBP_RD_POINTS || st.kind == NBP_STAGE_PRODUCTS) rd(i, 2 * slot + 1);
+    if (acc == NBP_RD_POINTS && st.kind == NBP_STAGE_PRODUCTS) wr(i, 2 * slot);
+  }, true);
+  stage_writes(p, st, [&](int i, int32_t slot) {
+    wr(i, 2 * slot);
+    if (st.kind != NBP_STAGE_COPY_POINTS) wr(i, 2 * slot + 1);
+  });
+  const char *d = p->blob.data() + st.offset;
+  for (int i = 0; i < st.n; i++)
+    if (st.kind == NBP_STAGE_PROPOSALS || st.kind == NBP_STAGE_DECONV) {
+      const nbp_proposal_desc &q = ((const nbp_proposal_desc *)d)[i];
+      if (q.mhidx_in >= 0) rd(i, NBP_LANE_SLOT_SIDE);
+      if (q.mhidx_out >= 0) wr(i, NBP_LANE_SLOT_SIDE);
+    } else if (st.kind == NBP_STAGE_PRODUCTS && ((const nbp_product_desc *)d)[i].labels_out >= 0) {
+      wr(i, NBP_LANE_SLOT_SIDE);
+    }
 }
 }
 
@@ -3014,28 +3054,104 @@
   return toc(c, c->ev[4]);
 }
 
+static size_t lane_desc_bytes(int kind) {
+  return kind == NBP_STAGE_PROPOSALS ? sizeof(nbp_proposal_desc) : (kind == NBP_STAGE_PRODUCTS ? sizeof(nbp_product_desc) :
+         (kind == NBP_STAGE_COPY_POINTS ? sizeof(nbp_copy_desc) : 0));
+}
+static void plan_sinks(nbp_program *p) {
+  if (!p->sinks || p->ctx->no_lanes || p->ctx->no_sinks) return;
+  const int ns = p->n_user_stages;
+  std::vector<nbp_sink_stage> sk((size_t)ns);
+  int first = -1, last = -1;
+  for (int s = 0, from = 0; s <= ns && first < 0; s++) {
+    const bool edge = s == ns || p->stages[(size_t)s].kind == NBP_STAGE_COPIES || (p->stages[(size_t)s].kind == NBP_STAGE_COPY_POINTS && p->stages[(size_t)s].n == 0);
+    if (!edge) continue;
+    for (int t = from; t < s; t++)
+      if (p->stages[(size_t)t].kind == NBP_STAGE_PRODUCTS) { first = from; last = s - 1; break; }
+    from = s + 1;
+  }
+  if (first < 0) return;
+  for (int s = 0; s < ns; s++) {
+    const nbp_stage &st = p->stages[(size_t)s];
+    nbp_sink_stage &g = sk[(size_t)s];
+    g.kind = st.kind == NBP_STAGE_PROPOSALS ? NBP_SINK_PROPOSALS : (st.kind == NBP_STAGE_PRODUCTS ? NBP_SINK_PRODUCTS : NBP_SINK_OTHER);
+    g.pass = s >= first && s <= last ? 0 : -1;
+    g.d.resize((size_t)st.n);
+    for (int i = 0; i < st.n; i++) {
+      g.d[(size_t)i].lane = !st.lane_hint.empty() && lane_desc_bytes(st.kind) ? st.lane_hint[(size_t)i] : 0;
+      if (st.kind == NBP_STAGE_PRODUCTS) g.d[(size_t)i].nfactors = ((const nbp_product_desc *)(p->blob.data() + st.offset))[i].nfactors;
+    }
+    stage_touches(p, st, [&](int i, int32_t x) { g.d[(size_t)i].reads.push_back(x); }, [&](int i, int32_t x) { g.d[(size_t)i].writes.push_back(x); });
+  }
+  nbp_sink_plan(sk, p->ctx->sink_placement == 1 ? NBP_SINK_LAST : NBP_SINK_TWO);
+  for (int s = 0; s < ns; s++) {
+    nbp_stage &st = p->stages[(size_t)s];
+    bool leaves = false;
+    for (const nbp_sink_desc &d : sk[(size_t)s].d) leaves = leaves || d.to != s;
+    if (!leaves) continue;
+    st.sink_to.resize((size_t)st.n);
+    for (int i = 0; i < st.n; i++) st.sink_to[(size_t)i] = sk[(size_t)s].d[(size_t)i].to;
+    st.sink_touched = true;
+    p->sunk = true;
+  }
+}
+
 static void plan_lanes(nbp_program *p) {
   if (p->ctx->no_lanes) return;
   for (int s = 0; s < p->n_user_stages; s++) {
     nbp_stage &st = p->stages[(size_t)s];
-    if (st.lane_hint.empty()) continue;
-    const size_t esz = st.kind == NBP_STAGE_PROPOSALS ? sizeof(nbp_proposal_desc) : (st.kind == NBP_STAGE_PRODUCTS ? sizeof(nbp_product_desc) :
-                       (st.kind == NBP_STAGE_COPY_POINTS ? sizeof(nbp_copy_desc) : 0));
+    if (st.lane_hint.empty() && st.sink_to.empty()) continue;
+    const size_t esz = lane_desc_bytes(st.kind);
     if (!esz) continue;
-    int n1 = 0;
-    for (int32_t l : st.lane_hint) n1 += l;
-    if (!n1) continue;
+    auto place = [&](int i) { return !st.lane_hint.empty() && st.lane_hint[(size_t)i] ? 2 : (!st.sink_to.empty() && st.sink_to[(size_t)i] != s ? 1 : 0); };
+    int cnt[3] = {0, 0, 0};
+    for (int i = 0; i < st.n; i++) cnt[place(i)]++;
+    if (!cnt[1] && !cnt[2]) continue;
     std::vector<char> moved((size_t)st.n * esz);
     st.moved_to.assign((size_t)st.n, 0);
     int at = 0;
-    for (int l = 0; l < 2; l++)
+    for (int l = 0; l < 3; l++)
       for (int i = 0; i < st.n; i++)
-        if (st.lane_hint[(size_t)i] == l) {
+        if (place(i) == l) {
           st.moved_to[(size_t)i] = at;
           memcpy(moved.data() + (size_t)at++ * esz, p->blob.data() + st.offset + (size_t)i * esz, esz);
         }
     memcpy(p->blob.data() + st.offset, moved.data(), moved.size());
-    st.lane_split = st.n - n1;
+    if (cnt[2]) st.lane_split = st.n - cnt[2];
+    if (cnt[1]) st.sink_stay = cnt[0];
+  }
+}
+
+static void gather_sinks(nbp_program *p) {
+  if (!p->sunk) return;
+  const int ns = p->n_user_stages;
+  std::vector<std::vector<std::pair<int, int>>> came((size_t)ns);
+  std::vector<int> from((size_t)ns, -1);
+  for (int s = 0; s < ns; s++) {
+    const nbp_stage &st = p->stages[(size_t)s];
+    for (int i = 0; i < (int)st.sink_to.size(); i++) {
+      const int to = st.sink_to[(size_t)i];
+      if (to == s) continue;
+      came[(size_t)to].push_back({s, st.moved_to[(size_t)i]});
+      if (from[(size_t)to] < 0) from[(size_t)to] = s;
+    }
+  }
+  for (int s = 0; s < ns; s++) {
+    if (came[(size_t)s].empty()) continue;
+    nbp_stage &st = p->stages[(size_t)s];
+    const size_t esz = lane_desc_bytes(st.kind);
+    const int own = st.sink_stay >= 0 ? st.sink_stay : (st.lane_split >= 0 ? st.lane_split : st.n);
+    for (int i = 0; i < own; i++) st.gather_src.push_back({s, i});
+    for (auto &c : came[(size_t)s]) st.gather_src.push_back(c);
+    st.gained = (int)came[(size_t)s].size();
+    st.gather_n = (int)st.gather_src.size();
+    st.gather_off = (p->blob.size() + 63) & ~(size_t)63;
+    st.sink_touched = true;
+    p->blob.resize(st.gather_off + (size_t)st.gather_n * esz);
+    for (int j = 0; j < st.gather_n; j++)
+      memcpy(p->blob.data() + st.gather_off + (size_t)j * esz,
+             p->blob.data() + p->stages[(size_t)st.gather_src[(size_t)j].first].offset + (size_t)st.gather_src[(size_t)j].second * esz, esz);
+    if (st.kind == NBP_STAGE_PRODUCTS) p->sink_regions.push_back({from[(size_t)s] - 1, s});
   }
 }
 
@@ -3043,6 +3159,7 @@
   nbp_stage &ps = p->stages[s], &qs = p->stages[s + 1];
   if (ps.kind != NBP_STAGE_PROPOSALS || qs.kind != NBP_STAGE_PRODUCTS || qs.n < p->ctx->pipe_min || qs.n < 128) return;
   if (ps.lane_split >= 0 || qs.lane_split >= 0) return;
+  if (ps.sink_touched || qs.sink_touched) return;
   nbp_proposal_desc *pd = (nbp_proposal_desc *)(p->blob.data() + ps.offset);
   nbp_product_desc *qd = (nbp_product_desc *)(p->blob.data() + qs.offset);
   std::unordered_map<int32_t, int> prop_of, prod_of, reader_of;
@@ -3184,7 +3301,6 @@
   }
 }
 
-#define NBP_LANE_SLOT_SIDE (-2)
 static void plan_parts(nbp_program *p, const nbp_liveness &live) {
   bool any = false;
   for (int s = 0; s < p->n_user_stages; s++) {
@@ -3193,9 +3309,15 @@
     if (st.fused || st.fused_second) return;
     any = true;
   }
-  if (!any) return;
+  for (int s = 0; s < p->n_user_stages && p->sunk; s++)
+    if (p->stages[(size_t)s].sink_touched && (p->stages[(size_t)s].fused || p->stages[(size_t)s].fused_second)) p->sunk = false;
+  if (!any && !p->sunk) return;
   std::vector<nbp_stage> &parts = p->parts;
   std::vector<const char *> dead;
+  std::vector<std::vector<char>> dead_gathered((size_t)p->n_user_stages);
+  auto dead_row = [&](int s) -> const std::vector<char> & {
+    return p->stages[(size_t)s].kind == NBP_STAGE_PRODUCTS ? live.dead_product[(size_t)s] : live.dead_proposal[(size_t)s];
+  };
   p->first_part.assign((size_t)p->n_user_stages + 1, 0);
   for (int s = 0; s < p->n_user_stages; s++) {
     const nbp_stage &st = p->stages[(size_t)s];
@@ -3204,18 +3326,27 @@
                        sizeof(nbp_copy_desc) : sizeof(nbp_proposal_desc));
     const int cut = st.lane_split < 0 ? st.n : st.lane_split;
     for (int l = 0; l < 2; l++) {
-      const int from = l ? cut : 0, n = l ? st.n - cut : cut;
-      if (n == 0 && (l || st.lane_split >= 0)) continue;
+      const bool gathered = !l && p->sunk && st.gather_n > 0;
+      const int from = l ? cut : 0, n = l ? st.n - cut : (gathered ? st.gather_n : (p->sunk && st.sink_stay >= 0 ? st.sink_stay : cut));
+      if (n == 0 && (l || st.lane_split >= 0 || st.n > 0)) continue;
       nbp_stage pt;
-      pt.kind = st.kind; pt.n = n; pt.offset = st.offset + (size_t)from * esz; pt.lane = l; pt.user = s;
+      pt.kind = st.kind; pt.n = n; pt.offset = gathered ? st.gather_off : st.offset + (size_t)from * esz; pt.lane = l; pt.user = s;
       pt.maxfd = st.maxfd; pt.mani = st.mani;
-      if (st.kind == NBP_STAGE_PRODUCTS && st.lane_split >= 0) {
+      pt.gathered = gathered;
+      pt.gained = gathered ? st.gained : 0;
+      if (st.kind == NBP_STAGE_PRODUCTS && (n != st.n || gathered)) {
         pt.maxfd = products_maxfd((const nbp_product_desc *)(p->blob.data() + pt.offset), n);
         pt.mani = products_uniform_manifold((const nbp_product_desc *)(p->blob.data() + pt.offset), n);
       }
-      if (st.kind == NBP_STAGE_PROPOSALS && st.lane_split >= 0) pt.mani = proposals_uniform_class((const nbp_proposal_desc *)(p->blob.data() + pt.offset), n);
-      const std::vector<char> &row = st.kind == NBP_STAGE_PRODUCTS ? live.dead_product[(size_t)s] : live.dead_proposal[(size_t)s];
-      dead.push_back(row.empty() ? nullptr : row.data() + from);
+      if (st.kind == NBP_STAGE_PROPOSALS && (n != st.n || gathered)) pt.mani = proposals_uniform_class((const nbp_proposal_desc *)(p->blob.data() + pt.offset), n);
+      const std::vector<char> &row = dead_row(s);
+      if (gathered && (st.kind == NBP_STAGE_PRODUCTS || st.kind == NBP_STAGE_PROPOSALS)) {
+        std::vector<char> &g = dead_gathered[(size_t)s];
+        for (const auto &src : st.gather_src) g.push_back(dead_row(src.first)[(size_t)src.second]);
+        dead.push_back(g.data());
+      } else {
+        dead.push_back(row.empty() ? nullptr : row.data() + from);
+      }
       parts.push_back(std::move(pt));
     }
   }
@@ -3287,25 +3418,8 @@
     a.stage = st.user;
     a.lane = st.lane;
     a.barrier = st.kind == 0 || ((st.kind == NBP_STAGE_COPIES || st.kind == NBP_STAGE_COPY_POINTS) && st.n == 0);
-    stage_reads(p, st, [&](int, int32_t slot, nbp_access acc) {
-      a.reads.push_back(2 * slot);
-      if (acc != NBP_RD_POINTS || st.kind == NBP_STAGE_PRODUCTS) a.reads.push_back(2 * slot + 1);
-      if (acc == NBP_RD_POINTS && st.kind == NBP_STAGE_PRODUCTS) a.writes.push_back(2 * slot);
-    }, true);
-    stage_writes(p, st, [&](int, int32_t slot) {
-      a.writes.push_back(2 * slot);
-      if (st.kind != NBP_STAGE_COPY_POINTS) a.writes.push_back(2 * slot + 1);
-    });
+    stage_touches(p, st, [&](int, int32_t x) { a.reads.push_back(x); }, [&](int, int32_t x) { a.writes.push_back(x); });
     for (const nbp_fits::fit &f : ran[(size_t)k].v) { a.reads.push_back(2 * f.slot); a.writes.push_back(2 * f.slot + 1); }
-    const char *d = p->blob.data() + st.offset;
-    for (int i = 0; i < st.n; i++)
-      if (st.kind == NBP_STAGE_PROPOSALS || st.kind == NBP_STAGE_DECONV) {
-        const nbp_proposal_desc &q = ((const nbp_proposal_desc *)d)[i];
-        if (q.mhidx_in >= 0) a.reads.push_back(NBP_LANE_SLOT_SIDE);
-        if (q.mhidx_out >= 0) a.writes.push_back(NBP_LANE_SLOT_SIDE);
-      } else if (st.kind == NBP_STAGE_PRODUCTS && ((const nbp_product_desc *)d)[i].labels_out >= 0) {
-        a.writes.push_back(NBP_LANE_SLOT_SIDE);
-      }
   }
   nbp_lane_sweep(sw);
   for (int k = 0; k < (int)parts.size(); k++) {
@@ -3351,11 +3465,38 @@
   std::sort(sorted.begin(), sorted.end());
   p->seed_rank.resize(so.size());
   for (size_t i = 0; i < so.size(); i++) p->seed_rank[i] = (int32_t)(std::lower_bound(sorted.begin(), sorted.end(), so[i]) - sorted.begin());
+  std::vector<int64_t> dup;
+  std::vector<int32_t> dup_src;
+  if (p->sunk || !p->sink_regions.empty()) {
+    std::unordered_map<int64_t, int32_t> entry;
+    for (size_t i = 0; i < so.size(); i++) entry[so[i]] = (int32_t)i;
+    for (int s = 0; s < p->n_user_stages; s++) {
+      const nbp_stage &st = p->stages[(size_t)s];
+      const size_t esz = st.kind == NBP_STAGE_PRODUCTS ? sizeof(nbp_product_desc) : sizeof(nbp_proposal_desc);
+      for (int j = 0; j < st.gather_n; j++) {
+        const int64_t from = (int64_t)(p->stages[(size_t)st.gather_src[(size_t)j].first].offset + (size_t)st.gather_src[(size_t)j].second * esz);
+        const int64_t to = (int64_t)(st.gather_off + (size_t)j * esz);
+        for (size_t field : {st.kind == NBP_STAGE_PRODUCTS ? offsetof(nbp_product_desc, seed) : offsetof(nbp_proposal_desc, seed),
+                             st.kind == NBP_STAGE_PRODUCTS ? (size_t)0 : offsetof(nbp_proposal_desc, meas_seed)}) {
+          auto it = field ? entry.find(from + (int64_t)field) : entry.end();
+          if (it == entry.end()) continue;
+          dup.push_back(to + (int64_t)field);
+          dup_src.push_back(it->second);
+        }
+      }
+    }
+  }
   p->seed_off = (p->blob.size() + 63) & ~(size_t)63;
   p->n_seeds = (int)so.size();
-  p->seed_val_off = p->seed_off + so.size() * 8;
-  p->blob.resize(p->seed_val_off + so.size() * 8);
+  p->n_dup = (int)dup.size();
+  p->seed_val_off = p->seed_off + (so.size() + dup.size()) * 8;
+  p->dup_src_off = p->seed_val_off + so.size() * 8;
+  p->blob.resize(p->dup_src_off + dup.size() * 4);
   if (!so.empty()) memcpy(p->blob.data() + p->seed_off, so.data(), so.size() * 8);
+  if (!dup.empty()) {
+    memcpy(p->blob.data() + p->seed_off + so.size() * 8, dup.data(), dup.size() * 8);
+    memcpy(p->blob.data() + p->dup_src_off, dup_src.data(), dup.size() * 4);
+  }
 }
 
 static nbp_status presize(nbp_program *p) {
@@ -3365,6 +3506,11 @@
       if (rc) return rc;
     }
   if (p->parts.empty()) return NBP_OK;
+  for (const nbp_stage &st : p->parts)
+    if (st.gathered && st.kind == NBP_STAGE_PRODUCTS) {
+      nbp_status rc = presize_products(p->ctx, st.n, st.maxfd, st.mani);
+      if (rc) return rc;
+    }
   nbp_ctx *c = p->ctx;
   size_t nsig = 0;
   for (const nbp_stage &st : p->parts) nsig += st.signals ? 1 : 0;
@@ -3438,7 +3584,16 @@
   HIPCHK(hipSetDevice(p->ctx->device));
   p->n_user_stages = (int)p->stages.size();
   p->stages.emplace_back();
+  plan_sinks(p);
   plan_lanes(p);
+  gather_sinks(p);
+  for (int s = 0; s < p->n_user_stages; s++) {
+    const nbp_stage &st = p->stages[(size_t)s];
+    if (!st.gather_n) continue;
+    const nbp_status rc = st.kind == NBP_STAGE_PRODUCTS ? check_products(p->ctx, (const nbp_product_desc *)(p->blob.data() + st.gather_off), st.gather_n)
+                                                        : check_proposals(p->ctx, (const nbp_proposal_desc *)(p->blob.data() + st.gather_off), st.gather_n);
+    if (rc) return rc;
+  }
   for (int s = 0; s + 1 < p->n_user_stages; s++) plan_pipeline(p, s);
   const nbp_liveness live = product_liveness(p);
   schedule_fits(p, live);
@@ -3457,6 +3612,14 @@
   if (p->parts.empty() || p->ctx->timing || first >= last) return false;
   auto has1 = [&](int s) { return s >= 0 && s < p->n_user_stages && p->stages[(size_t)s].lane_split >= 0; };
   if ((has1(first - 1) && has1(first)) || (has1(last - 1) && has1(last))) return false;
+  bool sink = false;
+  if (p->sunk)
+    for (const auto &r : p->sink_regions) {
+      auto inside = [&](int cut) { return r.first < cut && cut <= r.second; };
+      if (inside(first) || inside(last)) return false;
+      sink = sink || (first <= r.first && r.second < last);
+    }
+  if (sink) return true;
   for (int s = first; s < last; s++)
     if (has1(s)) return true;
   return false;
@@ -3520,6 +3683,10 @@
     }
     if (rc) return rc;
     if (st.lane) c->lane_side_launches += launches;
+    if (st.gained) {
+      c->sink_launches += launches;
+      if (st.kind == NBP_STAGE_PRODUCTS) c->sunk_updates += st.gained;
+    }
     if (st.signals) {
       if (nev >= c->lane_ev.size()) return fail(NBP_ERR_RANGE, "lanes: fewer events than signalling parts (sized at nbp_program_finalize)");
       ev[(size_t)(k - k0)] = c->lane_ev[nev++];
@@ -3648,15 +3815,15 @@
   HIPCHK(hipSetDevice(c->device));
   (void)hipGetLastError();
   if (p->n_seeds > 0)
-    hipLaunchKernelGGL(nbp_reseed_kernel, dim3((p->n_seeds + 255) / 256), dim3(256), 0, c->stream, p->dev,
-                       (const int64_t *)(p->dev + p->seed_off), p->n_seeds, salt);
+    hipLaunchKernelGGL(nbp_reseed_kernel, dim3((p->n_seeds + p->n_dup + 255) / 256), dim3(256), 0, c->stream, p->dev,
+                       (const int64_t *)(p->dev + p->seed_off), p->n_seeds + p->n_dup, salt);
   HIPCHK(hipGetLastError());
   return NBP_OK;
 }
 
-__global__ void nbp_setseed_kernel(char *blob, const int64_t *seed_off, const uint64_t *vals, int n) {
+__global__ void nbp_setseed_kernel(char *blob, const int64_t *seed_off, const uint64_t *vals, int n, const int32_t *dup_src, int ndup) {
   const int i = blockIdx.x * blockDim.x + threadIdx.x;
-  if (i < n) *(uint64_t *)(blob + seed_off[i]) = vals[i];
+  if (i < n + ndup) *(uint64_t *)(blob + seed_off[i]) = vals[i < n ? i : dup_src[i - n]];
 }
 nbp_status nbp_program_num_seeds(nbp_program *p, int32_t *out) {
   if (!p || !out) return fail(NBP_ERR_ARG, "null argument");
@@ -3678,8 +3845,8 @@
   pin_release_behind_stream(c, b);
   if (e != hipSuccess) return fail(NBP_ERR_HIP, std::string("hipMemcpyAsync (seeds): ") + hipGetErrorString(e));
   (void)hipGetLastError();
-  hipLaunchKernelGGL(nbp_setseed_kernel, dim3((n + 255) / 256), dim3(256), 0, c->stream, p->dev, (const int64_t *)(p->dev + p->seed_off),
-                     (const uint64_t *)(p->dev + p->seed_val_off), n);
+  hipLaunchKernelGGL(nbp_setseed_kernel, dim3((n + p->n_dup + 255) / 256), dim3(256), 0, c->stream, p->dev, (const int64_t *)(p->dev + p->seed_off),
+                     (const uint64_t *)(p->dev + p->seed_val_off), n, (const int32_t *)(p->dev + p->dup_src_off), p->n_dup);
   HIPCHK(hipGetLastError());
   return NBP_OK;
 }
@@ -3723,8 +3890,17 @@
     const nbp_stage &us = p->stages[(size_t)st.user];
     const size_t esz = st.kind == NBP_STAGE_PRODUCTS ? sizeof(nbp_product_desc) : (st.kind == NBP_STAGE_COPIES || st.kind == NBP_STAGE_COPY_POINTS ?
                        sizeof(nbp_copy_desc) : sizeof(nbp_proposal_desc));
-    out[k] = {st.user, st.lane, (int32_t)((st.offset - us.offset) / esz), st.n, st.waits.empty() ? -1 : st.waits[0], st.signals ? 1 : 0};
-  }
+    out[k] = {st.user, st.lane, st.gathered ? 0 : (int32_t)((st.offset - us.offset) / esz), st.n, st.waits.empty() ? -1 : st.waits[0], st.signals ? 1 : 0};
+  }
+  return NBP_OK;
+}
+
+nbp_status nbp_program_sink_plan(nbp_program *p, int32_t *gained, int32_t cap, int32_t *n_out) {
+  if (!p || !n_out || (!gained && cap > 0)) return fail(NBP_ERR_ARG, "null argument");
+  if (!p->finalized) return fail(NBP_ERR_ARG, "program not finalized");
+  const int np = p->parts.empty() ? 0 : (int)p->parts.size() - 1;
+  *n_out = np;
+  for (int k = 0; k < np && k < cap; k++) gained[k] = p->parts[(size_t)k].gained;
   return NBP_OK;
 }
 
@@ -4087,6 +4263,9 @@
   out->lane_waits = c->lane_waits;
   out->lane_side_updates = c->lane_side_updates;
   if (reset) c->lane_side_launches = c->lane_waits = c->lane_side_updates = 0;
+  out->sunk_updates = c->sunk_updates;
+  out->sink_launches = c->sink_launches;
+  if (reset) c->sunk_updates = c->sink_launches = 0;
   if (reset) HIPCHK(hipMemset(c->counters, 0, offsetof(nbp_counters, flags)));
   return NBP_OK;
 }
diff --git a/incrementalinference.jl_amd/csrc/nbp_host.cpp b/incrementalinference.jl_amd/csrc/nbp_host.cpp
--- a/incrementalinference.jl_amd/csrc/nbp_host.cpp
+++ b/incrementalinference.jl_amd/csrc/nbp_host.cpp
@@ -1426,7 +1426,9 @@
   if (!t || !ctx || !out) return hfail(NBP_ERR_ARG, "null argument");
   nbp_status rc = nbp_tree_schedule(t, seed);
   if (rc) return rc;
-  return assemble_program(ctx, t->stages, {{NBP_OPT_LAZY_BANDWIDTH, 1}}, out);
+  std::vector<std::array<int32_t, 2>> opts{{NBP_OPT_LAZY_BANDWIDTH, 1}};
+  if (t->owner.empty()) opts.push_back({NBP_OPT_UP_PASS_SINKS, 1});
+  return assemble_program(ctx, t->stages, opts, out);
 }
 
 nbp_status nbp_tree_set_owner(nbp_tree *t, const int32_t *owner, int32_t rank) {
```

Result: faster. 156,300 messages/s (median of 6 runs) (+8.4%).
